# Adelaide-Autonomous-Racing-Kit/ac-mpc

Measured on AMD Instinct MI355X. Metric: candidate-trajectories/sec (horizon=50), higher is better.
Workload: dtype f32; 1 GPU; monza (synthetic circuit): 4096 candidates x horizon 50 per solve per GPU, 4096 solves (poses) batched per launch (256 distinct poses); mode S rollout + cost + argmin + winner record; horizon=50, mode=S, layout=U[P][n][2][N], parallelism=candidate-sharded x1, one all-reduce(MIN) of 4096 packed keys per step

## Files before the change

ac-mpc_amd/acmpc_amd/_build.py:

```python
from __future__ import annotations

import os
import shutil
import subprocess

PKG_DIR = os.path.dirname(os.path.abspath(__file__))
CSRC_DIR = os.path.normpath(os.path.join(PKG_DIR, "..", "csrc"))
LIB_DIR = os.path.join(PKG_DIR, "lib")
LIB_PATH = os.path.join(LIB_DIR, "libacmpc_hip.so")
SOURCES = ("acmpc_kernels.hip", "acmpc_kernels_temporal.hip", "acmpc_capi.hip", "acmpc_prologue.hip", "acmpc_pf.hip",
           "acmpc_speed_profile.cpp", "acmpc_host_path.cpp", "acmpc_dynamic.hip", "acmpc_dynamic_terms.hip", "acmpc_identify.hip")
HEADERS = ("acmpc_kernels.h", "acmpc_device.h", "acmpc_dynamic.h", "acmpc_identify.h", "acmpc_frames.h", "acmpc_admm.h", "acmpc_prologue.h", "acmpc_lq.h", "acmpc_lq_box.h",
           os.path.join("..", "..", "include", "acmpc.h"))

HIPCC_FLAGS = ("--offload-arch=gfx950", "-O3", "-std=c++17", "-fPIC", "-ffp-contract=off", "-Wall", "-Wextra")
EXTRA_FLAGS = {"acmpc_kernels_temporal.hip": ("-fno-slp-vectorize",), "acmpc_speed_profile.cpp": ("-mfma",)}


def find_hipcc() -> str:
    for cand in (os.environ.get("HIPCC"), shutil.which("hipcc"), "/opt/rocm/bin/hipcc"):
        if cand and os.path.exists(cand):
            return cand
    raise RuntimeError("hipcc not found: set HIPCC or install ROCm")


FLAGS_PATH = os.path.join(LIB_DIR, "build_flags.txt")


def flag_record() -> str:
    lines = ["common: " + " ".join(HIPCC_FLAGS)]
    lines += ["%s: %s" % (src, " ".join(EXTRA_FLAGS.get(src, ()))) for src in SOURCES]
    lines.append("experiment: " + " ".join(os.environ.get("ACMPC_HIPCC_EXTRA", "").split()))
    return "\n".join(lines) + "\n"


def is_stale() -> bool:
    if not os.path.exists(LIB_PATH) or not os.path.exists(FLAGS_PATH):
        return True
    built = os.path.getmtime(LIB_PATH)
    deps = [os.path.join(CSRC_DIR, f) for f in SOURCES + HEADERS]
    deps.append(os.path.abspath(__file__))
    if any(os.path.getmtime(d) > built for d in deps):
        return True
    with open(FLAGS_PATH) as handle:
        return handle.read() != flag_record()


def build_library(force: bool = False, verbose: bool = False) -> str:
    if not force and not is_stale():
        return LIB_PATH
    os.makedirs(LIB_DIR, exist_ok=True)
    obj_dir = os.path.join(LIB_DIR, "obj")
    os.makedirs(obj_dir, exist_ok=True)
    hipcc = find_hipcc()

    def run(cmd):
        if verbose:
            print(" ".join(cmd))
        proc = subprocess.run(cmd, capture_output=True, text=True)
        if proc.returncode != 0:
            raise RuntimeError("hipcc failed:\n" + proc.stdout + proc.stderr)

    from concurrent.futures import ThreadPoolExecutor
    objects = [os.path.join(obj_dir, os.path.splitext(src)[0] + ".o") for src in SOURCES]
    experiment = tuple(os.environ.get("ACMPC_HIPCC_EXTRA", "").split())
    with ThreadPoolExecutor(max_workers=4) as pool:
        list(pool.map(lambda so: run([hipcc, *HIPCC_FLAGS, *EXTRA_FLAGS.get(so[0], ()), *experiment, "-c",
                                      os.path.join(CSRC_DIR, so[0]), "-o", so[1]]), zip(SOURCES, objects)))
    run([hipcc, "--offload-arch=gfx950", "-shared", "-fPIC", *objects, "-o", LIB_PATH])
    with open(FLAGS_PATH, "w") as handle:
        handle.write(flag_record())
    return LIB_PATH


if __name__ == "__main__":
    print(build_library(force=True, verbose=True))
```

ac-mpc_amd/csrc/acmpc_capi.hip:

```cpp
#include <dlfcn.h>
#include <hip/hip_runtime.h>
#include <rccl/rccl.h>

#include <cmath>
#include <cstdio>
#include <cstdlib>
#include <cstring>
#include <algorithm>
#include <atomic>
#include <chrono>
#include <functional>
#include <limits>
#include <new>
#include <string>
#include <vector>

#include "../../include/acmpc.h"
#include "acmpc_dynamic.h"
#include "acmpc_frames.h"
#include "acmpc_identify.h"
#include "acmpc_kernels.h"
#include "acmpc_lq.h"
#include "acmpc_lq_box.h"
#include "acmpc_prologue.h"
// ... 13 lines not shown
  int coef_stride = 0;

  std::vector<float> h_coef;
  int P_set = 0, n_set = 0;
  bool tables_dirty = false;
  bool frames_dirty = false;

  bool device_ready = false;
  bool touched_device = false;
  float* d_coef = nullptr;
  int64_t* d_partial_keys = nullptr;
  int* d_partial_feas = nullptr;
  size_t partial_slots = 0;
  bool stream_pending = false;
  acmpc::FinalizeArgs stream_fin{};
  int stream_fin_layout = 0;
  int stream_set = 0;
  double* d_soft_partial = nullptr;
  size_t soft_partial_doubles = 0;

  float* d_segments = nullptr;
  int segments_n = 0;
  int knot_begin[acmpc::kKnots + 1] = {};
  float* d_centre = nullptr;
  float* d_uref = nullptr;

  bool staging_ready = false;
  hipStream_t stream = nullptr;
  float* d_U = nullptr;
  float* d_x0 = nullptr;
  float* d_costs = nullptr;
  float* d_records = nullptr;
  int64_t* d_keys = nullptr;
  int* d_tickets = nullptr;
  unsigned tick_sequence = 0;
  float* d_trace = nullptr;
  std::vector<float> h_nn_frames;
  float* d_nn_frames = nullptr;
  int64_t* h_keys = nullptr;
  float* h_io = nullptr;

  struct OptKey {
    int P = 0, N = 0, n = 0, rounds = 0, has_uref = 0;
    double sigma_v = 0, sigma_k = 0, shrink = 0;
    bool operator==(const OptKey& o) const {
      return P == o.P && N == o.N && n == o.n && rounds == o.rounds && has_uref == o.has_uref &&
             sigma_v == o.sigma_v && sigma_k == o.sigma_k && shrink == o.shrink;
    }
  };
  static constexpr int kOptGraphs = 4;
  hipGraphExec_t opt_graph[kOptGraphs] = {nullptr, nullptr, nullptr, nullptr};
  OptKey opt_key[kOptGraphs];
  uint64_t opt_used[kOptGraphs] = {0, 0, 0, 0};
  uint64_t opt_clock = 0;
  bool opt_ready = false;
  unsigned char* h_opt = nullptr;
  unsigned char* d_opt = nullptr;
  size_t opt_capacity = 0;
  float* h_opt_records = nullptr;
  uint32_t* d_seed = nullptr;

  struct TickKey {
    int N = 0, n = 0, rounds = 0, from_map = 0;
    double sigma_v = 0, sigma_k = 0, shrink = 0;
    bool operator==(const TickKey& o) const {
      return N == o.N && n == o.n && rounds == o.rounds && from_map == o.from_map && sigma_v == o.sigma_v &&
             sigma_k == o.sigma_k && shrink == o.shrink;
    }
  };
  bool tick_ready = false;
  hipGraphExec_t tick_graph[kOptGraphs] = {nullptr, nullptr, nullptr, nullptr};
  TickKey tick_key[kOptGraphs];
  uint64_t tick_used[kOptGraphs] = {0, 0, 0, 0};
  unsigned char* h_tick = nullptr;
  unsigned char* d_tick = nullptr;
  unsigned char* h_tick_out = nullptr;
  std::vector<double> h_map;
  double map_spacing = 0.0;
  bool map_dirty = false;
  double* d_map = nullptr;
  double* d_coords = nullptr;
  double* d_warm = nullptr;
  int warm_stride = 0;
  int tick_last_n = 0;

  std::vector<double> h_tables;
  float* h_lq = nullptr;
  std::vector<double> tick_prev_table;
  double tick_prev_x0[3] = {0.0, 0.0, 0.0};
  std::vector<double> tick_lq_table;
  std::vector<double> tick_lq_scratch;
  std::vector<double> tick_host_coords;
  int tick_prev_n = 0;
  bool want_start_clocks = false;
  unsigned long long* d_start_clock = nullptr;
  size_t start_clock_slots = 0;
  int start_clock_count = 0;
  std::vector<acmpc::lqbox::State> lq_box_state;
  acmpc::lqbox::Workspace lq_box_ws;
  acmpc::lqbox::Result lq_box_last;
  int lq_box_iterations = 40;

  acmpc::LaunchOptions opt;
  struct Switches {
    bool no_verified_search = false, no_solo = false, no_fused_finalize = false, no_traced_finalize = false,
         no_chained_rounds = false, no_chained_stream = false, no_graph = false, no_fused_sampling = false, tick_graph = false, tick_no_flag = false, tick_no_inline_path = false, no_zero_copy = false,
         tailed_rollout = false,
         dynamic_matrix_rounds = false;
  } sw;

  std::vector<hipEvent_t> prof_start, prof_stop;
  size_t prof_used = 0;

  bool has_dynamics = false;
  acmpc::VehicleEnsemble vehicles{};
  int substeps = 1;
  double blend_lo = 0.0, blend_hi = 0.0;
  double vehicle_L[acmpc::kMaxVehicles] = {};
  double vehicle0[acmpc::kDynamicsCount] = {};
  unsigned char* d_identify = nullptr;
  float* d_identify_e = nullptr;
  size_t identify_e_floats = 0;
  std::vector<unsigned char> h_identify;
  double rate_weight[2] = {0.0, 0.0}, rate_max[2] = {HUGE_VAL, HUGE_VAL};
  double slip_weight = 0.0, slip_max = HUGE_VAL;
  std::vector<float> h_uprev;
  int uprev_P = 0;
  bool uprev_dirty = false;
  float* d_uprev = nullptr;

  mutable std::string err;
};

namespace {

int fail(const acmpc_ctx* ctx, int code, const std::string& msg) {
  if (ctx != nullptr) {
    ctx->err = msg;
  } else {
    g_create_error = msg;
  }
  return code;
}

int fail_hip(const acmpc_ctx* ctx, hipError_t e, const char* what) {
  (void)hipGetLastError();
  const bool nodev = (e == hipErrorNoDevice || e == hipErrorInvalidDevice || e == hipErrorInsufficientDriver ||
                      e == hipErrorNotInitialized);
  return fail(ctx, nodev ? ACMPC_ENODEVICE : ACMPC_EHIP,
              std::string(what) + ": " + hipGetErrorName(e) + " (" + hipGetErrorString(e) + ")");
}

#define ACMPC_HIP(ctx, call)                                   \
  do {                                                         \
    const hipError_t e_ = (call);                              \
    if (e_ != hipSuccess) return fail_hip((ctx), e_, #call);   \
  } while (0)

constexpr int kMaxVerifiedSteps = 256;

void verified_frames(const float* coef, int P, int n, std::vector<float>* out) {
  constexpr int W = acmpc::kVerifiedWindow;
  const int windows = n - W + 1;
  const int floats = acmpc::verified_frame_floats(n);
  out->assign(static_cast<size_t>(P) * floats, 0.0f);
  std::vector<acmpc::frames::Geometry> geometry(static_cast<size_t>(windows));
  for (int p = 0; p < P; ++p) {
    const float* t = coef + static_cast<size_t>(p) * n * acmpc::kCoefT;
    const float ox = t[0], oy = t[1];
    auto at = [t, ox, oy](int m, double& x, double& y) {
      x = static_cast<double>(t[m * acmpc::kCoefT] - ox);
      y = static_cast<double>(t[m * acmpc::kCoefT + 1] - oy);
    };
    double wn = 0.0;
    bool finite = true;
    for (int m = 0; m < n; ++m) {
      double x, y;
      at(m, x, y);
      finite = finite && std::isfinite(x) && std::isfinite(y);
      wn = std::max(wn, std::sqrt(x * x + y * y));
    }
    float largest_gap2 = 0.0f;
    for (int m = 0; m + 1 < n; ++m) {
      const float gap2 = acmpc::frames::squared_gap(t[(m + 1) * acmpc::kCoefT] - ox, t[(m + 1) * acmpc::kCoefT + 1] - oy,
                                                    t[m * acmpc::kCoefT] - ox, t[m * acmpc::kCoefT + 1] - oy);
      largest_gap2 = (gap2 > largest_gap2) ? gap2 : largest_gap2;
    }
    const int first = acmpc::frames::near_first(largest_gap2);
    double slab_max = 0.0;
// ... 435 lines not shown
  a.x0 = d_x0;
  a.coef = c->d_coef;
  a.costs = d_costs;
  a.partial_keys = c->d_partial_keys;
  a.partial_feas = c->d_partial_feas;
  a.P = P;
  a.N = N;
  a.n = n;
  a.index_offset = 0;
  a.w = c->w;
  acmpc::FinalizeArgs f{};
  if (regen != nullptr) {
    f.regenerate = true;
    f.centre = regen->d_centre;
    f.centre_stride = regen->centre_stride;
    f.u_ref = regen->d_uref;
    f.u_extra = regen->d_extra;
    f.spec = regen->spec;
  }
  f.U = d_U;
  f.x0 = d_x0;
  f.coef = c->d_coef;
  f.partial_keys = c->d_partial_keys;
  f.partial_feas = c->d_partial_feas;
  f.keys_out = d_keys;
  f.records = d_records;
  f.blocks_per_problem = shape.blocks_per_problem;
  f.P = P;
  f.N = N;
  f.n = n;
  f.index_offset = 0;
  f.w = c->w;
  hipEvent_t e0 = nullptr, e1 = nullptr;
  if (c->prof_used < c->prof_start.size()) {
    e0 = c->prof_start[c->prof_used];
    e1 = c->prof_stop[c->prof_used];
    ++c->prof_used;
  }
  ACMPC_HIP(c, acmpc::launch_rollout_tailed(layout, shape, a, f, c->d_tickets, s, e0, e1));
  return ACMPC_OK;
}

int ensure_matrix(acmpc_ctx* c) {
  const acmpc_params& p = c->prm;
  ACMPC_HIP(c, alloc_once(&c->d_U, static_cast<size_t>(p.max_problems) * p.max_candidates * p.max_steps * 2 * sizeof(float)));
  return ACMPC_OK;
}

int ensure_staging(acmpc_ctx* c) {
  if (c->staging_ready) return ACMPC_OK;
  c->touched_device = true;
  const acmpc_params& p = c->prm;
  const size_t cand = static_cast<size_t>(p.max_problems) * p.max_candidates;
  ACMPC_HIP(c, alloc_once(&c->d_centre, static_cast<size_t>(p.max_problems) * p.max_steps * 2 * sizeof(float)));
  ACMPC_HIP(c, alloc_once(&c->d_uref, static_cast<size_t>(p.max_problems) * p.max_steps * 2 * sizeof(float)));
  if (c->stream == nullptr) ACMPC_HIP(c, hipStreamCreateWithFlags(&c->stream, hipStreamNonBlocking));
  if (p.mode != ACMPC_MODE_DYNAMIC) {
    const int rc_matrix = ensure_matrix(c);
    if (rc_matrix != ACMPC_OK) return rc_matrix;
  }
  const size_t state_floats = p.mode == ACMPC_MODE_DYNAMIC ? acmpc::kDynamicStateFloats : 3;
  ACMPC_HIP(c, alloc_once(&c->d_x0, static_cast<size_t>(p.max_problems) * state_floats * sizeof(float)));
  ACMPC_HIP(c, alloc_once(&c->d_costs, cand * sizeof(float)));
  ACMPC_HIP(c, alloc_once(&c->d_records,
                          static_cast<size_t>(p.max_problems) * acmpc_record_floats(p.max_steps) * sizeof(float)));
  ACMPC_HIP(c, alloc_once(&c->d_keys, static_cast<size_t>(p.max_problems) * sizeof(int64_t)));
  const int rc_tail = ensure_tail_buffers(c);
  if (rc_tail != ACMPC_OK) return rc_tail;
  ACMPC_HIP(c, host_alloc_once(&c->h_keys, static_cast<size_t>(p.max_problems) * sizeof(int64_t)));
  ACMPC_HIP(c, host_alloc_once(&c->h_io, (static_cast<size_t>(p.max_problems) * (state_floats + acmpc_record_floats(p.max_steps)) + 4) * sizeof(float)));
  if (p.lq_candidate != 0 && c->h_lq == nullptr) {
    const size_t lq_bytes = static_cast<size_t>(p.max_problems) * p.max_steps * 2 * sizeof(float);
    ACMPC_HIP(c, host_alloc_once(&c->h_lq, lq_bytes));
    std::memset(c->h_lq, 0, lq_bytes);
  }
  c->staging_ready = true;
  return ACMPC_OK;
}

const char* const kOptionNames[] = {
    "ACMPC_SHAPE", "ACMPC_T_PACK", "ACMPC_NO_TILE", "ACMPC_TILE_ROWS", "ACMPC_TILE_TABLE", "ACMPC_NO_TRIO_ROUNDS",
    "ACMPC_NO_QUAD_ROUNDS", "ACMPC_NO_PAIR_ROUNDS", "ACMPC_SOLO_REGISTERS", "ACMPC_SOLO_SPLIT", "ACMPC_NO_VERIFIED_SEARCH",
    "ACMPC_NO_SOLO", "ACMPC_NO_FUSED_FINALIZE", "ACMPC_NO_TRACED_FINALIZE", "ACMPC_NO_CHAINED_ROUNDS", "ACMPC_NO_GRAPH",
    "ACMPC_NO_FUSED_SAMPLING", "ACMPC_TICK_GRAPH", "ACMPC_TICK_NO_FLAG", "ACMPC_TICK_NO_INLINE_PATH", "ACMPC_NO_ZERO_COPY", "ACMPC_TAILED_ROLLOUT", "ACMPC_NO_GROUP_FINALIZE", "ACMPC_FINALIZE_WAVES",
    "ACMPC_NO_CHAINED_STREAM", "ACMPC_LQ_BOX_ITERATIONS", "ACMPC_START_CLOCKS", "ACMPC_DYNAMIC_MATRIX_ROUNDS",
    "ACMPC_CONFORMANT_SYNC"};

bool apply_option(acmpc_ctx* c, const char* name, const char* value) {
  const std::string key(name);
  const bool present = value != nullptr && value[0] != '\0';
  const bool on = present && !(value[0] == '0' && value[1] == '\0');
  auto tri = [&](int* field) { *field = present ? (value[0] == '1' ? 1 : 0) : -1; return true; };
  acmpc::LaunchOptions& o = c->opt;
  if (key == "ACMPC_SHAPE") {
    o.shape_block = o.shape_cpt = 0;
    if (present && std::sscanf(value, "%d,%d", &o.shape_block, &o.shape_cpt) != 2) o.shape_block = o.shape_cpt = 0;
    return true;
  }
  if (key == "ACMPC_T_PACK") { o.temporal_pack = present ? (value[0] == '1' ? 1 : 2) : 0; return true; }
  if (key == "ACMPC_NO_TILE") { o.no_tile = on; return true; }
  if (key == "ACMPC_TILE_ROWS") { o.tile_rows = present ? std::atoi(value) : -1; return true; }
  if (key == "ACMPC_TILE_TABLE") { o.tile_table = present ? (value[0] == 'l' ? 1 : 2) : 0; return true; }
  if (key == "ACMPC_NO_TRIO_ROUNDS") { o.no_trio_rounds = on; return true; }
  if (key == "ACMPC_NO_QUAD_ROUNDS") { o.no_quad_rounds = on; return true; }
  if (key == "ACMPC_NO_PAIR_ROUNDS") { o.no_pair_rounds = on; return true; }
  if (key == "ACMPC_SOLO_REGISTERS") return tri(&o.solo_registers);
  if (key == "ACMPC_SOLO_SPLIT") return tri(&o.solo_split);
  if (key == "ACMPC_NO_GROUP_FINALIZE") { o.no_group_finalize = on; return true; }
  if (key == "ACMPC_FINALIZE_WAVES") { o.finalize_waves = on; return true; }
  acmpc_ctx::Switches& w = c->sw;
  if (key == "ACMPC_NO_VERIFIED_SEARCH") { w.no_verified_search = on; return true; }
  if (key == "ACMPC_NO_SOLO") { w.no_solo = on; return true; }
  if (key == "ACMPC_NO_FUSED_FINALIZE") { w.no_fused_finalize = on; return true; }
  if (key == "ACMPC_NO_TRACED_FINALIZE") { w.no_traced_finalize = on; return true; }
  if (key == "ACMPC_NO_CHAINED_ROUNDS") { w.no_chained_rounds = on; return true; }
  if (key == "ACMPC_NO_CHAINED_STREAM") { w.no_chained_stream = on; return true; }
  if (key == "ACMPC_NO_GRAPH") { w.no_graph = on; return true; }
  if (key == "ACMPC_NO_FUSED_SAMPLING") { w.no_fused_sampling = on; return true; }
  if (key == "ACMPC_TICK_GRAPH") { w.tick_graph = on; return true; }
  if (key == "ACMPC_TICK_NO_FLAG") { w.tick_no_flag = on; return true; }
  if (key == "ACMPC_TICK_NO_INLINE_PATH") { w.tick_no_inline_path = on; return true; }
  if (key == "ACMPC_NO_ZERO_COPY") { w.no_zero_copy = on; return true; }
  if (key == "ACMPC_TAILED_ROLLOUT") { w.tailed_rollout = on; return true; }
  if (key == "ACMPC_START_CLOCKS") { c->want_start_clocks = on; return true; }
  if (key == "ACMPC_DYNAMIC_MATRIX_ROUNDS") { w.dynamic_matrix_rounds = on; return true; }
  if (key == "ACMPC_CONFORMANT_SYNC") {
    w.no_solo = w.no_fused_finalize = w.no_chained_stream = w.tick_no_flag = on;
    if (on) w.tailed_rollout = false;
    return true;
  }
  if (key == "ACMPC_LQ_BOX_ITERATIONS") { c->lq_box_iterations = present ? std::max(0, std::atoi(value)) : 40; return true; }
  return false;
}

}

extern "C" {

const char* acmpc_version(void) { return "acmpc-hip 0.1 gfx950"; }

int32_t acmpc_record_floats(int32_t n) { return ACMPC_REC_HEADER + 2 * n + 3 * (n + 1); }

int acmpc_lq_plan(const double* table, int32_t n, const double x0[3], const double step_cost[3], const double r_term[2],
                  const double final_cost[3], const float u_min[2], const float u_max[2], float* plan) {
  if (table == nullptr || x0 == nullptr || step_cost == nullptr || r_term == nullptr || final_cost == nullptr ||
      u_min == nullptr || u_max == nullptr || plan == nullptr || n < 1)
    return ACMPC_EINVAL;
  return acmpc::lq::plan(table, n, x0, step_cost, r_term, final_cost, u_min, u_max, plan) ? ACMPC_OK : ACMPC_ESTATE;
}

int acmpc_lq_box_plan(const double* table, int32_t n, const double x0[3], const double step_cost[3], const double r_term[2],
                      const double final_cost[3], const float u_min[2], const float u_max[2], double margin, double w_bound,
                      int32_t iterations, double* state, float* plan, double* info) {
  if (table == nullptr || x0 == nullptr || step_cost == nullptr || r_term == nullptr || final_cost == nullptr ||
      u_min == nullptr || u_max == nullptr || plan == nullptr || state == nullptr || info == nullptr || n < 1)
    return ACMPC_EINVAL;
  if (!acmpc::lq::plan(table, n, x0, step_cost, r_term, final_cost, u_min, u_max, plan)) return ACMPC_ESTATE;
  acmpc::lqbox::State st;
  const size_t m = static_cast<size_t>(n) * 2;
  if (state[0] == static_cast<double>(n)) {
    st.n = n;
    st.wx.assign(state + 1, state + 1 + m);
    st.wu.assign(state + 1 + m, state + 1 + 2 * m);
    st.lx.assign(state + 1 + 2 * m, state + 1 + 3 * m);
    st.lu.assign(state + 1 + 3 * m, state + 1 + 4 * m);
  }
  acmpc::lqbox::Workspace ws;
  const acmpc::lqbox::Result r = acmpc::lqbox::refine(table, n, x0, step_cost, r_term, final_cost, u_min, u_max, margin,
                                                      w_bound, iterations, st, ws, plan);
  state[0] = static_cast<double>(st.n);
  if (st.n == n) {
    std::copy(st.wx.begin(), st.wx.end(), state + 1);
    std::copy(st.wu.begin(), st.wu.end(), state + 1 + m);
    std::copy(st.lx.begin(), st.lx.end(), state + 1 + 2 * m);
    std::copy(st.lu.begin(), st.lu.end(), state + 1 + 3 * m);
  }
  info[0] = r.iterations, info[1] = r.chosen, info[2] = r.triggered ? 1.0 : 0.0, info[3] = r.cost.J, info[4] = r.cost.V;
  return ACMPC_OK;
}

int acmpc_lq_box_stats(const acmpc_ctx* c, double info[5]) {
  if (c == nullptr || info == nullptr) return ACMPC_EINVAL;
  const acmpc::lqbox::Result& r = c->lq_box_last;
  info[0] = r.iterations, info[1] = r.chosen, info[2] = r.triggered ? 1.0 : 0.0, info[3] = r.cost.J, info[4] = r.cost.V;
  return ACMPC_OK;
}

int64_t acmpc_pack_key(float cost, uint32_t index) { return acmpc::pack_key(cost, index); }

float acmpc_key_cost(int64_t key) {
  const int32_t hi = static_cast<int32_t>(key >> 32);
  const int32_t bits = (hi >= 0) ? hi : (hi ^ 0x7fffffff);
  float f;
  std::memcpy(&f, &bits, sizeof f);
  return f;
}

uint32_t acmpc_key_index(int64_t key) { return static_cast<uint32_t>(key & 0xffffffffLL); }

const char* acmpc_last_error(const acmpc_ctx* ctx) { return ctx != nullptr ? ctx->err.c_str() : g_create_error.c_str(); }

int acmpc_create(const acmpc_params* params, acmpc_ctx** out) {
  if (params == nullptr || out == nullptr) return fail(nullptr, ACMPC_EINVAL, "null argument");
  *out = nullptr;
// ... 834 lines not shown
  if (rc != ACMPC_OK) return rc;
  Regenerate regen{d_centre, centre_stride, d_u_ref, make_spec(c, sigma_v, sigma_kappa, seed, round)};
  const int blocks = c->prm.mode == ACMPC_MODE_DYNAMIC
                         ? acmpc::dynamic_blocks_per_problem(P, N, c->vehicles.K)
                         : acmpc::choose_shape(P, N, ACMPC_LAYOUT_STEP_MAJOR, c->prm.mode, n, c->opt).blocks_per_problem;
  return finalize(c, d_keys, nullptr, d_x0, nullptr, P, N, n, ACMPC_LAYOUT_STEP_MAJOR, 0, d_records, blocks, s, &regen);
}

int acmpc_rollout_sampled_device(acmpc_ctx* c, const float* d_x0, const float* d_centre, int32_t centre_stride,
                                 const float* d_u_ref, int32_t P, int32_t N, int32_t n, int64_t index_offset,
                                 double sigma_v, double sigma_kappa, uint64_t seed, uint32_t round, float* d_costs,
                                 int64_t* d_keys, void* stream) {
  if (c == nullptr) return ACMPC_EINVAL;
  if (d_x0 == nullptr || d_centre == nullptr) return fail(c, ACMPC_EINVAL, "null device pointer");
  if (c->prm.mode != ACMPC_MODE_DYNAMIC)
    return fail(c, ACMPC_ESTATE, "acmpc_rollout_sampled_device is mode D's: modes S and T draw inside acmpc_optimize");
  if (centre_stride < 2 * n) return fail(c, ACMPC_EINVAL, "centre_stride must be at least 2 n");
  if (index_offset < 0 || index_offset + N > 0xffffffffLL) return fail(c, ACMPC_EINVAL, "global index exceeds 32 bits");
  int rc = check_shape(c, P, N, n, ACMPC_LAYOUT_STEP_MAJOR);
  if (rc != ACMPC_OK) return rc;
  rc = ensure_device(c);
  if (rc != ACMPC_OK) return rc;
  hipStream_t s = static_cast<hipStream_t>(stream);
  rc = upload_tables(c, s);
  if (rc != ACMPC_OK) return rc;
  rc = rollout_sampled_dynamic(c, d_x0, d_centre, centre_stride, d_u_ref, P, N, n, index_offset, sigma_v, sigma_kappa, seed,
                               round, d_costs, s);
  if (rc != ACMPC_OK || d_keys == nullptr) return rc;
  return finalize(c, nullptr, d_keys, d_x0, nullptr, P, N, n, ACMPC_LAYOUT_STEP_MAJOR, index_offset, nullptr,
                  acmpc::dynamic_blocks_per_problem(P, N, c->vehicles.K), s);
}

extern "C++" {
namespace {

struct OptInputs {
  const float* x0;
  const float* centre;
  const float* uref;
  const float* coef;
  const float* frames = nullptr;
  const float* extra = nullptr;
  std::function<bool()> before_last;
};

const float* own_frames(const acmpc_ctx* c) { return c->h_nn_frames.empty() ? nullptr : c->d_nn_frames; }

bool use_fused_finalize(const acmpc_ctx* c, int n) {
  return !c->sw.no_fused_finalize && acmpc::fused_finalize_fits(c->prm.mode, n);
}

bool use_traced_finalize(const acmpc_ctx* c, int P, int N, int n) {
  return !c->sw.no_traced_finalize && acmpc::traced_finalize_fits(c->prm.mode, n) &&
         static_cast<long long>(P) * ((N + 63) / 64) <= kTraceBlocks;
}

bool lq_plan_into(acmpc_ctx* c, const double* table, int n, const double start[3], float* out,
                  bool start_is_pose = false, int problem = 0) {
  double x0[3] = {start[0], start[1], start[2]};
  if (start_is_pose || c->prm.mode == ACMPC_MODE_TEMPORAL) acmpc::lq::frenet_start(table, n, start, x0);
  const float lo[2] = {c->w.ulo0, c->w.ulo1}, hi[2] = {c->w.uhi0, c->w.uhi1};
  const bool finite_start = std::isfinite(x0[0]) && std::isfinite(x0[1]) && std::isfinite(x0[2]);
  if (finite_start && acmpc::lq::plan(table, n, x0, c->prm.step_cost, c->prm.r_term, c->prm.final_cost, lo, hi, out)) {
    if (c->prm.lq_candidate == 2) {
      if (c->lq_box_state.size() <= static_cast<size_t>(problem)) c->lq_box_state.resize(static_cast<size_t>(problem) + 1);
      c->lq_box_last = acmpc::lqbox::refine(table, n, x0, c->prm.step_cost, c->prm.r_term, c->prm.final_cost, lo, hi,
                                            c->prm.margin, c->prm.w_bound, c->lq_box_iterations,
                                            c->lq_box_state[static_cast<size_t>(problem)], c->lq_box_ws, out);
    }
    return true;
  }
  if (c->prm.lq_candidate == 2 && c->lq_box_state.size() > static_cast<size_t>(problem))
    c->lq_box_state[static_cast<size_t>(problem)].reset();
  const double *kappa = table + 3 * static_cast<size_t>(n), *vel = table + 6 * static_cast<size_t>(n);
  for (int i = 0; i < n; ++i) {
    out[2 * i] = std::fmin(std::fmax(static_cast<float>(vel[i]), lo[0]), hi[0]);
    out[2 * i + 1] = std::fmin(std::fmax(static_cast<float>(kappa[i]), lo[1]), hi[1]);
  }
  return false;
}

int enqueue_rounds(acmpc_ctx* c, const OptInputs& in, int P, int N, int n, int rounds, double sigma_v, double sigma_k,
                   double shrink, uint64_t seed, const uint32_t* d_seed, hipStream_t s, bool fused,
                   float* final_records = nullptr, unsigned* done = nullptr, unsigned done_value = 0) {
  const bool has_uref = in.uref != nullptr;
  const bool fused_finalize = use_fused_finalize(c, n);
  const int layout = ACMPC_LAYOUT_STEP_MAJOR;
  const int rec_floats = acmpc_record_floats(n);
  double scale = 1.0;
  for (int r = 0; r < rounds; ++r, scale *= shrink) {
    const float* d_c = (r == 0) ? in.centre : c->d_records + ACMPC_REC_HEADER;
    const int stride = (r == 0) ? 2 * n : rec_floats;
    const float* d_ref = has_uref ? in.uref : nullptr;
    const float* d_extra = nullptr;
    if (r + 1 == rounds && in.extra != nullptr && (!in.before_last || in.before_last())) d_extra = in.extra;
    if (!fused) {
      const bool softmin = c->prm.centre_update == 1;
      const bool mean_round = softmin && r > 0;
      if (mean_round)
        ACMPC_HIP(c, hipMemcpy2DAsync(c->d_uref, static_cast<size_t>(2 * n) * sizeof(float),
                                      c->d_records + ACMPC_REC_HEADER, static_cast<size_t>(rec_floats) * sizeof(float),
                                      static_cast<size_t>(2 * n) * sizeof(float), P, hipMemcpyDeviceToDevice, s));
      int rc = sample(c, mean_round ? c->d_centre : d_c, mean_round ? 2 * n : stride, mean_round ? c->d_uref : d_ref, P,
                      N, n, layout, 0, sigma_v * scale, sigma_k * scale, seed, static_cast<uint32_t>(r), c->d_U, s,
                      d_seed, d_extra);
      if (rc != ACMPC_OK) return rc;
      acmpc::LaunchShape shape;
      rc = rollout(c, in.x0, c->d_U, P, N, n, layout, 0, softmin ? c->d_costs : nullptr, s, &shape);
      if (rc != ACMPC_OK) return rc;
      rc = finalize(c, nullptr, softmin ? c->d_keys : nullptr, in.x0, c->d_U, P, N, n, layout, 0, c->d_records,
                    shape.blocks_per_problem, s);
      if (rc != ACMPC_OK) return rc;
      if (softmin && r + 1 < rounds) {
        acmpc::SoftminArgs sm{};
        sm.costs = c->d_costs;
        sm.keys = c->d_keys;
        sm.U = c->d_U;
        sm.partial = c->d_soft_partial;
        sm.mean = c->d_centre;
        sm.weight_sum = nullptr;
        sm.chunks = acmpc::softmin_chunks(N);
        sm.P = P;
        sm.N = N;
        sm.n = n;
        sm.lambda = static_cast<float>(c->prm.softmin_lambda);
        ACMPC_HIP(c, acmpc::launch_softmin(layout, sm, s));
      }
      continue;
    }
    int rc = upload_segments(c, n, s);
    if (rc != ACMPC_OK) return rc;
    const int blocks = (N + 63) / 64;
    const bool traced = fused_finalize && use_traced_finalize(c, P, N, n);
    const bool chain = traced && blocks <= acmpc::kChainBlocks && !c->sw.no_chained_rounds;
    const size_t set = (chain && (r & 1)) ? 1 : 0;
    const size_t trace_set_floats = static_cast<size_t>(kTraceBlocks) * acmpc::trace_floats(c->prm.max_steps);
    float* d_trace = c->d_trace + set * trace_set_floats;
    acmpc::RolloutArgs ra{};
    ra.x0 = in.x0;
    ra.coef = in.coef;
    ra.nn_frames = !c->sw.no_verified_search ? in.frames : nullptr;
    ra.partial_keys = c->d_partial_keys + set * c->partial_slots;
    ra.partial_feas = c->d_partial_feas + set * c->partial_slots;
    ra.P = P;
    ra.N = N;
    ra.n = n;
    ra.index_offset = 0;
    ra.w = c->w;
    acmpc::SampleArgs sa{};
    sa.centre = d_c;
    sa.centre_stride = stride;
    sa.u_ref = d_ref;
    sa.u_extra = d_extra;
    sa.P = P;
    sa.N = N;
    sa.n = n;
    sa.spec = make_spec(c, sigma_v * scale, sigma_k * scale, seed, static_cast<uint32_t>(r));
    sa.spec.seed_ptr = d_seed;
    if (chain && r > 0) {
      sa.prev_keys = c->d_partial_keys + (set ^ 1) * c->partial_slots;
      sa.prev_trace = c->d_trace + (set ^ 1) * trace_set_floats;
      sa.prev_blocks = blocks;
      sa.prev_pitch = acmpc::trace_floats(n);
    }
    hipEvent_t e0 = nullptr, e1 = nullptr;
    if (c->prof_used < c->prof_start.size()) {
      e0 = c->prof_start[c->prof_used];
      e1 = c->prof_stop[c->prof_used];
      ++c->prof_used;
    }
    if (fused_finalize) {
      const bool last = r + 1 == rounds;
      const bool tail = last || !chain;
      const acmpc::FusedFinalize ff{tail ? c->d_tickets : nullptr,
                                    (last && final_records != nullptr) ? final_records : c->d_records, !last,
                                    traced ? d_trace : nullptr, acmpc::trace_floats(n),
                                    last ? done : nullptr, done_value};
      ACMPC_HIP(c, acmpc::launch_rollout_sampled(c->prm.mode, ra, sa, ff, s, e0, e1, c->opt));
    } else {
      ACMPC_HIP(c, acmpc::launch_rollout_sampled(c->prm.mode, ra, sa, acmpc::FusedFinalize{nullptr, nullptr, false, nullptr, 0, nullptr, 0}, s, e0, e1, c->opt));
      Regenerate regen{d_c, stride, d_ref, sa.spec, d_extra};
      rc = finalize(c, nullptr, nullptr, in.x0, nullptr, P, N, n, layout, 0, c->d_records, (N + 63) / 64, s, &regen,
                    in.coef);
      if (rc != ACMPC_OK) return rc;
    }
  }
  return ACMPC_OK;
}

}
}

int acmpc_optimize(acmpc_ctx* c, const float* x0, const float* centre, const float* u_ref, int32_t P, int32_t N,
                   int32_t n, int32_t rounds, const double sigma[2], double shrink, uint64_t seed, float* records) {
  if (c == nullptr) return ACMPC_EINVAL;
  if (x0 == nullptr || centre == nullptr || sigma == nullptr || records == nullptr)
    return fail(c, ACMPC_EINVAL, "null argument");
  if (rounds < 1) return fail(c, ACMPC_EINVAL, "rounds must be positive");
  const int layout = ACMPC_LAYOUT_STEP_MAJOR;
  int rc = check_shape(c, P, N, n, layout);
  if (rc != ACMPC_OK) return rc;
  if (c->prm.mode == ACMPC_MODE_DYNAMIC && c->prm.centre_update == 1 && !(c->prm.softmin_lambda > 0.0))
    return fail(c, ACMPC_EINVAL, "softmin_lambda must be positive");
  rc = ensure_device(c);
  if (rc != ACMPC_OK) return rc;
  rc = ensure_staging(c);
  if (rc != ACMPC_OK) return rc;
  if (c->prm.mode == ACMPC_MODE_DYNAMIC) {
    return optimize_dynamic(c, x0, centre, u_ref, P, N, n, rounds, sigma, shrink, seed, records);
  }
  hipStream_t s = c->stream;
  const size_t x0_bytes = static_cast<size_t>(P) * 3 * sizeof(float);
  const size_t path_bytes = static_cast<size_t>(P) * n * 2 * sizeof(float);
  const size_t table_bytes = static_cast<size_t>(P) * n * c->coef_stride * sizeof(float);
  const size_t rec_bytes = static_cast<size_t>(P) * acmpc_record_floats(n) * sizeof(float);
  const bool has_uref = u_ref != nullptr;
  const bool has_extra = c->prm.lq_candidate != 0 && c->h_tables.size() == static_cast<size_t>(P) * 7 * n;
  if (has_extra) {
    for (int p = 0; p < P; ++p) {
      const double start[3] = {x0[3 * p], x0[3 * p + 1], x0[3 * p + 2]};
      (void)lq_plan_into(c, c->h_tables.data() + static_cast<size_t>(p) * 7 * n, n, start, c->h_lq + static_cast<size_t>(p) * n * 2,
                         false, p);
    }
  }

  if (c->prof_used < c->prof_start.size() || c->sw.no_graph) {
    rc = upload_tables(c, s);
    if (rc != ACMPC_OK) return rc;
    ACMPC_HIP(c, hipMemcpyAsync(c->d_x0, x0, x0_bytes, hipMemcpyHostToDevice, s));
    ACMPC_HIP(c, hipMemcpyAsync(c->d_centre, centre, path_bytes, hipMemcpyHostToDevice, s));
    if (has_uref) ACMPC_HIP(c, hipMemcpyAsync(c->d_uref, u_ref, path_bytes, hipMemcpyHostToDevice, s));
    OptInputs in{c->d_x0, c->d_centre, has_uref ? c->d_uref : nullptr, c->d_coef, own_frames(c)};
    in.extra = has_extra ? c->h_lq : nullptr;
    rc = enqueue_rounds(c, in, P, N, n, rounds, sigma[0], sigma[1], shrink, seed, nullptr, s,
                        !c->sw.no_fused_sampling && c->prm.centre_update == 0);
    if (rc != ACMPC_OK) return rc;
    ACMPC_HIP(c, hipMemcpyAsync(records, c->d_records, rec_bytes, hipMemcpyDeviceToHost, s));
    ACMPC_HIP(c, hipStreamSynchronize(s));
    return ACMPC_OK;
  }

  auto align16 = [](size_t v) { return (v + 15) & ~static_cast<size_t>(15); };
  const size_t off_x0 = 0, off_centre = align16(off_x0 + x0_bytes), off_uref = align16(off_centre + path_bytes),
               off_table = align16(off_uref + path_bytes), off_seed = align16(off_table + table_bytes);
  if (!c->opt_ready) {
    const acmpc_params& p = c->prm;
    const size_t cap = 64 + 16 * 5 + static_cast<size_t>(p.max_problems) *
                                         (3 + 4 * static_cast<size_t>(p.max_steps) +
                                          static_cast<size_t>(p.max_steps) * c->coef_stride) * sizeof(float);
    ACMPC_HIP(c, host_alloc_once(&c->h_opt, cap));
    ACMPC_HIP(c, alloc_once(&c->d_opt, cap));
    c->opt_capacity = cap;
    ACMPC_HIP(c, host_alloc_once(&c->h_opt_records,
                                 static_cast<size_t>(p.max_problems) * acmpc_record_floats(p.max_steps) * sizeof(float)));
    ACMPC_HIP(c, alloc_once(&c->d_seed, 2 * sizeof(uint32_t)));
    c->opt_ready = true;
  }
  acmpc_ctx::OptKey key;
  key.P = P;
  key.N = N;
  key.n = n;
  key.rounds = rounds;
// ... 70 lines not shown
  ACMPC_HIP(c, hipGraphLaunch(c->opt_graph[slot], s));
  ACMPC_HIP(c, hipStreamSynchronize(s));
  std::memcpy(records, c->h_opt_records, rec_bytes);
  return ACMPC_OK;
}


extern "C++" {
namespace {

size_t align16(size_t v) { return (v + 15) & ~static_cast<size_t>(15); }

struct TickLayout {
  size_t coords, centre_in, host_total;
  size_t seed, x0, centre, uref, coef, frames, total;
  explicit TickLayout(int n, int coef_stride = ACMPC_COEF_STRIDE_SPATIAL) {
    coords = align16(sizeof(acmpc::TickHeader));
    centre_in = align16(coords + static_cast<size_t>(n + 1) * 3 * sizeof(double));
    host_total = align16(centre_in + static_cast<size_t>(n) * 2 * sizeof(float));
    seed = 0;
    x0 = 16;
    centre = 32;
    uref = align16(centre + static_cast<size_t>(n) * 2 * sizeof(float));
    coef = align16(uref + static_cast<size_t>(n) * 2 * sizeof(float));
    frames = align16(coef + static_cast<size_t>(n) * coef_stride * sizeof(float));
    total = align16(frames + static_cast<size_t>(acmpc::verified_frame_floats(std::max(n, acmpc::kVerifiedWindow))) * sizeof(float));
  }
};

struct TickOutLayout {
  size_t record, table, status, coords, done, total;
  explicit TickOutLayout(int n) {
    record = 0;
    table = align16(static_cast<size_t>(acmpc_record_floats(n)) * sizeof(float));
    status = align16(table + static_cast<size_t>(7) * n * sizeof(double));
    coords = status + 16;
    done = align16(coords + static_cast<size_t>(n + 1) * 3 * sizeof(double));
    total = done + 16;
  }
};

int upload_map(acmpc_ctx* c, hipStream_t s) {
  if (!c->map_dirty) return ACMPC_OK;
  for (hipGraphExec_t& g : c->tick_graph) {
    if (g != nullptr) (void)hipGraphExecDestroy(g);
    g = nullptr;
  }
  ACMPC_HIP(c, hipStreamSynchronize(s));
  (void)hipFree(c->d_map);
  c->d_map = nullptr;
  ACMPC_HIP(c, hipMalloc(reinterpret_cast<void**>(&c->d_map), c->h_map.size() * sizeof(double)));
  ACMPC_HIP(c, hipMemcpyAsync(c->d_map, c->h_map.data(), c->h_map.size() * sizeof(double), hipMemcpyHostToDevice, s));
  ACMPC_HIP(c, hipStreamSynchronize(s));
  c->map_dirty = false;
  return ACMPC_OK;
}

int map_window_args(acmpc_ctx* c, int H, int points, const TickOutLayout& out, acmpc::MapWindowArgs* a) {
  if (c->h_map.empty()) return fail(c, ACMPC_ESTATE, "no map bound (acmpc_bind_map)");
  if (points < H || points % H != 0) return fail(c, ACMPC_EINVAL, "centreline_points must be a multiple of the horizon");
  a->header = reinterpret_cast<const acmpc::TickHeader*>(c->h_tick);
  a->centre = c->d_map;
  a->M = static_cast<int>(c->h_map.size() / 2);
  a->count = static_cast<int>(std::lround(150.0 / c->map_spacing)) + 1;
  if (a->count < 2 || a->count > a->M) return fail(c, ACMPC_EINVAL, "the map is shorter than the 150 m look-ahead window");
  a->points = points;
  a->H = H;
  a->coords = c->d_coords;
  a->coords_out = reinterpret_cast<double*>(c->h_tick_out + out.coords);
  a->first_out = reinterpret_cast<int*>(c->h_tick_out + out.status) + 2;
  return ACMPC_OK;
}

int ensure_tick(acmpc_ctx* c) {
  if (c->tick_ready) return ACMPC_OK;
  c->touched_device = true;
  const int n_cap = std::min(c->prm.max_steps, acmpc::kPrologueMaxSteps);
  ACMPC_HIP(c, host_alloc_once(&c->h_tick, TickLayout(n_cap).host_total));
  ACMPC_HIP(c, alloc_once(&c->d_tick, TickLayout(n_cap).total));
  ACMPC_HIP(c, host_alloc_once(&c->h_tick_out, TickOutLayout(n_cap).total));
  std::memset(c->h_tick_out, 0, TickOutLayout(n_cap).total);
  ACMPC_HIP(c, alloc_once(&c->d_coords, static_cast<size_t>(n_cap + 1) * 3 * sizeof(double)));
  c->warm_stride = 2 + 3 * n_cap;
  const size_t warm_bytes = static_cast<size_t>(2) * c->warm_stride * sizeof(double);
  ACMPC_HIP(c, alloc_once(&c->d_warm, warm_bytes));
  ACMPC_HIP(c, hipMemset(c->d_warm, 0, warm_bytes));
  ACMPC_HIP(c, hipStreamSynchronize(nullptr));
  c->tick_ready = true;
  return ACMPC_OK;
}

}
}

int acmpc_control_tick(acmpc_ctx* c, const acmpc_tick* t, const double* coords, const float* centre, double* table,
                       float* record, double* decision, double* projected_control, double* prediction,
                       double* cum_time, double* times, double* accelerations, double* steer_rates, double* info,
                       double* coords_out) {
  if (c == nullptr) return ACMPC_EINVAL;
  if (t == nullptr || table == nullptr || record == nullptr || decision == nullptr ||
      projected_control == nullptr || prediction == nullptr || cum_time == nullptr || times == nullptr ||
      accelerations == nullptr || steer_rates == nullptr || info == nullptr)
    return fail(c, ACMPC_EINVAL, "null argument");
  if (t->struct_size != sizeof(acmpc_tick)) return fail(c, ACMPC_EINVAL, "acmpc_tick size mismatch");
  if (c->stream_pending)
    return fail(c, ACMPC_ESTATE, "a batch of acmpc_solve_stream_device is pending: acmpc_solve_stream_flush first");
  if (c->prm.mode == ACMPC_MODE_DYNAMIC)
    return fail(c, ACMPC_ESTATE, "mode D has no control tick: use acmpc_set_paths + acmpc_optimize");
  if (c->prm.centre_update != 0) return fail(c, ACMPC_ESTATE, "acmpc_control_tick needs a handle with centre_update = 0");
  const bool temporal = c->prm.mode == ACMPC_MODE_TEMPORAL;
  if (temporal && !(c->prm.dt > 0.0)) return fail(c, ACMPC_ESTATE, "mode T needs a positive dt");
  const int H = t->horizon, n = H - 1, N = t->n_candidates;
  if (H < 3 || t->rounds < 1 || N < 1) return fail(c, ACMPC_EINVAL, "need horizon >= 3, rounds >= 1, n_candidates >= 1");
  if (n > c->prm.max_steps || N > c->prm.max_candidates) return fail(c, ACMPC_ECAPACITY, "horizon or candidates exceed capacity");
  if (n > acmpc::kPrologueMaxSteps) return fail(c, ACMPC_ESTATE, "the device prologue holds at most 128 steps");
  if (centre == nullptr && t->centre_is_reference == 0) return fail(c, ACMPC_EINVAL, "null centre");
  if (coords == nullptr && c->h_map.empty()) return fail(c, ACMPC_EINVAL, "null coords and no map bound");
  if (!acmpc::fused_finalize_fits(c->prm.mode, n)) return fail(c, ACMPC_ESTATE, "fused finalize does not fit");
  int rc = ensure_device(c);
  if (rc != ACMPC_OK) return rc;
  rc = ensure_staging(c);
  if (rc != ACMPC_OK) return rc;
  rc = ensure_tick(c);
  if (rc != ACMPC_OK) return rc;
  hipStream_t s = c->stream;
  const TickLayout in(n, c->coef_stride);
  const TickOutLayout out(n);
  const int rec_floats = acmpc_record_floats(n);
  const bool from_map = coords == nullptr;
  acmpc::MapWindowArgs ma{};
  if (from_map) {
    rc = map_window_args(c, H, t->centreline_points, out, &ma);
    if (rc != ACMPC_OK) return rc;
    rc = upload_map(c, s);
    if (rc != ACMPC_OK) return rc;
    ma.centre = c->d_map;
  }

  acmpc::PrologueArgs pa{};
  pa.header = reinterpret_cast<const acmpc::TickHeader*>(c->h_tick);
  pa.coords = reinterpret_cast<const double*>(c->h_tick + in.coords);
  if (from_map) {
    pa.map_centre = c->d_map;
    pa.map_M = ma.M;
    pa.map_count = ma.count;
    pa.map_points = ma.points;
    pa.map_first = reinterpret_cast<const int*>(c->d_coords);
    pa.coords_out = ma.coords_out;
    pa.index_out = ma.first_out;
    ma.coords = nullptr;
    ma.coords_out = nullptr;
    ma.first_out = reinterpret_cast<int*>(c->d_coords);
  }
  pa.temporal = temporal ? 1 : 0;
  pa.centre_in = reinterpret_cast<const float*>(c->h_tick + in.centre_in);
  pa.x0 = reinterpret_cast<float*>(c->d_tick + in.x0);
  pa.u_ref = reinterpret_cast<float*>(c->d_tick + in.uref);
  pa.coef = reinterpret_cast<float*>(c->d_tick + in.coef);
  pa.frames = (temporal && c->prm.nn_ahead < 0 && n >= acmpc::kVerifiedWindow && acmpc::trio_frames_fit(n) &&
               !c->opt.no_trio_rounds && !c->sw.no_verified_search)
                  ? reinterpret_cast<float*>(c->d_tick + in.frames)
                  : nullptr;
  pa.centre = reinterpret_cast<float*>(c->d_tick + in.centre);
  pa.seed = reinterpret_cast<uint32_t*>(c->d_tick + in.seed);
  pa.table_out = reinterpret_cast<double*>(c->h_tick_out + out.table);
  pa.status = reinterpret_cast<int*>(c->h_tick_out + out.status);
  pa.warm_state = c->d_warm;
  pa.warm_stride = c->warm_stride;
  pa.warm_capacity = (c->warm_stride - 2) / 3;
  pa.margin = c->prm.margin;
  pa.u_lo0 = c->prm.u_min[0];
  pa.u_lo1 = c->prm.u_min[1];
  pa.u_hi0 = c->prm.u_max[0];
  pa.u_hi1 = c->prm.u_max[1];
  const bool direct = use_fused_finalize(c, n);
  const bool use_graph = c->sw.tick_graph;
  const bool lq_on = c->prm.lq_candidate != 0;
  const double lq_offset = t->offset;
  const bool host_window = lq_on && from_map && t->map_index >= 0;
  const int window_M = ma.M, window_count = ma.count, window_points = ma.points;
  auto plan_previous = [c, n, H, given = coords, lq_offset, t, host_window, window_M, window_count, window_points]() -> bool {
    const double* coords = given;
    if (host_window) {
      c->tick_host_coords.resize(static_cast<size_t>(H) * 3);
      const int first = ((t->map_index % window_M) + window_M) % window_M;
      const acmpc::MapFrame frame = acmpc::map_frame(c->h_map.data(), window_M, first);
      for (int r = 0; r < H; ++r) {
        double row[3];
        acmpc::map_path_row(c->h_map.data(), window_M, first, window_count, window_points, H, r, t->lateral_offset, frame, row);
        for (int e = 0; e < 3; ++e) c->tick_host_coords[static_cast<size_t>(3) * r + e] = row[e];
      }
      coords = c->tick_host_coords.data();
    }
    const bool have_previous = c->tick_prev_n == n;
    if (!have_previous && coords == nullptr) return false;
    if (coords == nullptr) return lq_plan_into(c, c->tick_prev_table.data(), n, c->tick_prev_x0, c->h_lq);
    c->tick_lq_table.resize(static_cast<size_t>(7) * n);
    if (acmpc_waypoint_table(coords, H, kEps, c->tick_lq_table.data()) != ACMPC_OK) return false;
    {
      c->tick_lq_scratch.resize(static_cast<size_t>(3) * n);
      double* ceiling = c->tick_lq_scratch.data();
      double* dual = ceiling + n;
      double* profile = c->tick_lq_table.data() + static_cast<size_t>(6) * n;
      const double* spacing = c->tick_lq_table.data() + static_cast<size_t>(4) * n;
      int32_t iterations = 0;
      if (acmpc_velocity_ceiling(c->tick_lq_table.data() + static_cast<size_t>(3) * n, n, t->ay_max, t->ki_min, t->v_min,
                                 t->v_max, t->localised, t->has_end_velocity, t->end_velocity, ceiling) != ACMPC_OK)
        return false;
      const bool swept = t->qp_method == 0 &&
                         acmpc_speed_profile_exact(ceiling, spacing, n, t->a_min, t->a_max, t->v_min, profile, dual) == 0;
      if (!swept) {
        if (have_previous) {
          std::memcpy(profile, c->tick_prev_table.data() + static_cast<size_t>(6) * n, static_cast<size_t>(n) * sizeof(double));
        } else if (acmpc_speed_profile_qp(ceiling, spacing, n, t->a_min, t->a_max, t->v_min, t->qp_max_iter, t->qp_check_every,
                                          t->qp_eps_abs, t->qp_eps_rel, profile, dual, 0, &iterations) != 0) {
          return false;
        }
      }
    }
    const double pose[3] = {lq_offset, 0.0, M_PI / 2.0};
    return lq_plan_into(c, c->tick_lq_table.data(), n, pose, c->h_lq, true);
  };
  const bool flagged = direct && !use_graph && !c->sw.tick_no_flag;
  unsigned* done_flag = reinterpret_cast<unsigned*>(c->h_tick_out + out.done);
  const unsigned done_value = ++c->tick_sequence;
  auto enqueue = [&](hipStream_t q, int* rc_rounds) -> hipError_t {
    hipError_t e = (from_map && t->map_index < 0) ? acmpc::launch_map_window(ma, q) : hipSuccess;
    if (e == hipSuccess) e = acmpc::launch_prologue(pa, n, q);
    if (e != hipSuccess) return e;
    OptInputs oi{pa.x0, pa.centre, pa.u_ref, pa.coef, pa.frames};
    if (lq_on) {
      oi.extra = c->h_lq;
      if (!use_graph) oi.before_last = plan_previous;
    }
    *rc_rounds = enqueue_rounds(c, oi, 1, N, n, t->rounds, t->sigma[0], t->sigma[1], t->shrink,
                                use_graph ? 0 : t->seed, use_graph ? pa.seed : nullptr, q, true,
                                direct ? reinterpret_cast<float*>(c->h_tick_out + out.record) : nullptr,
                                flagged ? done_flag : nullptr, done_value);
    if (*rc_rounds == ACMPC_OK && !direct)
      e = hipMemcpyAsync(c->h_tick_out + out.record, c->d_records, static_cast<size_t>(rec_floats) * sizeof(float),
                         hipMemcpyDeviceToHost, q);
    return e;
  };
  int slot = -1;
  if (use_graph) {
    acmpc_ctx::TickKey key;
    key.N = N;
    key.n = n;
    key.rounds = t->rounds;
    key.sigma_v = t->sigma[0];
    key.sigma_k = t->sigma[1];
    key.shrink = t->shrink;
    key.from_map = from_map ? (t->map_index < 0 ? -t->centreline_points : t->centreline_points) : 0;
    for (int g = 0; g < acmpc_ctx::kOptGraphs; ++g)
      if (c->tick_graph[g] != nullptr && key == c->tick_key[g]) slot = g;
    if (slot < 0) {
      slot = 0;
      for (int g = 1; g < acmpc_ctx::kOptGraphs; ++g)
        if (c->tick_used[g] < c->tick_used[slot]) slot = g;
      if (c->tick_graph[slot] != nullptr) {
        (void)hipGraphExecDestroy(c->tick_graph[slot]);
        c->tick_graph[slot] = nullptr;
      }
      rc = upload_segments(c, n, s);
      if (rc != ACMPC_OK) return rc;
      hipGraph_t graph = nullptr;
      ACMPC_HIP(c, hipStreamBeginCapture(s, hipStreamCaptureModeThreadLocal));
      int rc_rounds = ACMPC_OK;
      const hipError_t e = enqueue(s, &rc_rounds);
      const hipError_t e_end = hipStreamEndCapture(s, &graph);
      if (rc_rounds != ACMPC_OK) {
        if (graph != nullptr) (void)hipGraphDestroy(graph);
        return rc_rounds;
      }
      if (e != hipSuccess) {
        if (graph != nullptr) (void)hipGraphDestroy(graph);
        return fail_hip(c, e, "capturing the tick graph");
      }
      ACMPC_HIP(c, e_end);
      const hipError_t e_inst = hipGraphInstantiate(&c->tick_graph[slot], graph, nullptr, nullptr, 0);
      (void)hipGraphDestroy(graph);
      if (e_inst != hipSuccess) c->tick_graph[slot] = nullptr;
      ACMPC_HIP(c, e_inst);
      c->tick_key[slot] = key;
    }
    c->tick_used[slot] = ++c->opt_clock;
  } else {
    rc = upload_segments(c, n, s);
    if (rc != ACMPC_OK) return rc;
  }

  acmpc::TickHeader* h = reinterpret_cast<acmpc::TickHeader*>(c->h_tick);
  h->offset = t->offset;
  h->v_min = t->v_min;
  h->v_max = t->v_max;
  h->a_min = t->a_min;
  h->a_max = t->a_max;
  h->ay_max = t->ay_max;
  h->ki_min = t->ki_min;
  h->end_velocity = t->end_velocity;
  h->qp_eps_abs = t->qp_eps_abs;
  h->qp_eps_rel = t->qp_eps_rel;
  h->eps = kEps;
  h->horizon = H;
  h->localised = t->localised;
  h->has_end_velocity = t->has_end_velocity;
  h->centre_is_reference = t->centre_is_reference;
  h->qp_max_iter = t->qp_max_iter;
  h->qp_check_every = t->qp_check_every;
  h->qp_method = t->qp_method;
  h->seed_lo = static_cast<uint32_t>(t->seed);
  h->seed_hi = static_cast<uint32_t>(t->seed >> 32);
  h->use_map = from_map ? 1 : 0;
  h->map_index = t->map_index;
  h->pose_x = t->pose_x;
  h->pose_y = t->pose_y;
  h->lateral_offset = t->lateral_offset;
  if (!from_map) std::memcpy(c->h_tick + in.coords, coords, static_cast<size_t>(H) * 3 * sizeof(double));
  if (centre != nullptr) std::memcpy(c->h_tick + in.centre_in, centre, static_cast<size_t>(n) * 2 * sizeof(float));
  if (use_graph) {
    if (lq_on && !plan_previous()) {
      if (centre != nullptr && t->centre_is_reference == 0)
        std::memcpy(c->h_lq, centre, static_cast<size_t>(n) * 2 * sizeof(float));
      else
        std::memset(c->h_lq, 0, static_cast<size_t>(n) * 2 * sizeof(float));
    }
    ACMPC_HIP(c, hipGraphLaunch(c->tick_graph[slot], s));
  } else {
    pa.header_by_value = 1;
    pa.header_value = *h;
    if (!from_map && H <= acmpc::kInlinePathPoints && !c->sw.tick_no_inline_path) {
      pa.path_by_value = 1;
      std::memcpy(pa.coords_value, coords, static_cast<size_t>(H) * 3 * sizeof(double));
      if (centre != nullptr) std::memcpy(pa.centre_value, centre, static_cast<size_t>(n) * 2 * sizeof(float));
    }
    int rc_rounds = ACMPC_OK;
    const hipError_t e = enqueue(s, &rc_rounds);
    if (rc_rounds != ACMPC_OK || e != hipSuccess) {
      (void)hipStreamSynchronize(s);
      if (rc_rounds != ACMPC_OK) return rc_rounds;
      ACMPC_HIP(c, e);
    }
  }
  if (flagged) {
    volatile unsigned* flag = done_flag;
    const auto give_up = std::chrono::steady_clock::now() + std::chrono::milliseconds(200);
    unsigned spins = 0;
    while (*flag != done_value) {
      __builtin_ia32_pause();
      if ((++spins & 0x3fffu) == 0 && std::chrono::steady_clock::now() > give_up) break;
    }
    std::atomic_thread_fence(std::memory_order_acquire);
    if (*flag != done_value) {
      ACMPC_HIP(c, hipStreamSynchronize(s));
      if (*flag != done_value) return fail(c, ACMPC_EHIP, "the tick finished without its completion flag");
    }
  } else {
    ACMPC_HIP(c, hipStreamSynchronize(s));
  }
  c->tick_last_n = n;

  const float* rec = reinterpret_cast<const float*>(c->h_tick_out + out.record);
  std::memcpy(record, rec, static_cast<size_t>(rec_floats) * sizeof(float));
  std::memcpy(table, c->h_tick_out + out.table, static_cast<size_t>(7) * n * sizeof(double));
  const int* status = reinterpret_cast<const int*>(c->h_tick_out + out.status);
  const float* ru = rec + ACMPC_REC_HEADER;
  const float* rx = ru + 2 * n;
  double biggest = 0.0;
  bool finite = std::isfinite(rec[ACMPC_REC_COST]) && std::isfinite(rec[ACMPC_REC_VIOLATION]);
  for (int i = 0; i < 3 * (n + 1); ++i) {
    decision[i] = static_cast<double>(rx[i]);
    biggest = std::max(biggest, std::fabs(decision[i]));
    finite = finite && std::isfinite(rx[i]);
  }
  for (int i = 0; i < 2 * n; ++i) {
    decision[3 * (n + 1) + i] = static_cast<double>(ru[i]);
    biggest = std::max(biggest, std::fabs(static_cast<double>(ru[i])));
    finite = finite && std::isfinite(ru[i]);
  }
  rc = temporal ? acmpc_unpack_decision_temporal(decision, n, c->prm.dt, c->prm.wheelbase, projected_control, prediction,
                                                 cum_time, times, accelerations, steer_rates)
                : acmpc_unpack_decision(decision, n, table, c->prm.wheelbase, projected_control, prediction, cum_time,
                                        times, accelerations, steer_rates);
  if (rc != ACMPC_OK) return fail(c, rc, "acmpc_unpack_decision");
  info[0] = rec[ACMPC_REC_COST];
  info[1] = rec[ACMPC_REC_VIOLATION];
  info[2] = rec[ACMPC_REC_NFEASIBLE];
  info[3] = biggest;
  info[4] = status[0];
  info[5] = status[1];
  info[6] = from_map ? static_cast<double>(status[2]) : -1.0;
  info[7] = finite ? 0.0 : 1.0;
  if (lq_on) {
    c->tick_prev_n = (finite && status[0] == 0) ? n : 0;
    if (c->tick_prev_n != 0) {
      c->tick_prev_table.assign(table, table + static_cast<size_t>(7) * n);
      for (int q = 0; q < 3; ++q) c->tick_prev_x0[q] = static_cast<double>(rx[q]);
    }
  }
  if (coords_out != nullptr)
    std::memcpy(coords_out, from_map ? reinterpret_cast<const void*>(c->h_tick_out + out.coords)
                                     : reinterpret_cast<const void*>(coords),
                static_cast<size_t>(H) * 3 * sizeof(double));
  return ACMPC_OK;
}

int acmpc_bind_map(acmpc_ctx* c, const double* centre, int32_t M, double spacing) {
  if (c == nullptr) return ACMPC_EINVAL;
  if (centre == nullptr || M < 3 || !(spacing > 0.0)) return fail(c, ACMPC_EINVAL, "need a centre line of >= 3 points and a positive spacing");
  c->h_map.assign(centre, centre + 2 * static_cast<size_t>(M));
  c->map_spacing = spacing;
  c->map_dirty = true;
  return ACMPC_OK;
}

int acmpc_map_reference_path(acmpc_ctx* c, int32_t map_index, double pose_x, double pose_y, double lateral_offset,
                             int32_t horizon, int32_t centreline_points, double* coords, int32_t* first_index) {
  if (c == nullptr) return ACMPC_EINVAL;
  if (coords == nullptr) return fail(c, ACMPC_EINVAL, "null output");
  const int n = horizon - 1;
  if (horizon < 3 || n > std::min(c->prm.max_steps, acmpc::kPrologueMaxSteps))
    return fail(c, ACMPC_ECAPACITY, "horizon out of range for this handle");
  int rc = ensure_device(c);
  if (rc != ACMPC_OK) return rc;
  rc = ensure_staging(c);
  if (rc != ACMPC_OK) return rc;
  rc = ensure_tick(c);
  if (rc != ACMPC_OK) return rc;
  hipStream_t s = c->stream;
  const TickOutLayout out(n);
  acmpc::MapWindowArgs ma{};
  rc = map_window_args(c, horizon, centreline_points, out, &ma);
  if (rc != ACMPC_OK) return rc;
  rc = upload_map(c, s);
  if (rc != ACMPC_OK) return rc;
  ma.centre = c->d_map;
  acmpc::TickHeader* h = reinterpret_cast<acmpc::TickHeader*>(c->h_tick);
  h->use_map = 1;
  h->map_index = map_index;
  h->pose_x = pose_x;
  h->pose_y = pose_y;
  h->lateral_offset = lateral_offset;
  ACMPC_HIP(c, acmpc::launch_map_window(ma, s));
  ACMPC_HIP(c, hipStreamSynchronize(s));
  std::memcpy(coords, c->h_tick_out + out.coords, static_cast<size_t>(horizon) * 3 * sizeof(double));
  if (first_index != nullptr) *first_index = reinterpret_cast<const int*>(c->h_tick_out + out.status)[2];
  return ACMPC_OK;
}
// ... 242 lines not shown
```

ac-mpc_amd/csrc/acmpc_kernels.h:

```cpp
#pragma once
#include <hip/hip_runtime.h>
#include <stdint.h>

#include "acmpc_device.h"

namespace acmpc {

struct RolloutArgs {
  const float* U;
  const float* x0;
  const float* coef;
  const float* nn_frames;
  float* costs;
  int64_t* partial_keys;
  int* partial_feas;
  int P, N, n;
  int64_t index_offset;
  Weights w;
  int even_progress = 0;
  unsigned long long* start_clock = nullptr;
};

struct FinalizeArgs {
  const float* U;
  const float* x0;
  const float* coef;
  const int64_t* partial_keys;
  const int* partial_feas;
  const int64_t* keys_in;
  int64_t* keys_out;
  float* records;
  bool regenerate;
  bool controls_only;
  const float* centre;
  const float* u_ref;
  const float* u_extra;
  int centre_stride;
  SampleSpec spec;
  int blocks_per_problem;
  int P, N, n;
  int64_t index_offset;
  Weights w;
};

struct SoftminArgs {
  const float* costs;
  const int64_t* keys;
  const float* U;
  double* partial;
  float* mean;
  double* weight_sum;
  int chunks;
  int P, N, n;
  float lambda;
};

constexpr int kSampleKnots = kKnots;

struct SampleArgs {
  const float* centre;
  const float* u_ref;
  const float* u_extra;
  float* U;
  int centre_stride;
  int P, N, n;
  int64_t index_offset;
  SampleSpec spec;
  const int64_t* prev_keys;
  const float* prev_trace;
  int prev_blocks;
  int prev_pitch;
};
constexpr int kTileRowsMaxSteps = 80;
constexpr int kChainBlocks = 256;

struct LaunchOptions {
  int shape_block = 0, shape_cpt = 0;
  int temporal_pack = 0;
  bool no_tile = false;
  int tile_rows = -1;
  int tile_table = 0;
  bool no_trio_rounds = false, no_quad_rounds = false, no_pair_rounds = false;
  int solo_registers = -1, solo_split = -1;
  bool no_group_finalize = false;
  bool finalize_waves = false;
};

struct LaunchShape {
  int block;
  int cpt;
  int blocks_per_problem;
  bool tile;
  int tile_waves;
  int pack;
  int tile_table = 0;
};

LaunchShape choose_shape(int P, int N, int layout, int mode, int n, const LaunchOptions& opt = LaunchOptions());
int max_blocks_per_problem(int N);
size_t tile_lds_bytes(int mode, int n);

hipError_t launch_rollout(int mode, int layout, const LaunchShape& shape, const RolloutArgs& args, hipStream_t s,
                          hipEvent_t start = nullptr, hipEvent_t stop = nullptr);
hipError_t launch_rollout_temporal_plain(const LaunchShape& shape, const RolloutArgs& args, hipStream_t s,
                                         hipEvent_t start, hipEvent_t stop);
hipError_t launch_rollout_tile_rows_plain(const LaunchShape& shape, const RolloutArgs& args, hipStream_t s,
                                          hipEvent_t start, hipEvent_t stop);
hipError_t launch_finalize(int mode, int layout, const FinalizeArgs& args, hipStream_t s,
                           const LaunchOptions& opt = LaunchOptions());
bool chained_rollout_fits(int mode, int layout, const LaunchShape& shape, int P, const FinalizeArgs& fin, int fin_layout);
hipError_t launch_rollout_chained(int layout, const LaunchShape& shape, const RolloutArgs& args, const FinalizeArgs& fin,
                                  int fin_layout, hipStream_t s, hipEvent_t e0, hipEvent_t e1);
bool tailed_rollout_fits(int mode, int layout, const LaunchShape& shape, int n);
hipError_t launch_rollout_tailed(int layout, const LaunchShape& shape, const RolloutArgs& args, const FinalizeArgs& fin,
                                 int* tickets, hipStream_t s, hipEvent_t start = nullptr, hipEvent_t stop = nullptr);
hipError_t launch_sample(int layout, const SampleArgs& args, hipStream_t s);
constexpr int kTicketGroups = 8;
constexpr int kTicketStride = 64;
constexpr int kTicketGroupsMax = 32;
constexpr int kSoloBlocks = 1024;
struct FusedFinalize {
  int* tickets;
  float* records;
  bool controls_only;
  float* trace;
  int trace_pitch;
  unsigned* done;
  unsigned done_value;
  int64_t* keys_out = nullptr;
  int ticket_groups = 0;
};

hipError_t launch_rollout_sampled(int mode, const RolloutArgs& rollout, const SampleArgs& sample,
                                  const FusedFinalize& fused, hipStream_t s, hipEvent_t start = nullptr,
                                  hipEvent_t stop = nullptr, const LaunchOptions& opt = LaunchOptions());
bool solo_fits(int P, int N, int n, int layout, const LaunchOptions& opt = LaunchOptions());
int solo_trace_floats(int n);
hipError_t launch_rollout_solo(int layout, const RolloutArgs& args, const FusedFinalize& fused, hipStream_t s,
                               hipEvent_t start = nullptr, hipEvent_t stop = nullptr,
                               const LaunchOptions& opt = LaunchOptions());
int trace_floats(int n);
bool trio_frames_fit(int n);
bool traced_finalize_fits(int mode, int n);
bool fused_finalize_fits(int mode, int n);
int softmin_chunks(int N);
hipError_t launch_softmin(int layout, const SoftminArgs& args, hipStream_t s);
hipError_t launch_softmin_sampled(const SoftminArgs& args, const SampleArgs& sample, hipStream_t s);

}
```

ac-mpc_amd/csrc/acmpc_kernels.hip:

```cpp
#include "acmpc_kernels.h"

#include <hip/hip_ext.h>

#include <algorithm>
#include <cstdint>
#include <cstdio>
#include <cstdlib>
#include <type_traits>

#pragma clang fp contract(off)

#if defined(__HIP_DEVICE_COMPILE__) && !defined(__gfx950__)
#error "acmpc kernels are written for gfx950 (MI355X): see the note above before building for another architecture"
#endif

namespace acmpc {

namespace {

typedef float f32x4 __attribute__((ext_vector_type(4)));

#ifdef ACMPC_STAMPS
__device__ unsigned long long g_stamps[4096 * 16];
#define ACMPC_STAMP(slot)                                                                                         \
  do {                                                                                                            \
    if ((threadIdx.x & 63) == 0)                                                                                  \
      g_stamps[((blockIdx.y * gridDim.x + blockIdx.x) * 2 + (threadIdx.x >> 6)) * 16 + (slot)] = wall_clock64(); \
  } while (0)
#else
#define ACMPC_STAMP(slot) \
  do {                    \
  } while (0)
#endif

template <int CPT>
struct VecOf;
template <>
struct VecOf<1> {
  using type = float;
};
template <>
struct VecOf<2> {
  using type = f32x2;
};
template <>
struct VecOf<4> {
  using type = f32x4;
};

template <int CPT>
__device__ __forceinline__ void unpack(const typename VecOf<CPT>::type& v, float (&out)[CPT]) {
  if constexpr (CPT == 1) {
    out[0] = v;
  } else {
#pragma unroll
    for (int j = 0; j < CPT; ++j) out[j] = v[j];
  }
}

template <int LAYOUT, int CPT>
__device__ __forceinline__ void load_controls(const float* __restrict__ U, int p, int N, int n, int i, int c0,
                                              float (&v)[CPT], float (&k)[CPT]) {
  if constexpr (LAYOUT == 1) {
    using V = typename VecOf<CPT>::type;
    const float* row = U + (static_cast<size_t>(p) * n + i) * 2 * static_cast<size_t>(N) + c0;
    unpack<CPT>(__builtin_nontemporal_load(reinterpret_cast<const V*>(row)), v);
    unpack<CPT>(__builtin_nontemporal_load(reinterpret_cast<const V*>(row + N)), k);
  } else {
#pragma unroll
    for (int j = 0; j < CPT; ++j) {
      const f32x2 vk = *reinterpret_cast<const f32x2*>(U + ((static_cast<size_t>(p) * N + c0 + j) * n + i) * 2);
      v[j] = vk[0];
      k[j] = vk[1];
    }
  }
}

template <typename T>
__device__ __forceinline__ void publish(T* where, T value) {
  __hip_atomic_store(where, value, __ATOMIC_RELAXED, __HIP_MEMORY_SCOPE_AGENT);
}
template <typename T>
__device__ __forceinline__ T observe(const T* where) {
// ... 1010 lines not shown
  }
  wave_lds_handoff();

  float J = 0.0f, V = 0.0f;
  for (int base = 0; base < n; base += kAhead) {
    f32x4 first[kAhead];
    float ht[kAhead];
#pragma unroll
    for (int j = 0; j < kAhead; ++j) {
      const int i = min(base + j, n - 1);
      first[j] = *reinterpret_cast<const f32x4*>(s_terms + i * kGroupRow);
      ht[j] = s_terms[i * kGroupRow + 4];
    }
#pragma unroll
    for (int j = 0; j < kAhead; ++j) {
      if (base + j < n) {
        J = J + first[j][0];
        V = V + first[j][1];
        V = V + first[j][2];
        V = V + first[j][3];
        V = V + ht[j];
      }
    }
  }
  wave_lds_handoff();
  if (owner) {
    if (sub == 0) {
      const StateS st{ey, ep, t, J, V};
      s_rec[0] = finish_spatial(st, w);
      s_rec[1] = V;
      s_rec[2] = static_cast<float>(nfeas);
      s_rec[3] = 1.0f;
    }
  } else {
    for (int e = sub; e < rec_floats; e += kLanes) s_rec[e] = (e == 2) ? static_cast<float>(nfeas) : 0.0f;
  }
  wave_lds_handoff();
  const int count = min(kProblems, a.P - p_first) * rec_floats;
  float* __restrict__ out = a.records + static_cast<size_t>(p_first) * rec_floats;
  const int whole = ((reinterpret_cast<uintptr_t>(out) & 15u) == 0) ? (count & ~3) : 0;
  for (int e = 4 * lane; e < whole; e += 4 * kWave) *reinterpret_cast<f32x4*>(out + e) = *reinterpret_cast<const f32x4*>(s_group + e);
  for (int e = whole + lane; e < count; e += kWave) out[e] = s_group[e];
}

template <int LAYOUT>
__global__ void __launch_bounds__(kWave) finalize_groups_kernel(const FinalizeArgs a) {
  extern __shared__ __attribute__((aligned(16))) float s_group[];
  finalize_group<LAYOUT, kGroupPass, kGroupAhead>(a, static_cast<int>(blockIdx.x), s_group);
}

constexpr int kFinalizeWaves = 4;

template <int LAYOUT>
__global__ void __launch_bounds__(kFinalizeWaves * kWave) finalize_waves_kernel(const FinalizeArgs a) {
  extern __shared__ __attribute__((aligned(16))) float s_group[];
  const int wave = static_cast<int>(threadIdx.x) / kWave;
  const int p = static_cast<int>(blockIdx.x) * kFinalizeWaves + wave;
  if (p >= a.P) return;
  finalize_group<LAYOUT, 1, kGroupAhead, kWave>(a, p, s_group + wave * group_finalize_floats_device(a.n));
}

#ifndef ACMPC_CHAINED_PASS
#define ACMPC_CHAINED_PASS 1
#endif
#ifndef ACMPC_CHAINED_AHEAD
#define ACMPC_CHAINED_AHEAD 4
#endif
template <int LAYOUT, int CPT, int BLOCK, int PACK>
__global__ void __launch_bounds__(BLOCK, 8) rollout_chained_kernel(const RolloutArgs a, const FinalizeArgs f) {
  extern __shared__ __attribute__((aligned(16))) unsigned char smem[];
  const int y = static_cast<int>(blockIdx.y);
  if (y >= a.P) {
    static_assert(BLOCK == kFinalizeWaves * kWave, "a finalize workgroup is four wavefronts, a problem each");
    const int wave = static_cast<int>(threadIdx.x) / kWave;
    const int p = ((y - a.P) * static_cast<int>(gridDim.x) + static_cast<int>(blockIdx.x)) * kFinalizeWaves + wave;
    if (p >= f.P) return;
    finalize_group<1, ACMPC_CHAINED_PASS, ACMPC_CHAINED_AHEAD, kWave>(
        f, p, reinterpret_cast<float*>(smem) + wave * group_finalize_floats_device(f.n));
    return;
  }
  rollout_block<0, LAYOUT, CPT, BLOCK, PACK, false>(a, smem, y);
}

__device__ __forceinline__ void finalize_from_trace(const RolloutArgs& a, const FusedFinalize& fused, const int p) {
  const int lane = threadIdx.x;
  const int n = a.n;
  const int blocks = static_cast<int>(gridDim.x);
  constexpr int kBatch = 4;
  int nfeas = 0;
  int64_t key = kKeyMax;
  for (int b0 = 0; b0 < blocks; b0 += kBatch * kWave) {
    int64_t kb[kBatch];
    int fb[kBatch];
#pragma unroll
    for (int q = 0; q < kBatch; ++q) {
      kb[q] = kKeyMax;
      fb[q] = 0;
      if (b0 + q * kWave < blocks) {
        const size_t slot = static_cast<size_t>(p) * blocks + min(b0 + q * kWave + lane, blocks - 1);
        kb[q] = observe(&a.partial_keys[slot]);
        fb[q] = observe(&a.partial_feas[slot]);
      }
    }
#pragma unroll
    for (int q = 0; q < kBatch; ++q) {
      const bool mine = b0 + q * kWave + lane < blocks;
      key = (mine && kb[q] < key) ? kb[q] : key;
      nfeas += mine ? fb[q] : 0;
    }
  }
  nfeas = wave_sum_int(nfeas);
  const int64_t best = wave_min_key(key);
  const int block = static_cast<int>(static_cast<int64_t>(static_cast<uint32_t>(best & 0xffffffffLL)) - a.index_offset) / kWave;
  const float* trace = fused.trace + (static_cast<size_t>(p) * blocks + block) * fused.trace_pitch;
  const int rec_floats = 4 + 2 * n + 3 * (n + 1);
  float* __restrict__ rec = fused.records + static_cast<size_t>(p) * rec_floats;
  const float* __restrict__ x0 = a.x0 + p * 3;
  const int count = fused.controls_only ? 4 + 2 * n : rec_floats;
  constexpr int kSlots = 8;
  for (int e0 = 0; e0 < count; e0 += kSlots * kWave) {
    float value[kSlots];
#pragma unroll
    for (int q = 0; q < kSlots; ++q) {
      if (e0 + q * kWave < count) {
        const int e = min(e0 + q * kWave + lane, count - 1);
        const float* src = trace + (e - 7);
        src = (e < 4 + 2 * n + 3) ? x0 + (e - (4 + 2 * n)) : src;
        src = (e < 4 + 2 * n) ? trace + (e - 4) : src;
        src = (e < 4) ? trace + 5 * n + (1 - min(e, 1)) : src;
        value[q] = observe(src);
      }
    }
#pragma unroll
    for (int q = 0; q < kSlots; ++q) {
      const int e = e0 + q * kWave + lane;
      if (e0 + q * kWave < count) {
        float out = value[q];
        if (fused.controls_only) out = (e == 0) ? key_cost(best) : (e == 1) ? 0.0f : out;
        out = (e == 2) ? static_cast<float>(nfeas) : (e == 3) ? 1.0f : out;
        if (e < count) rec[e] = out;
      }
    }
  }
}

__device__ __forceinline__ bool last_workgroup_of_problem(int* tickets, const int groups_cfg) {
  const int blocks = static_cast<int>(gridDim.x);
  const int group = static_cast<int>(blockIdx.x) & (groups_cfg - 1);
  const int group_size = (blocks - group + groups_cfg - 1) / groups_cfg;
  const int groups = min(blocks, groups_cfg);
  published();
  ACMPC_STAMP(5);
  int ticket = 0;
  if (threadIdx.x == 0) ticket = atomicAdd(&tickets[group * kTicketStride], 1);
  ticket = __builtin_amdgcn_readfirstlane(ticket);
  __atomic_signal_fence(__ATOMIC_SEQ_CST);
  if (ticket != group_size - 1) return false;
  ACMPC_STAMP(6);
  if (threadIdx.x == 0) {
    publish(&tickets[group * kTicketStride], 0);
    ticket = atomicAdd(&tickets[groups_cfg * kTicketStride], 1);
  }
  ticket = __builtin_amdgcn_readfirstlane(ticket);
  __atomic_signal_fence(__ATOMIC_SEQ_CST);
  if (ticket != groups - 1) return false;
  ACMPC_STAMP(7);
  if (threadIdx.x == 0) publish(&tickets[groups_cfg * kTicketStride], 0);
  return true;
}

#ifndef ACMPC_TAILED_WAVES
#define ACMPC_TAILED_WAVES 8
#endif
template <int MODE, int LAYOUT, int CPT, int BLOCK, int PACK>
__global__ void __launch_bounds__(BLOCK, ACMPC_TAILED_WAVES) rollout_tailed_kernel(const RolloutArgs a, const FinalizeArgs f, int* tickets) {
  extern __shared__ __attribute__((aligned(16))) unsigned char smem[];
  rollout_block<MODE, LAYOUT, CPT, BLOCK, PACK, true>(a, smem, static_cast<int>(blockIdx.y));
  if (threadIdx.x >= kWave) return;
  const int p = blockIdx.y;
  if (!last_workgroup_of_problem(tickets + static_cast<size_t>(p) * (kTicketGroups + 1) * kTicketStride, kTicketGroups)) return;
  finalize_problem<MODE, LAYOUT>(f, p, reinterpret_cast<float*>(smem + 64));
}

template <int MODE>
__device__ __forceinline__ void fused_tail(const RolloutArgs& a, const SampleArgs& smp, const FusedFinalize& fused,
                                           const bool traced, float* s_finalize) {
  const int p = blockIdx.y;
  if (fused.tickets == nullptr) return;
  if (!last_workgroup_of_problem(fused.tickets + static_cast<size_t>(p) * (kTicketGroups + 1) * kTicketStride, kTicketGroups)) return;
  auto signal_done = [&]() {
    if (fused.done == nullptr || p != 0) return;
    __threadfence_system();
    if (threadIdx.x == 0) __hip_atomic_store(fused.done, fused.done_value, __ATOMIC_RELAXED, __HIP_MEMORY_SCOPE_SYSTEM);
  };
  if (traced) {
    finalize_from_trace(a, fused, p);
    signal_done();
    return;
  }
  FinalizeArgs f{};
  f.x0 = a.x0;
  f.coef = a.coef;
  f.partial_keys = a.partial_keys;
  f.partial_feas = a.partial_feas;
  f.records = fused.records;
  f.regenerate = true;
  f.controls_only = fused.controls_only;
  f.centre = smp.centre;
  f.u_ref = smp.u_ref;
  f.u_extra = smp.u_extra;
  f.centre_stride = smp.centre_stride;
  f.spec = smp.spec;
  f.blocks_per_problem = static_cast<int>(gridDim.x);
  f.P = a.P;
  f.N = a.N;
  f.n = a.n;
  f.index_offset = a.index_offset;
  f.w = a.w;
  finalize_problem<MODE, 1>(f, p, s_finalize);
  signal_done();
}

template <int MODE>
__global__ void __launch_bounds__(kWave) rollout_sampled_kernel(const RolloutArgs a, const SampleArgs smp,
                                                                const FusedFinalize fused, const int rollout_lds_floats,
                                                                const int uniform_lds_floats) {
  extern __shared__ __attribute__((aligned(16))) float s_fused[];
  const int p = blockIdx.y;
  const bool traced = fused.trace != nullptr;
  rollout_sampled_body<MODE>(a, smp, s_fused, uniform_lds_floats, traced, rollout_lds_floats,
                             fused.trace + (static_cast<size_t>(p) * gridDim.x + blockIdx.x) * fused.trace_pitch);
  fused_tail<MODE>(a, smp, fused, traced, s_fused + rollout_lds_floats);
}

constexpr int kPairChunk = 7;
constexpr int kPairValues = 2;

__global__ void __launch_bounds__(2 * kWave) rollout_sampled_pair_kernel(const RolloutArgs a, const SampleArgs smp,
                                                                         const FusedFinalize fused,
                                                                         const int uniform_lds_floats,
                                                                         const int exchange_lds_floats) {
  extern __shared__ __attribute__((aligned(16))) float s_fused[];
  float* s_trace = s_fused;
  float* s_row = s_fused + uniform_lds_floats;
  const int p = blockIdx.y;
  const int lane = threadIdx.x & (kWave - 1);
  const bool consumer = threadIdx.x < kWave;
  const int n = a.n;
  float* s_centre = s_row + n * kCoefS;
  float* s_ref = s_centre + 2 * n;
  float* s_extra = s_ref + 2 * n;
  float* s_weight = s_extra + 2 * n;
  float* s_exchange = s_fused + exchange_lds_floats + lane;
  constexpr int kStepFloats = kPairValues * kWave, kBufferFloats = kPairChunk * kStepFloats;
  const int c = blockIdx.x * kWave + lane;
  const bool active = c < a.N;
  const Weights w = a.w;

  if (!consumer) {
    const SampleSpec sp = smp.spec;
    const float* __restrict__ centre = smp.centre + static_cast<size_t>(p) * smp.centre_stride;
    const float* __restrict__ ref = (smp.u_ref != nullptr) ? smp.u_ref + static_cast<size_t>(p) * n * 2 : nullptr;
    const float* __restrict__ extra = holds_candidate_2(a, smp) ? smp.u_extra + static_cast<size_t>(p) * n * 2 : nullptr;
    const float* __restrict__ knot_weight = sp.segments;
    const bool chained = smp.prev_keys != nullptr;
    constexpr int kPairs = (kStagedSteps + kWave - 1) / kWave;
    f32x2 g_centre[kPairs], g_ref[kPairs], g_extra[kPairs], g_weight[kPairs];
#pragma unroll
    for (int q = 0; q < kPairs; ++q) {
      const int j = min(lane + q * kWave, n - 1);
      if (!chained) g_centre[q] = reinterpret_cast<const f32x2*>(centre)[j];
      if (ref != nullptr) g_ref[q] = reinterpret_cast<const f32x2*>(ref)[j];
      if (extra != nullptr) g_extra[q] = reinterpret_cast<const f32x2*>(extra)[j];
      g_weight[q] = reinterpret_cast<const f32x2*>(knot_weight)[j];
    }
    int64_t prev_key[kChainBlocks / kWave];
    if (chained) {
#pragma unroll
      for (int q = 0; q < kChainBlocks / kWave; ++q)
// ... 71 lines not shown
        if (++in_chunk == kPairChunk || i == n - 1) {
          __syncthreads();
          in_chunk = 0;
          buffer ^= 1;
          out = s_exchange + buffer * kBufferFloats;
        }
      }
    }
    return;
  }

  {
    const float* __restrict__ coef = a.coef + static_cast<size_t>(p) * n * kCoefS;
    for (int q = lane; q < n * (kCoefS / 4); q += kWave)
      reinterpret_cast<f32x4*>(s_row)[q] = reinterpret_cast<const f32x4*>(coef)[q];
  }
  const float* __restrict__ x0 = a.x0 + p * 3;
  StateS st{x0[0], x0[1], x0[2], 0.0f, 0.0f};
  __syncthreads();
  struct StepInputs {
    float v, k;
    f32x4 lo, hi;
    float last;
  };
  auto inputs_of = [&](const float* in, int i) {
    StepInputs s;
    s.v = in[0];
    s.k = in[kWave];
    const float* t = s_row + i * kCoefS;
    s.lo = *reinterpret_cast<const f32x4*>(t);
    s.hi = *reinterpret_cast<const f32x4*>(t + 4);
    s.last = t[8];
    return s;
  };
  auto advance = [&](int i, const StepInputs& in) {
    const float row[9] = {in.lo[0], in.lo[1], in.lo[2], in.lo[3], in.hi[0], in.hi[1], in.hi[2], in.hi[3], in.last};
    step_spatial<float>(st, row, in.v, in.k, w);
    s_trace[(2 * n + 3 * i) * kWave + lane] = st.ey;
    s_trace[(2 * n + 3 * i + 1) * kWave + lane] = st.ep;
    s_trace[(2 * n + 3 * i + 2) * kWave + lane] = st.t;
  };
  for (int first = 0, buffer = 0; first < n; first += kPairChunk, buffer ^= 1) {
    __syncthreads();
    const float* in = s_exchange + buffer * kBufferFloats;
    if (first + kPairChunk <= n) {
      StepInputs steps[kPairChunk];
#pragma unroll
      for (int j = 0; j < kPairChunk; ++j) steps[j] = inputs_of(in + j * kStepFloats, first + j);
#pragma unroll
      for (int j = 0; j < kPairChunk; ++j) advance(first + j, steps[j]);
    } else {
      for (int j = 0; first + j < n; ++j) advance(first + j, inputs_of(in + j * kStepFloats, first + j));
    }
  }
  const float cost = finish_spatial<float>(st, w);
  s_trace[(5 * n) * kWave + lane] = st.V;
  s_trace[(5 * n + 1) * kWave + lane] = cost;
  if (active && a.costs != nullptr) a.costs[static_cast<size_t>(p) * a.N + c] = cost;
  const int64_t own_key = active ? pack_key(cost, static_cast<uint32_t>(a.index_offset + c)) : kKeyMax;
  int nfeas = (active && st.V == 0.0f) ? 1 : 0;
  int best_lane;
  const int64_t key = wave_min_key_by_lane(own_key, best_lane);
  nfeas = wave_sum_int(nfeas);
  {
    __syncthreads();
    float* trace_out = fused.trace + (static_cast<size_t>(p) * gridDim.x + blockIdx.x) * fused.trace_pitch;
    for (int e = lane; e < 5 * n + 2; e += kWave) publish(&trace_out[e], s_trace[e * kWave + best_lane]);
  }
  if (lane == 0) {
    const size_t slot = static_cast<size_t>(p) * gridDim.x + blockIdx.x;
    publish(&a.partial_keys[slot], key);
    publish(&a.partial_feas[slot], nfeas);
  }
  fused_tail<0>(a, smp, fused, true, nullptr);
}

#ifndef ACMPC_QUAD_CHUNK
#define ACMPC_QUAD_CHUNK 7
#endif
constexpr int kQuadChunk = ACMPC_QUAD_CHUNK;

constexpr int kQuadWaves = 4;

__global__ void __launch_bounds__(kQuadWaves * kWave) rollout_sampled_quad_kernel(const RolloutArgs a, const SampleArgs smp,
                                                                         const FusedFinalize fused, const int uniform_lds_floats,
                                                                         const int normals_lds_floats) {
  extern __shared__ __attribute__((aligned(16))) float s_fused[];
  float* s_trace = s_fused;
  float* s_row = s_fused + uniform_lds_floats;
  const int p = blockIdx.y;
  const int lane = threadIdx.x & (kWave - 1);
  const int wave = __builtin_amdgcn_readfirstlane(static_cast<int>(threadIdx.x) / kWave);
  const int n = a.n;
  float* s_centre = s_row + n * kCoefS;
  float* s_ref = s_centre + 2 * n;
  float* s_extra = s_ref + 2 * n;
  float* s_weight = s_extra + 2 * n;
  float* s_z = s_fused + normals_lds_floats;
  float* s_j = s_z + 2 * kKnots * kWave;
  const int c = blockIdx.x * kWave + lane;
  const bool active = c < a.N;
  const Weights w = a.w;
  const SampleSpec sp = smp.spec;
  const uint32_t gidx = static_cast<uint32_t>(a.index_offset + c);
  const int chunks = (n + kQuadChunk - 1) / kQuadChunk;
  float* col = s_trace + lane;
  const float* __restrict__ x0 = a.x0 + p * 3;

  auto draw_quarter = [&](auto quarter) {
    constexpr int Q = decltype(quarter)::value;
    float z[kKnots][2] = {};
    draw_normals<Q, Q + 1>(sp, gidx, static_cast<uint32_t>(p), z);
#pragma unroll
    for (int knot = 2 * Q; knot < 2 * Q + 2; ++knot) {
      s_z[(2 * knot) * kWave + lane] = z[knot][0];
      s_z[(2 * knot + 1) * kWave + lane] = z[knot][1];
    }
  };
  static_assert(kKnots == 8, "four Philox calls per candidate, one per wave");

  auto produce_controls = [&](const float (&z)[kKnots][2], const int parity) {
    const bool use_extra = (gidx == 2u) && (smp.u_extra != nullptr);
    const bool use_ref = ((gidx == 1u) && (smp.u_ref != nullptr)) || use_extra;
    const f32x2* s_alt = reinterpret_cast<const f32x2*>(use_extra ? s_extra : s_ref);
    const float amp = use_ref ? 0.0f : candidate_amplitude(gidx);
    struct Operands {
      f32x2 centre, ref;
      float weight;
    };
    auto request = [&](int i) {
      Operands o;
      o.centre = reinterpret_cast<const f32x2*>(s_centre)[i];
      o.ref = s_alt[i];
      o.weight = s_weight[i];
      return o;
    };
    Operands now = request(parity);
    int in_chunk = 0;
#pragma unroll
    for (int knot = 0; knot < kKnots - 1; ++knot) {
      for (int i = sp.knot_begin[knot]; i < sp.knot_begin[knot + 1]; ++i) {
        if ((i & 1) == parity) {
          const Operands next = request(i + 2);
          float v, k;
          blend_control(sp, amp, now.weight, use_ref ? now.ref[0] : now.centre[0], use_ref ? now.ref[1] : now.centre[1],
                        z[knot][0], z[knot][1], z[knot + 1][0], z[knot + 1][1], v, k);
          col[(2 * i) * kWave] = v;
          col[(2 * i + 1) * kWave] = k;
          now = next;
        }
        if (++in_chunk == kQuadChunk || i == n - 1) {
          __syncthreads();
          in_chunk = 0;
        }
      }
    }
  };

  if (wave == 3) {
    draw_quarter(std::integral_constant<int, 3>{});
    __syncthreads();
    float z[kKnots][2];
#pragma unroll
    for (int knot = 0; knot < kKnots; ++knot) {
      z[knot][0] = s_z[(2 * knot) * kWave + lane];
      z[knot][1] = s_z[(2 * knot + 1) * kWave + lane];
    }
    produce_controls(z, 1);
    return;
  }
  if (wave == 2) {
    const float* __restrict__ centre = smp.centre + static_cast<size_t>(p) * smp.centre_stride;
    const float* __restrict__ ref = (smp.u_ref != nullptr) ? smp.u_ref + static_cast<size_t>(p) * n * 2 : nullptr;
    const float* __restrict__ extra = holds_candidate_2(a, smp) ? smp.u_extra + static_cast<size_t>(p) * n * 2 : nullptr;
    const float* __restrict__ knot_weight = sp.segments;
    const bool chained = smp.prev_keys != nullptr;
    constexpr int kPairs = (kStagedSteps + kWave - 1) / kWave;
    f32x2 g_centre[kPairs], g_ref[kPairs], g_extra[kPairs], g_weight[kPairs];
#pragma unroll
    for (int q = 0; q < kPairs; ++q) {
      const int j = min(lane + q * kWave, n - 1);
      if (!chained) g_centre[q] = reinterpret_cast<const f32x2*>(centre)[j];
      if (ref != nullptr) g_ref[q] = reinterpret_cast<const f32x2*>(ref)[j];
      if (extra != nullptr) g_extra[q] = reinterpret_cast<const f32x2*>(extra)[j];
      g_weight[q] = reinterpret_cast<const f32x2*>(knot_weight)[j];
    }
    int64_t prev_key[kChainBlocks / kWave];
    if (chained) {
#pragma unroll
      for (int q = 0; q < kChainBlocks / kWave; ++q)
        prev_key[q] = smp.prev_keys[static_cast<size_t>(p) * smp.prev_blocks + min(lane + q * kWave, smp.prev_blocks - 1)];
    }
    draw_quarter(std::integral_constant<int, 2>{});
    if (chained) {
      int64_t best = kKeyMax;
#pragma unroll
      for (int q = 0; q < kChainBlocks / kWave; ++q) {
        const int64_t kb = (lane + q * kWave < smp.prev_blocks) ? prev_key[q] : kKeyMax;
        best = (kb < best) ? kb : best;
      }
      const int64_t winner = wave_min_key(best);
      const int block = static_cast<int>(static_cast<int64_t>(static_cast<uint32_t>(winner & 0xffffffffLL)) - a.index_offset) / kWave;
      centre = smp.prev_trace + (static_cast<size_t>(p) * smp.prev_blocks + block) * smp.prev_pitch;
#pragma unroll
      for (int q = 0; q < kPairs; ++q) g_centre[q] = reinterpret_cast<const f32x2*>(centre)[min(lane + q * kWave, n - 1)];
    }
#pragma unroll
    for (int q = 0; q < kPairs; ++q) {
      const int j = lane + q * kWave;
      if (j < n) {
        reinterpret_cast<f32x2*>(s_centre)[j] = g_centre[q];
        reinterpret_cast<f32x2*>(s_ref)[j] = (ref != nullptr) ? g_ref[q] : g_centre[q];
        if (extra != nullptr) reinterpret_cast<f32x2*>(s_extra)[j] = g_extra[q];
        s_weight[j] = g_weight[q][1];
      }
    }
    for (int j = lane + kPairs * kWave; j < n; j += kWave) {
      const f32x2 cj = reinterpret_cast<const f32x2*>(centre)[j];
      reinterpret_cast<f32x2*>(s_centre)[j] = cj;
      reinterpret_cast<f32x2*>(s_ref)[j] = (ref != nullptr) ? reinterpret_cast<const f32x2*>(ref)[j] : cj;
      if (extra != nullptr) reinterpret_cast<f32x2*>(s_extra)[j] = reinterpret_cast<const f32x2*>(extra)[j];
      s_weight[j] = knot_weight[2 * j + 1];
    }
    __syncthreads();
    float z[kKnots][2];
#pragma unroll
    for (int knot = 0; knot < kKnots; ++knot) {
      z[knot][0] = s_z[(2 * knot) * kWave + lane];
      z[knot][1] = s_z[(2 * knot + 1) * kWave + lane];
    }
    produce_controls(z, 0);
    return;
  }

  {
    const float* __restrict__ coef = a.coef + static_cast<size_t>(p) * n * kCoefS;
    for (int q = threadIdx.x; q < n * (kCoefS / 4); q += 2 * kWave)
      reinterpret_cast<f32x4*>(s_row)[q] = reinterpret_cast<const f32x4*>(coef)[q];
  }
  if (wave == 0) draw_quarter(std::integral_constant<int, 0>{});
  if (wave == 1) draw_quarter(std::integral_constant<int, 1>{});
  __syncthreads();

  if (wave == 1) {
    StateS st{x0[0], x0[1], x0[2], 0.0f, 0.0f};
    auto roll = [&](int i, float v, float k, const f32x4& lo, const f32x4& hi) {
      const float cr[7] = {lo[0], lo[1], lo[2], lo[3], hi[0], hi[1], hi[2]};
      step_spatial_cost(st, cr, v, k, w);
      col[(2 * n + 3 * i) * kWave] = st.ey;
      col[(2 * n + 3 * i + 1) * kWave] = st.ep;
      col[(2 * n + 3 * i + 2) * kWave] = st.t;
    };
    __syncthreads();
    for (int t = 1; t <= chunks; ++t) {
      const int first = (t - 1) * kQuadChunk;
      if (first + kQuadChunk <= n) {
        float v[kQuadChunk], k[kQuadChunk];
        f32x4 lo[kQuadChunk], hi[kQuadChunk];
#pragma unroll
        for (int q = 0; q < kQuadChunk; ++q) {
          v[q] = col[(2 * (first + q)) * kWave];
          k[q] = col[(2 * (first + q) + 1) * kWave];
          lo[q] = *reinterpret_cast<const f32x4*>(s_row + (first + q) * kCoefS);
          hi[q] = *reinterpret_cast<const f32x4*>(s_row + (first + q) * kCoefS + 4);
        }
#pragma unroll
        for (int q = 0; q < kQuadChunk; ++q) roll(first + q, v[q], k[q], lo[q], hi[q]);
      } else {
        for (int i = first; i < n; ++i)
          roll(i, col[(2 * i) * kWave], col[(2 * i + 1) * kWave], *reinterpret_cast<const f32x4*>(s_row + i * kCoefS),
               *reinterpret_cast<const f32x4*>(s_row + i * kCoefS + 4));
      }
      if (t == chunks) s_j[lane] = st.J;
      __syncthreads();
    }
    return;
  }

  StateS st{x0[0], x0[1], x0[2], 0.0f, 0.0f};
  __syncthreads();
  __syncthreads();
  {
    auto account = [&](float v, float k, float ey_lo, float ey_hi, float ey_after, float t_after) {
      st.V = st.V + hinge2<float>(w.ulo0 - v, v - w.uhi0);
      st.V = st.V + hinge2<float>(w.ulo1 - k, k - w.uhi1);
      st.V = st.V + hinge2<float>(ey_lo - ey_after, ey_after - ey_hi);
      const float tv = vmax(w.tmin - t_after, 0.0f);
      st.V = st.V + tv * tv;
    };
    for (int t = 2; t <= chunks + 1; ++t) {
      const int first = (t - 2) * kQuadChunk;
      if (first + kQuadChunk <= n) {
        float v[kQuadChunk], k[kQuadChunk], ey[kQuadChunk], tt[kQuadChunk], lo[kQuadChunk], hi[kQuadChunk];
#pragma unroll
        for (int q = 0; q < kQuadChunk; ++q) {
          const int i = first + q;
          v[q] = col[(2 * i) * kWave];
          k[q] = col[(2 * i + 1) * kWave];
          ey[q] = col[(2 * n + 3 * i) * kWave];
          tt[q] = col[(2 * n + 3 * i + 2) * kWave];
          lo[q] = s_row[i * kCoefS + 7];
          hi[q] = s_row[i * kCoefS + 8];
        }
#pragma unroll
        for (int q = 0; q < kQuadChunk; ++q) account(v[q], k[q], lo[q], hi[q], ey[q], tt[q]);
      } else {
        for (int i = first; i < n; ++i)
          account(col[(2 * i) * kWave], col[(2 * i + 1) * kWave], s_row[i * kCoefS + 7], s_row[i * kCoefS + 8],
                  col[(2 * n + 3 * i) * kWave], col[(2 * n + 3 * i + 2) * kWave]);
      }
      __syncthreads();
    }
    st.ey = col[(2 * n + 3 * (n - 1)) * kWave];
    st.ep = col[(2 * n + 3 * (n - 1) + 1) * kWave];
    st.t = col[(2 * n + 3 * (n - 1) + 2) * kWave];
  }
  st.J = s_j[lane];
  const float cost = finish_spatial<float>(st, w);
  s_trace[(5 * n) * kWave + lane] = st.V;
  s_trace[(5 * n + 1) * kWave + lane] = cost;
  if (active && a.costs != nullptr) a.costs[static_cast<size_t>(p) * a.N + c] = cost;
  const int64_t own_key = active ? pack_key(cost, static_cast<uint32_t>(a.index_offset + c)) : kKeyMax;
  int best_lane;
  const int64_t key = wave_min_key_by_lane(own_key, best_lane);
  const int nfeas = wave_sum_int((active && st.V == 0.0f) ? 1 : 0);
  {
    __syncthreads();
    float* trace_out = fused.trace + (static_cast<size_t>(p) * gridDim.x + blockIdx.x) * fused.trace_pitch;
    for (int e = lane; e < 5 * n + 2; e += kWave) publish(&trace_out[e], s_trace[e * kWave + best_lane]);
  }
  if (lane == 0) {
    const size_t slot = static_cast<size_t>(p) * gridDim.x + blockIdx.x;
    publish(&a.partial_keys[slot], key);
    publish(&a.partial_feas[slot], nfeas);
  }
  fused_tail<0>(a, smp, fused, true, nullptr);
}

#ifndef ACMPC_TRIO_CHUNK
#define ACMPC_TRIO_CHUNK 3
#endif
constexpr int kTrioChunk = ACMPC_TRIO_CHUNK;

__global__ void __launch_bounds__(3 * kWave) rollout_sampled_trio_kernel(const RolloutArgs a, const SampleArgs smp,
                                                                         const FusedFinalize fused, const int trace_lds_floats,
                                                                         const int uniform_lds_floats,
                                                                         const int index_lds_floats) {
  extern __shared__ __attribute__((aligned(16))) float s_fused[];
  const int p = blockIdx.y;
  const int lane = threadIdx.x & (kWave - 1);
  const int wave = __builtin_amdgcn_readfirstlane(static_cast<int>(threadIdx.x) / kWave);
  const int n = a.n;
  const Weights w = a.w;
  float* s_wp = s_fused;
  float* s_abc = s_wp + n * kCoefT;
  float* s_trace = s_fused + trace_lds_floats;
  float* s_centre = s_fused + uniform_lds_floats;
  float* s_ref = s_centre + 2 * n;
  float* s_extra = s_ref + 2 * n;
  float* s_weight = s_extra + 2 * n;
  unsigned short* s_index = reinterpret_cast<unsigned short*>(s_fused + index_lds_floats);
  const int c = blockIdx.x * kWave + lane;
  const bool active = c < a.N;
  const float* __restrict__ coef = a.coef + static_cast<size_t>(p) * n * kCoefT;
  const float* __restrict__ x0 = a.x0 + p * 3;
  const int chunks = (n + kTrioChunk - 1) / kTrioChunk;
  float* col = s_trace + lane;

  if (wave == 2) {
    const SampleSpec sp = smp.spec;
    const float* __restrict__ centre = smp.centre + static_cast<size_t>(p) * smp.centre_stride;
    const float* __restrict__ ref = (smp.u_ref != nullptr) ? smp.u_ref + static_cast<size_t>(p) * n * 2 : nullptr;
    const float* __restrict__ extra = holds_candidate_2(a, smp) ? smp.u_extra + static_cast<size_t>(p) * n * 2 : nullptr;
    const float* __restrict__ knot_weight = sp.segments;
    const bool chained = smp.prev_keys != nullptr;
    constexpr int kPairs = (kStagedSteps + kWave - 1) / kWave;
    f32x2 g_centre[kPairs], g_ref[kPairs], g_extra[kPairs], g_weight[kPairs];
#pragma unroll
    for (int q = 0; q < kPairs; ++q) {
      const int j = min(lane + q * kWave, n - 1);
      if (!chained) g_centre[q] = reinterpret_cast<const f32x2*>(centre)[j];
      if (ref != nullptr) g_ref[q] = reinterpret_cast<const f32x2*>(ref)[j];
      if (extra != nullptr) g_extra[q] = reinterpret_cast<const f32x2*>(extra)[j];
      g_weight[q] = reinterpret_cast<const f32x2*>(knot_weight)[j];
    }
    int64_t prev_key[kChainBlocks / kWave];
    if (chained) {
#pragma unroll
      for (int q = 0; q < kChainBlocks / kWave; ++q)
        prev_key[q] = smp.prev_keys[static_cast<size_t>(p) * smp.prev_blocks + min(lane + q * kWave, smp.prev_blocks - 1)];
    }
    float z[kKnots][2] = {};
    const uint32_t gidx = static_cast<uint32_t>(a.index_offset + c);
    draw_normals<0, kKnots / 4>(sp, gidx, static_cast<uint32_t>(p), z);
    if (chained) {
      int64_t best = kKeyMax;
#pragma unroll
      for (int q = 0; q < kChainBlocks / kWave; ++q) {
        const int64_t kb = (lane + q * kWave < smp.prev_blocks) ? prev_key[q] : kKeyMax;
        best = (kb < best) ? kb : best;
      }
      const int64_t winner = wave_min_key(best);
      const int block = static_cast<int>(static_cast<int64_t>(static_cast<uint32_t>(winner & 0xffffffffLL)) - a.index_offset) / kWave;
      centre = smp.prev_trace + (static_cast<size_t>(p) * smp.prev_blocks + block) * smp.prev_pitch;
#pragma unroll
      for (int q = 0; q < kPairs; ++q) g_centre[q] = reinterpret_cast<const f32x2*>(centre)[min(lane + q * kWave, n - 1)];
    }
    draw_normals<kKnots / 4, kKnots / 2>(sp, gidx, static_cast<uint32_t>(p), z);
#pragma unroll
    for (int q = 0; q < kPairs; ++q) {
      const int j = lane + q * kWave;
      if (j < n) {
        reinterpret_cast<f32x2*>(s_centre)[j] = g_centre[q];
        reinterpret_cast<f32x2*>(s_ref)[j] = (ref != nullptr) ? g_ref[q] : g_centre[q];
        if (extra != nullptr) reinterpret_cast<f32x2*>(s_extra)[j] = g_extra[q];
        s_weight[j] = g_weight[q][1];
      }
    }
    for (int j = lane + kPairs * kWave; j < n; j += kWave) {
// ... 935 lines not shown
        hipLaunchKernelGGL((finalize_waves_kernel<0>), waves_grid, dim3(kFinalizeWaves * kWave), waves_lds, s, args);
      } else {
        hipLaunchKernelGGL((finalize_waves_kernel<1>), waves_grid, dim3(kFinalizeWaves * kWave), waves_lds, s, args);
      }
      return hipGetLastError();
    }
    const dim3 groups_grid((args.P + kGroupProblems - 1) / kGroupProblems);
    const size_t groups_lds = group_finalize_floats(args.n) * sizeof(float);
    if (layout == 0) {
      hipLaunchKernelGGL((finalize_groups_kernel<0>), groups_grid, dim3(kWave), groups_lds, s, args);
    } else {
      hipLaunchKernelGGL((finalize_groups_kernel<1>), groups_grid, dim3(kWave), groups_lds, s, args);
    }
    return hipGetLastError();
  }
  const dim3 grid(args.P), block(kWave);
  const size_t rec_floats = static_cast<size_t>(4 + 2 * args.n + 3 * (args.n + 1));
  const size_t lds = (((rec_floats + 3) & ~static_cast<size_t>(3)) + (mode == 1 ? args.n * (kCoefT + kKeyStride) : 0)) * sizeof(float);
  if (mode == 0 && layout == 0) {
    hipLaunchKernelGGL((finalize_kernel<0, 0>), grid, block, lds, s, args);
  } else if (mode == 0 && layout == 1) {
    hipLaunchKernelGGL((finalize_kernel<0, 1>), grid, block, lds, s, args);
  } else if (mode == 1 && layout == 0) {
    hipLaunchKernelGGL((finalize_kernel<1, 0>), grid, block, lds, s, args);
  } else if (mode == 1 && layout == 1) {
    hipLaunchKernelGGL((finalize_kernel<1, 1>), grid, block, lds, s, args);
  } else {
    return hipErrorInvalidValue;
  }
  return hipGetLastError();
}

hipError_t launch_sample(int layout, const SampleArgs& args, hipStream_t s) {
  clear_stale_error();
  const dim3 grid((args.N + 255) / 256, args.P);
  const size_t sample_lds = (((static_cast<size_t>(args.n) + 3) & ~static_cast<size_t>(3)) + 2 * args.n) * sizeof(float);
  if (layout == 0) {
    hipLaunchKernelGGL((sample_kernel<0>), grid, dim3(256), sample_lds, s, args);
  } else if (layout == 1) {
    hipLaunchKernelGGL((sample_kernel<1>), grid, dim3(256), sample_lds, s, args);
  } else {
    return hipErrorInvalidValue;
  }
  return hipGetLastError();
}

namespace {
size_t sampled_rollout_floats(int mode, int n) {
  return (mode == 1) ? ((static_cast<size_t>(n) * (kCoefT + kKeyStride) + 3) & ~static_cast<size_t>(3)) : 0;
}
size_t sampled_uniform_floats(int mode, int n) {
  return static_cast<size_t>(n) * ((mode == 0 ? kCoefS : 0) + 7) + 4;
}
size_t sampled_finalize_floats(int mode, int n) {
  const size_t rec_floats = static_cast<size_t>(4 + 2 * n + 3 * (n + 1));
  return ((rec_floats + 3) & ~static_cast<size_t>(3)) + (mode == 1 ? static_cast<size_t>(n) * (kCoefT + kKeyStride) : 0);
}
}

bool fused_finalize_fits(int mode, int n) {
  return (sampled_rollout_floats(mode, n) + sampled_finalize_floats(mode, n) + sampled_uniform_floats(mode, n)) *
             sizeof(float) <= 64 * 1024;
}

int trace_floats(int n) { return 5 * n + 2; }

bool trio_frames_fit(int n) {
  if (n < kVerifiedWindow) return false;
  const size_t tables = ((static_cast<size_t>(n) * (kCoefT + kKeyStride) + 3) & ~static_cast<size_t>(3)) +
                        static_cast<size_t>(verified_frame_floats(n));
  const size_t trace = static_cast<size_t>(trace_floats(n)) * kWave;
  const size_t uniform = (static_cast<size_t>(n) * 7 + 4 + 3) & ~static_cast<size_t>(3);
  const size_t index = (static_cast<size_t>(n) * kWave / 2 + 3) & ~static_cast<size_t>(3);
  return (tables + trace + uniform + index) * sizeof(float) <= 160u * 1024u;
}

bool traced_finalize_fits(int mode, int n) {
  return (sampled_rollout_floats(mode, n) + static_cast<size_t>(trace_floats(n)) * kWave +
          sampled_uniform_floats(mode, n)) * sizeof(float) <= 160 * 1024;
}

static hipError_t raise_lds_limit(const void* kernel, int which, size_t lds) {
  if (lds <= 64 * 1024) return hipSuccess;
  static bool raised[13][64] = {};
  int device = 0;
  hipError_t e = hipGetDevice(&device);
  if (e != hipSuccess) return e;
  if (device < 0 || device >= 64) return hipErrorInvalidDevice;
  if (!raised[which][device]) {
    e = hipFuncSetAttribute(kernel, hipFuncAttributeMaxDynamicSharedMemorySize, 160 * 1024);
    if (e != hipSuccess) return e;
    raised[which][device] = true;
  }
  return hipSuccess;
}

hipError_t launch_rollout_sampled(int mode, const RolloutArgs& rollout, const SampleArgs& sample,
                                  const FusedFinalize& fused, hipStream_t s, hipEvent_t e0, hipEvent_t e1,
                                  const LaunchOptions& opt) {
  clear_stale_error();
  const int n = rollout.n;
  const dim3 grid((rollout.N + kWave - 1) / kWave, rollout.P);
  const size_t rollout_floats = sampled_rollout_floats(mode, n);
  const bool traced = fused.trace != nullptr;
  const size_t finalize_floats = traced                     ? static_cast<size_t>(trace_floats(n)) * kWave
                                 : fused.tickets != nullptr ? sampled_finalize_floats(mode, n)
                                                            : 0;
  const size_t uniform_floats = sampled_uniform_floats(mode, n);
  const size_t lds = (rollout_floats + finalize_floats + uniform_floats) * sizeof(float);
  if (lds > 160u * 1024u) return hipErrorInvalidValue;
  const int uniform_offset = static_cast<int>(rollout_floats + finalize_floats);
  if (traced && fused.trace_pitch < trace_floats(n)) return hipErrorInvalidValue;
  const int offset = static_cast<int>(rollout_floats);
  if (mode != 0 && mode != 1) return hipErrorInvalidValue;
  {
    const hipError_t e = raise_lds_limit(mode == 0 ? reinterpret_cast<const void*>(&rollout_sampled_kernel<0>)
                                                   : reinterpret_cast<const void*>(&rollout_sampled_kernel<1>),
                                         mode, lds);
    if (e != hipSuccess) return e;
  }
  if (mode == 1 && traced && !opt.no_trio_rounds) {
    const size_t plain_tables = (static_cast<size_t>(n) * (kCoefT + kKeyStride) + 3) & ~static_cast<size_t>(3);
    const size_t trace = static_cast<size_t>(trace_floats(n)) * kWave;
    const size_t uniform = (static_cast<size_t>(n) * 7 + 4 + 3) & ~static_cast<size_t>(3);
    const size_t index = (static_cast<size_t>(n) * kWave / 2 + 3) & ~static_cast<size_t>(3);
    RolloutArgs rollout_trio = rollout;
    size_t tables = plain_tables + (rollout.nn_frames != nullptr ? static_cast<size_t>(verified_frame_floats(n)) : 0);
    if ((tables + trace + uniform + index) * sizeof(float) > 160u * 1024u) {
      rollout_trio.nn_frames = nullptr;
      tables = plain_tables;
    }
    const size_t trio_lds = (tables + trace + uniform + index) * sizeof(float);
    if (trio_lds <= 160u * 1024u) {
      hipError_t e = raise_lds_limit(reinterpret_cast<const void*>(&rollout_sampled_trio_kernel), 11, trio_lds);
      if (e != hipSuccess) return e;
      if (e0 != nullptr && e1 != nullptr) {
        hipExtLaunchKernelGGL(rollout_sampled_trio_kernel, grid, dim3(3 * kWave), static_cast<std::uint32_t>(trio_lds), s, e0,
                              e1, 0, rollout_trio, sample, fused, static_cast<int>(tables), static_cast<int>(tables + trace),
                              static_cast<int>(tables + trace + uniform));
      } else {
        hipLaunchKernelGGL(rollout_sampled_trio_kernel, grid, dim3(3 * kWave), trio_lds, s, rollout_trio, sample, fused,
                           static_cast<int>(tables), static_cast<int>(tables + trace),
                           static_cast<int>(tables + trace + uniform));
      }
      return hipGetLastError();
    }
  }
  if (mode == 0 && traced && !opt.no_quad_rounds && !opt.no_pair_rounds) {
    const size_t trace = static_cast<size_t>(trace_floats(n)) * kWave;
    const size_t uniform = (uniform_floats + 3) & ~static_cast<size_t>(3);
    const size_t quad_lds = (trace + uniform + static_cast<size_t>(2 * kKnots + 1) * kWave) * sizeof(float);
    if (quad_lds <= 160u * 1024u) {
      hipError_t e = raise_lds_limit(reinterpret_cast<const void*>(&rollout_sampled_quad_kernel), 12, quad_lds);
      if (e != hipSuccess) return e;
      if (e0 != nullptr && e1 != nullptr) {
        hipExtLaunchKernelGGL(rollout_sampled_quad_kernel, grid, dim3(kQuadWaves * kWave), static_cast<std::uint32_t>(quad_lds), s, e0,
                              e1, 0, rollout, sample, fused, static_cast<int>(trace), static_cast<int>(trace + uniform));
      } else {
        hipLaunchKernelGGL(rollout_sampled_quad_kernel, grid, dim3(kQuadWaves * kWave), quad_lds, s, rollout, sample, fused,
                           static_cast<int>(trace), static_cast<int>(trace + uniform));
      }
      return hipGetLastError();
    }
  }
  if (mode == 0 && traced && !opt.no_pair_rounds) {
    const size_t trace = static_cast<size_t>(trace_floats(n)) * kWave;
    const size_t exchange = static_cast<size_t>(2) * kPairChunk * kPairValues * kWave;
    const size_t pair_lds = (trace + uniform_floats + exchange) * sizeof(float);
    if (pair_lds <= 160u * 1024u) {
      hipError_t e = raise_lds_limit(reinterpret_cast<const void*>(&rollout_sampled_pair_kernel), 2, pair_lds);
      if (e != hipSuccess) return e;
      if (e0 != nullptr && e1 != nullptr) {
        hipExtLaunchKernelGGL(rollout_sampled_pair_kernel, grid, dim3(2 * kWave), static_cast<std::uint32_t>(pair_lds), s,
                              e0, e1, 0, rollout, sample, fused, static_cast<int>(trace),
                              static_cast<int>(trace + uniform_floats));
      } else {
        hipLaunchKernelGGL(rollout_sampled_pair_kernel, grid, dim3(2 * kWave), pair_lds, s, rollout, sample, fused,
                           static_cast<int>(trace), static_cast<int>(trace + uniform_floats));
      }
      return hipGetLastError();
    }
  }
  const bool timed = e0 != nullptr && e1 != nullptr;
  const std::uint32_t lds32 = static_cast<std::uint32_t>(lds);
// ... 115 lines not shown
```

ac-mpc_amd/csrc/acmpc_prologue.h:

```cpp
#pragma once
#include <hip/hip_runtime.h>
#include <stdint.h>

#include "acmpc_admm.h"

namespace acmpc {

struct TickHeader {
  double offset;
  double v_min, v_max, a_min, a_max, ay_max, ki_min, end_velocity;
  double qp_eps_abs, qp_eps_rel;
  double eps;
  int32_t horizon;
  int32_t localised;
  int32_t has_end_velocity;
  int32_t centre_is_reference;
  int32_t qp_max_iter, qp_check_every;
  uint32_t seed_lo, seed_hi;
  int32_t qp_method;
  int32_t reserved;
  int32_t use_map;
  int32_t map_index;
  double pose_x, pose_y;
  double lateral_offset;
};

struct MapWindowArgs {
  const TickHeader* header;
  const double* centre;
  int M;
  int count;
  int points;
  int H;
  double* coords;
  double* coords_out;
  int* first_out;
};

struct PrologueArgs {
  int header_by_value;
  TickHeader header_value;
  int path_by_value;
  double coords_value[3 * 64];
  float centre_value[2 * 64];
  const TickHeader* header;
  const double* coords;
  const float* centre_in;
  int temporal;
  float* x0;
  float* u_ref;
  float* coef;
  float* frames;
  float* centre;
  uint32_t* seed;
  double* table_out;
  int* status;
  double* warm_state;
  int warm_stride;
  int warm_capacity;
  double margin;
  double u_lo0, u_lo1, u_hi0, u_hi1;
  const double* map_centre;
  int map_M, map_count, map_points;
  const int* map_first;
  double* coords_out;
  int* index_out;
};

struct MapFrame {
  double x0, y0, c, sn;
};
__host__ __device__ inline MapFrame map_frame(const double* centre, int M, int first) {
  const double* w0 = centre + 2 * first;
  const double* w1 = centre + 2 * ((first + 1) % M);
  const double heading = atan2(w1[1] - w0[1], w1[0] - w0[0]);
  const double rot = 3.14159265358979323846 / 2.0 - heading;
  return MapFrame{w0[0], w0[1], cos(rot), sin(rot)};
}
__host__ __device__ inline void map_path_row(const double* centre, int M, int first, int count, int points, int H, int r,
                                             double lateral_offset, const MapFrame& f, double (&row)[3]) {
  const int stride = points / H;
  const double step = static_cast<double>(count - 1) / static_cast<double>(points - 1);
  const int q = r * stride;
  const double t = (q == points - 1) ? static_cast<double>(count - 1) : static_cast<double>(q) * step;
  int j = static_cast<int>(t);
  if (j > count - 2) j = count - 2;
  double local[2][2];
  for (int e = 0; e < 2; ++e) {
    const double* wp = centre + 2 * ((first + j + e) % M);
    const double dx = wp[0] - f.x0, dy = wp[1] - f.y0;
    local[e][0] = (dx * f.c + dy * (-f.sn)) - lateral_offset;
    local[e][1] = dx * f.sn + dy * f.c;
  }
  const double frac = t - static_cast<double>(j);
  const bool last = t >= static_cast<double>(count - 1);
  const double x = last ? local[1][0] : (local[1][0] - local[0][0]) * frac + local[0][0];
  const double y = last ? local[1][1] : (local[1][1] - local[0][1]) * frac + local[0][1];
  row[0] = static_cast<double>(static_cast<float>(x));
  row[1] = static_cast<double>(static_cast<float>(y));
  row[2] = (r == H - 1) ? 6.0 : 10.0 + static_cast<double>(r) * ((6.0 - 10.0) / static_cast<double>(H - 1));
}

constexpr int kInlinePathPoints = 64;
// ... 11 lines not shown
```

ac-mpc_amd/csrc/acmpc_prologue.hip:

```cpp
#include <hip/hip_runtime.h>

#include <type_traits>

#include "acmpc_admm.h"
#include "acmpc_frames.h"
#include "acmpc_prologue.h"

#pragma clang fp contract(off)

namespace acmpc {

#ifdef ACMPC_STAMPS
__device__ unsigned long long g_prologue_stamps[16];
#define ACMPC_PSTAMP(slot)                                                    \
  do {                                                                        \
    if (threadIdx.x == 0) g_prologue_stamps[(slot)] = wall_clock64();         \
  } while (0)
#else
#define ACMPC_PSTAMP(slot) \
  do {                     \
  } while (0)
#endif

namespace {

constexpr double kPi = 3.14159265358979323846;

__device__ __forceinline__ double wrap_angle(double a) {
  const double two_pi = 2.0 * kPi;
  double m = fmod(a + kPi, two_pi);
  if (m != 0.0 && (m < 0.0)) m += two_pi;
  return m - kPi;
}

struct WaveTeam {
  static constexpr int size = 64;
  __device__ __forceinline__ int rank() const { return static_cast<int>(threadIdx.x); }
  __device__ __forceinline__ void sync() const { __syncthreads(); }
  __device__ __forceinline__ double max(double v, double*) const {
#pragma unroll
    for (int m = 32; m >= 1; m >>= 1) {
      const double o = __shfl_xor(v, m, 64);
      v = o > v ? o : v;
    }
    return v;
  }
};

}

__device__ void tabulate_frames(const double* xr, const double* yr, double* gap_doubles, int n, int lane, float* out) {
  const WaveTeam team;
  constexpr int W = kVerifiedWindow;
  const int windows = n - W + 1;
  const double inf = __builtin_huge_val();
  auto at = [&](int mm, double& x, double& y) {
    x = xr[mm];
    y = yr[mm];
  };
  double wn = 0.0;
  bool finite = true;
  for (int i = lane; i < n; i += 64) {
    const double x = xr[i], y = yr[i];
    finite = finite && (fabs(x) < inf) && (fabs(y) < inf);
    const double norm = sqrt(x * x + y * y);
    wn = (norm > wn) ? norm : wn;
  }
  wn = team.max(wn, nullptr);
  finite = __ballot(!finite) == 0ull;
  float largest_gap2 = 0.0f;
  for (int i = lane; i + 1 < n; i += 64) {
    const float gap2 = frames::squared_gap(static_cast<float>(xr[i + 1]), static_cast<float>(yr[i + 1]),
                                           static_cast<float>(xr[i]), static_cast<float>(yr[i]));
    largest_gap2 = (gap2 > largest_gap2) ? gap2 : largest_gap2;
  }
#pragma unroll
  for (int m = 32; m >= 1; m >>= 1) {
    const float other = __shfl_xor(largest_gap2, m, 64);
    largest_gap2 = (other > largest_gap2) ? other : largest_gap2;
  }
  const int near0 = __builtin_amdgcn_readfirstlane(frames::near_first(largest_gap2));
  constexpr int kSlots = (kPrologueMaxSteps + 63) / 64;
  const int slots = (n + 63) / 64;
  float own_x[kSlots], own_y[kSlots];
#pragma unroll
  for (int r = 0; r < kSlots; ++r) {
    const int q = min(lane + 64 * r, n - 1);
    own_x[r] = static_cast<float>(xr[q]);
    own_y[r] = static_cast<float>(yr[q]);
  }
  auto lane_value = [](float v, int src) {
    return __builtin_bit_cast(float, __builtin_amdgcn_readlane(__builtin_bit_cast(int, v), src));
  };
  auto waypoint = [&](int mm, float& x, float& y) {
    const int src = mm & 63;
    x = lane_value((mm < 64) ? own_x[0] : own_x[kSlots - 1], src);
    y = lane_value((mm < 64) ? own_y[0] : own_y[kSlots - 1], src);
  };
  static_assert(kSlots <= 2, "waypoint(): two slots per lane");
  float* gap = reinterpret_cast<float*>(gap_doubles);
  const int nowhere = n * W;
  const float finf = __builtin_inff();
  float r2[kSlots];
#pragma unroll
  for (int q = 0; q < kSlots; ++q) r2[q] = finf;
  auto sweep = [&](auto slots_tag, auto pass_tag) {
    constexpr int kLive = decltype(slots_tag)::value;
    constexpr bool kAhead = decltype(pass_tag)::value == 0;
    float running[kLive];
#pragma unroll
    for (int r = 0; r < kLive; ++r) running[r] = finf;
    const int count = n - 1 - near0;
    for (int it = 0, mm = kAhead ? n - 1 : 0; it < count; ++it, mm += kAhead ? -1 : 1) {
      float xm, ym;
      waypoint(mm, xm, ym);
#pragma unroll
      for (int r = 0; r < kLive; ++r) {
        const int q = lane + 64 * r;
        const int j = kAhead ? q + near0 + W - mm : q - near0 - 1 - mm;
        const int applies = static_cast<int>(q < n) & static_cast<int>(kAhead ? mm > q + near0
                                                                              : mm < q - near0);
        const float d2 = frames::squared_gap(xm, ym, own_x[r], own_y[r]);
        running[r] = ((applies & static_cast<int>(d2 < running[r])) != 0) ? d2 : running[r];
        const int kept = applies & static_cast<int>(j >= 0) & static_cast<int>(j < W);
        gap[(kept != 0) ? q * W + j : nowhere] = running[r];
      }
    }
  };
  auto sweep_either = [&](auto pass_tag) {
    if (slots == 1) {
      sweep(std::integral_constant<int, 1>{}, pass_tag);
    } else {
      sweep(std::integral_constant<int, kSlots>{}, pass_tag);
    }
  };
  for (int pass = 0; pass < 2; ++pass) {
    for (int e = lane; e < n * W; e += 64) gap[e] = finf;
    team.sync();
    if (pass == 0) {
      sweep_either(std::integral_constant<int, 0>{});
    } else {
      sweep_either(std::integral_constant<int, 1>{});
    }
    team.sync();
#pragma unroll
    for (int q = 0; q < kSlots; ++q) {
      const int lo = lane + 64 * q;
      if (lo < windows) {
        float g[W];
#pragma unroll
        for (int j = 0; j < W; ++j) g[j] = gap[(lo + j) * W + j];
#pragma unroll
        for (int j = 0; j < W; ++j) r2[q] = (g[j] < r2[q]) ? g[j] : r2[q];
      }
    }
    team.sync();
  }
  frames::Geometry geometry[kSlots];
  double slab_max = 0.0;
#pragma unroll
  for (int q = 0; q < kSlots; ++q) {
    const int lo = lane + 64 * q;
    geometry[q].usable = false;
    const bool mine = lo < windows;
    double R = (mine && finite) ? frames::far_from_squared(r2[q]) : inf;
    const int near = (mine && finite) ? frames::choose_near(at, n, lo, near0, R) : near0;
    const bool first_choice_stands = __ballot(mine && near != near0) == 0ull;
    if (first_choice_stands && near0 == 16) {
      if (mine) geometry[q] = frames::window_geometry<16>(at, n, lo, finite, near, R);
    } else if (first_choice_stands && near0 == 32) {
      if (mine) geometry[q] = frames::window_geometry<32>(at, n, lo, finite, near, R);
    } else if (mine) {
      geometry[q] = frames::window_geometry<0>(at, n, lo, finite, near, R);
    }
    const double slab = geometry[q].aA - geometry[q].aB;
    if (mine && geometry[q].usable) slab_max = (slab > slab_max) ? slab : slab_max;
  }
  slab_max = team.max(slab_max, nullptr);
  const frames::Scale scale = frames::path_scale(wn, slab_max);
#pragma unroll
  for (int q = 0; q < kSlots; ++q) {
    const int lo = lane + 64 * q;
    if (lo < windows) frames::frame_row(geometry[q], scale, out + static_cast<size_t>(kFrameStride) * lo);
  }
}

__global__ void __launch_bounds__(64) prologue_kernel(const PrologueArgs a) {
  extern __shared__ __attribute__((aligned(16))) double s_mem[];
  const TickHeader h = (a.header_by_value != 0) ? a.header_value : *a.header;
  ACMPC_PSTAMP(0);
  const int lane = static_cast<int>(threadIdx.x);
  const int H = __builtin_amdgcn_readfirstlane(h.horizon);
  const int n = H - 1;
  const int m = n - 1;
  if (blockIdx.x == 1) {
    if (a.frames == nullptr || n < kVerifiedWindow) return;
    double* xr = s_mem;
    double* yr = s_mem + n;
    if (h.use_map != 0) {
      int first = (h.map_index < 0) ? a.map_first[0] : h.map_index;
      first = ((first % a.map_M) + a.map_M) % a.map_M;
      const MapFrame frame = map_frame(a.map_centre, a.map_M, first);
      for (int r = lane; r < n; r += 64) {
        double row[3];
        map_path_row(a.map_centre, a.map_M, first, a.map_count, a.map_points, H, r, h.lateral_offset, frame, row);
        xr[r] = static_cast<double>(static_cast<float>(row[0]));
        yr[r] = static_cast<double>(static_cast<float>(row[1]));
      }
    } else {
      for (int r = lane; r < n; r += 64) {
        xr[r] = static_cast<double>(static_cast<float>((a.path_by_value != 0) ? a.coords_value[3 * r] : a.coords[3 * r]));
        yr[r] = static_cast<double>(static_cast<float>((a.path_by_value != 0) ? a.coords_value[3 * r + 1] : a.coords[3 * r + 1]));
      }
    }
    __syncthreads();
    {
      const float ox = static_cast<float>(xr[0]), oy = static_cast<float>(yr[0]);
      __syncthreads();
      for (int r = lane; r < n; r += 64) {
        xr[r] = static_cast<double>(static_cast<float>(xr[r]) - ox);
        yr[r] = static_cast<double>(static_cast<float>(yr[r]) - oy);
      }
      __syncthreads();
    }
    tabulate_frames(xr, yr, s_mem + 2 * n, n, lane, a.frames);
    return;
  }
  double* table = s_mem;
  double *tx = table, *ty = table + n, *tpsi = table + 2 * n, *tkappa = table + 3 * n, *tds = table + 4 * n,
         *twidth = table + 5 * n, *tv = table + 6 * n;
  double* v_hi = table + 7 * n;
  double* seg = v_hi + n;
  double* qv = seg + (n + 1);
  double* qy = qv + n;
  admm::Workspace ws;
  ws.bind(qy + 2 * n, n);
  double* s_coords = qy + 2 * n + admm::workspace_doubles(n);
  const double* __restrict__ coords = a.coords;
  const WaveTeam team;
  constexpr int kPerLane = (kPrologueMaxSteps + 63) / 64;
  float centre_in_v[kPerLane], centre_in_k[kPerLane];
  double warm_v[kPerLane], warm_y[2 * kPerLane];
  double* state = a.warm_state + static_cast<size_t>(h.localised != 0 ? 1 : 0) * a.warm_stride;
  const double warm_flag = state[0], warm_n = state[1];
#pragma unroll
  for (int q = 0; q < kPerLane; ++q) {
    const int i = min(lane + 64 * q, n - 1);
    if (a.path_by_value != 0) {
      centre_in_v[q] = (h.centre_is_reference != 0) ? 0.0f : a.centre_value[2 * min(i, kInlinePathPoints - 1)];
      centre_in_k[q] = (h.centre_is_reference != 0) ? 0.0f : a.centre_value[2 * min(i, kInlinePathPoints - 1) + 1];
    } else {
      centre_in_v[q] = (h.centre_is_reference != 0) ? 0.0f : a.centre_in[2 * i];
      centre_in_k[q] = (h.centre_is_reference != 0) ? 0.0f : a.centre_in[2 * i + 1];
    }
    warm_v[q] = (a.warm_capacity >= n) ? state[2 + i] : 0.0;
  }
#pragma unroll
  for (int q = 0; q < 2 * kPerLane; ++q)
    warm_y[q] = (a.warm_capacity >= n) ? state[2 + n + min(lane + 64 * q, 2 * n - 2)] : 0.0;
  if (h.use_map != 0) {
    int first = (h.map_index < 0) ? a.map_first[0] : h.map_index;
    first = ((first % a.map_M) + a.map_M) % a.map_M;
    const MapFrame frame = map_frame(a.map_centre, a.map_M, first);
    for (int r = lane; r < H; r += 64) {
      double row[3];
      map_path_row(a.map_centre, a.map_M, first, a.map_count, a.map_points, H, r, h.lateral_offset, frame, row);
      for (int e = 0; e < 3; ++e) {
        s_coords[3 * r + e] = row[e];
        a.coords_out[3 * r + e] = row[e];
      }
    }
    if (lane == 0) a.index_out[0] = first;
    team.sync();
    coords = s_coords;
  } else if (a.path_by_value != 0) {
    for (int r = lane; r < 3 * H; r += 64) s_coords[r] = a.coords_value[r];
    team.sync();
    coords = s_coords;
  }

  ACMPC_PSTAMP(1);
  for (int i = lane; i <= n; i += 64) {
    const double* here = coords + 3 * ((i == n) ? 0 : i);
    const double* from = coords + 3 * ((i == n) ? H - 1 : i);
    const double* to = coords + 3 * ((i == n) ? 0 : i + 1);
    const double ax = to[0] - from[0], ay = to[1] - from[1];
    seg[i] = atan2(ay, ax);
    if (i < n) {
      tx[i] = here[0];
      ty[i] = here[1];
      tds[i] = sqrt(ax * ax + ay * ay);
      twidth[i] = to[2];
    }
  }
  team.sync();
  for (int i = lane; i < n; i += 64) {
    const double psi = seg[i];
    const double behind = seg[(i == 0) ? n : i - 1];
    tpsi[i] = psi;
    tkappa[i] = wrap_angle(psi - behind) / (tds[i] + h.eps) + h.eps;
  }
  team.sync();
  if (lane == 0) tkappa[0] = tkappa[1];
  team.sync();

  ACMPC_PSTAMP(2);
  for (int i = lane; i < n; i += 64) {
    double c;
    if (h.localised != 0) {
      c = h.v_max;
    } else {
      const double curvature = fabs(tkappa[i]);
      c = sqrt(h.ay_max / (curvature + 1e-12));
      if (curvature < h.ki_min) c = h.v_max;
      c = fmin(c, h.v_max);
      c = fmax(h.v_min, c);
      c = c + 2.0;
      if (h.has_end_velocity != 0 && i == n - 1) c = h.end_velocity;
    }
    v_hi[i] = c;
  }
  const bool warm = warm_flag == 1.0 && warm_n == static_cast<double>(n) && a.warm_capacity >= n;
  if (warm) {
#pragma unroll
    for (int q = 0; q < kPerLane; ++q)
      if (lane + 64 * q < n) qv[lane + 64 * q] = warm_v[q];
#pragma unroll
    for (int q = 0; q < 2 * kPerLane; ++q)
      if (lane + 64 * q < 2 * n - 1) qy[lane + 64 * q] = warm_y[q];
  }
  team.sync();
  ACMPC_PSTAMP(3);
  const admm::Settings settings{h.a_min, h.a_max, h.v_min, h.qp_max_iter, h.qp_check_every > 0 ? h.qp_check_every : 10,
                                h.qp_eps_abs, h.qp_eps_rel};
  int iterations = 0;
  const bool swept = h.qp_method == 0 && admm::exact_profile(team, ws, v_hi, tds, n, settings, qv, qy, ws.ex[0]);
  const int status = swept ? 0 : admm::solve(team, ws, v_hi, tds, n, settings, qv, qy, warm ? 1 : 0, &iterations);
  ACMPC_PSTAMP(4);
  if (status == 0 && a.warm_capacity >= n) {
    for (int i = lane; i < n; i += 64) state[2 + i] = qv[i];
    for (int i = lane; i < 2 * n - 1; i += 64) state[2 + n + i] = qy[i];
    if (lane == 0) {
      state[0] = 1.0;
      state[1] = static_cast<double>(n);
    }
  }
  for (int i = lane; i < n; i += 64) tv[i] = (status == 0) ? qv[i] : 0.0;
  team.sync();

  ACMPC_PSTAMP(5);
  if (lane == 0) {
    const double wx = tx[0], wy = ty[0], wpsi = tpsi[0];
    const double lateral = cos(wpsi) * (0.0 - wy) - sin(wpsi) * (h.offset - wx);
    if (a.temporal != 0) {
      a.x0[0] = static_cast<float>(h.offset);
      a.x0[1] = 0.0f;
      a.x0[2] = static_cast<float>(kPi / 2.0);
    } else {
      a.x0[0] = static_cast<float>(lateral);
      a.x0[1] = static_cast<float>(wrap_angle(kPi / 2.0 - wpsi));
      a.x0[2] = 0.0f;
    }
    a.status[0] = status;
    a.status[1] = iterations;
    a.seed[0] = h.seed_lo;
    a.seed[1] = h.seed_hi;
  }
#pragma unroll
  for (int q = 0; q < kPerLane; ++q) {
    const int i = lane + 64 * q;
    if (i >= n) break;
    const double v = tv[i], ds = tds[i], kappa = tkappa[i], width = twidth[i];
    const double vds = v * ds + 1e-12;
    if (a.temporal != 0) {
      float* out = a.coef + static_cast<size_t>(i) * 8;
      const double psi = tpsi[i];
      out[0] = static_cast<float>(tx[i]);
      out[1] = static_cast<float>(ty[i]);
      out[2] = static_cast<float>(cos(psi));
      out[3] = static_cast<float>(sin(psi));
      out[4] = static_cast<float>(psi);
      out[5] = static_cast<float>(kappa);
      out[6] = static_cast<float>(v);
      out[7] = static_cast<float>(width / 2.0 - a.margin);
    } else {
      float* out = a.coef + static_cast<size_t>(i) * 12;
      out[0] = static_cast<float>(ds);
      out[1] = static_cast<float>(-(kappa * kappa) * ds);
      out[2] = static_cast<float>(-kappa / vds);
      out[3] = static_cast<float>(-1.0 / (v * v * ds + 1e-12));
      out[4] = static_cast<float>(1.0 / vds);
      out[5] = static_cast<float>(v);
      out[6] = static_cast<float>(kappa);
      out[7] = static_cast<float>(-width / 2.0 + a.margin);
      out[8] = static_cast<float>(width / 2.0 - a.margin);
      out[9] = 0.0f;
      out[10] = 0.0f;
      out[11] = 0.0f;
    }
    const double uv = fmin(fmax(v, a.u_lo0), a.u_hi0);
    const double uk = fmin(fmax(kappa, a.u_lo1), a.u_hi1);
    a.u_ref[2 * i] = static_cast<float>(uv);
    a.u_ref[2 * i + 1] = static_cast<float>(uk);
    a.centre[2 * i] = (h.centre_is_reference != 0) ? static_cast<float>(uv) : centre_in_v[q];
    a.centre[2 * i + 1] = (h.centre_is_reference != 0) ? static_cast<float>(uk) : centre_in_k[q];
  }
  ACMPC_PSTAMP(6);
  for (int e = lane; e < 7 * n; e += 64) a.table_out[e] = table[e];
  ACMPC_PSTAMP(7);
  (void)m;
}

__global__ void __launch_bounds__(256) map_window_kernel(const MapWindowArgs a) {
  __shared__ double s_d[4];
  __shared__ int s_i[4];
  __shared__ int s_first;
  const int tid = static_cast<int>(threadIdx.x);
  const TickHeader h = *a.header;
  int first = h.map_index;
  if (first < 0) {
    double best = __builtin_inf();
    int best_i = 0x7fffffff;
    for (int m = tid; m < a.M; m += 256) {
      const double dx = h.pose_x - a.centre[2 * m], dy = h.pose_y - a.centre[2 * m + 1];
      const double d = dx * dx + dy * dy;
      if (d < best) {
        best = d;
        best_i = m;
      }
    }
#pragma unroll
    for (int mask = 32; mask >= 1; mask >>= 1) {
      const double od = __shfl_xor(best, mask, 64);
      const int oi = __shfl_xor(best_i, mask, 64);
      if (od < best || (od == best && oi < best_i)) {
        best = od;
        best_i = oi;
      }
    }
    if ((tid & 63) == 0) {
      s_d[tid >> 6] = best;
      s_i[tid >> 6] = best_i;
    }
    __syncthreads();
    if (tid == 0) {
      for (int q = 1; q < 4; ++q)
        if (s_d[q] < best || (s_d[q] == best && s_i[q] < best_i)) {
          best = s_d[q];
          best_i = s_i[q];
        }
      s_first = best_i;
    }
    __syncthreads();
    first = s_first;
  }
  first = ((first % a.M) + a.M) % a.M;
  const MapFrame frame = map_frame(a.centre, a.M, first);
  for (int r = tid; r < a.H; r += 256) {
    double row[3];
    map_path_row(a.centre, a.M, first, a.count, a.points, a.H, r, h.lateral_offset, frame, row);
    for (int e = 0; e < 3; ++e) {
      if (a.coords != nullptr) a.coords[3 * r + e] = row[e];
      if (a.coords_out != nullptr) a.coords_out[3 * r + e] = row[e];
    }
  }
  if (tid == 0 && a.first_out != nullptr) a.first_out[0] = first;
}

#ifdef ACMPC_STAMPS
extern "C" int acmpc_debug_prologue_stamps(unsigned long long* out) {
  return static_cast<int>(hipMemcpyFromSymbol(out, HIP_SYMBOL(g_prologue_stamps), sizeof(unsigned long long) * 16));
}
#endif

hipError_t launch_map_window(const MapWindowArgs& args, hipStream_t s) {
  (void)hipGetLastError();
  hipLaunchKernelGGL(map_window_kernel, dim3(1), dim3(256), 0, s, args);
  return hipGetLastError();
}

size_t prologue_lds_bytes(int n) {
  return static_cast<size_t>(7 * n + n + (n + 1) + n + 2 * n + admm::workspace_doubles(n) + 3 * (n + 1)) * sizeof(double);
}

hipError_t launch_prologue(const PrologueArgs& args, int n, hipStream_t s) {
  (void)hipGetLastError();
  hipLaunchKernelGGL(prologue_kernel, dim3(args.frames != nullptr ? 2 : 1), dim3(64), prologue_lds_bytes(n), s, args);
  return hipGetLastError();
}

__global__ void __launch_bounds__(64) admm_kernel(const double* v_hi_in, const double* ds_in, int n, admm::Settings s,
                                                  double* v, double* y, int warm, int* out) {
  extern __shared__ __attribute__((aligned(16))) double s_mem[];
  double* v_hi = s_mem;
  double* ds = v_hi + n;
  double* qv = ds + n;
  double* qy = qv + n;
  admm::Workspace ws;
  ws.bind(qy + 2 * n, n);
  const int lane = static_cast<int>(threadIdx.x);
  for (int i = lane; i < n; i += 64) {
    v_hi[i] = v_hi_in[i];
    ds[i] = ds_in[i];
    qv[i] = v[i];
  }
  for (int i = lane; i < 2 * n - 1; i += 64) qy[i] = y[i];
  __syncthreads();
  int iterations = 0;
  const int status = admm::solve(WaveTeam{}, ws, v_hi, ds, n, s, qv, qy, warm, &iterations);
  for (int i = lane; i < n; i += 64) v[i] = qv[i];
  for (int i = lane; i < 2 * n - 1; i += 64) y[i] = qy[i];
  if (lane == 0) {
    out[0] = status;
    out[1] = iterations;
  }
}

hipError_t launch_admm(const double* d_v_hi, const double* d_ds, int n, const admm::Settings& s, double* d_v, double* d_y,
                       int warm, int* d_out, hipStream_t stream) {
  (void)hipGetLastError();
  const size_t lds = static_cast<size_t>(5 * n + admm::workspace_doubles(n)) * sizeof(double);
  hipLaunchKernelGGL(admm_kernel, dim3(1), dim3(64), lds, stream, d_v_hi, d_ds, n, s, d_v, d_y, warm, d_out);
  return hipGetLastError();
}

}
```

Before: 16.19 billion candidate-trajectories/s.

## Fuse the tick prologue into the first quad rollout round via an extra wave

Adds a path where the prologue (path tables, speed-profile QP, coefficient rows) runs inside an extra wave of the first quad rollout kernel. Every workgroup recomputes it into LDS, and one writer block publishes it to global memory. The separate prologue kernel launch and its dependency are removed from the tick path. Warm-start state is now double-buffered so that concurrent readers and the single writer do not race. The trade-off is redundant prologue work in every workgroup and more LDS and registers in the rollout kernel. The path only applies to the tick API under specific conditions, so the batched throughput benchmark may not use it.

```diff
diff --git a/ac-mpc_amd/acmpc_amd/_build.py b/ac-mpc_amd/acmpc_amd/_build.py
--- a/ac-mpc_amd/acmpc_amd/_build.py
+++ b/ac-mpc_amd/acmpc_amd/_build.py
@@ -10,7 +10,7 @@
 LIB_PATH = os.path.join(LIB_DIR, "libacmpc_hip.so")
 SOURCES = ("acmpc_kernels.hip", "acmpc_kernels_temporal.hip", "acmpc_capi.hip", "acmpc_prologue.hip", "acmpc_pf.hip",
            "acmpc_speed_profile.cpp", "acmpc_host_path.cpp", "acmpc_dynamic.hip", "acmpc_dynamic_terms.hip", "acmpc_identify.hip")
-HEADERS = ("acmpc_kernels.h", "acmpc_device.h", "acmpc_dynamic.h", "acmpc_identify.h", "acmpc_frames.h", "acmpc_admm.h", "acmpc_prologue.h", "acmpc_lq.h", "acmpc_lq_box.h",
+HEADERS = ("acmpc_kernels.h", "acmpc_device.h", "acmpc_dynamic.h", "acmpc_identify.h", "acmpc_frames.h", "acmpc_admm.h", "acmpc_prologue.h", "acmpc_prologue_body.h", "acmpc_lq.h", "acmpc_lq_box.h",
            os.path.join("..", "..", "include", "acmpc.h"))
 
 HIPCC_FLAGS = ("--offload-arch=gfx950", "-O3", "-std=c++17", "-fPIC", "-ffp-contract=off", "-Wall", "-Wextra")
diff --git a/ac-mpc_amd/csrc/acmpc_capi.hip b/ac-mpc_amd/csrc/acmpc_capi.hip
--- a/ac-mpc_amd/csrc/acmpc_capi.hip
+++ b/ac-mpc_amd/csrc/acmpc_capi.hip
@@ -119,6 +119,7 @@
   double* d_coords = nullptr;
   double* d_warm = nullptr;
   int warm_stride = 0;
+  int warm_copy[2] = {0, 0};
   int tick_last_n = 0;
 
   std::vector<double> h_tables;
@@ -142,6 +143,7 @@
   struct Switches {
     bool no_verified_search = false, no_solo = false, no_fused_finalize = false, no_traced_finalize = false,
          no_chained_rounds = false, no_chained_stream = false, no_graph = false, no_fused_sampling = false, tick_graph = false, tick_no_flag = false, tick_no_inline_path = false, no_zero_copy = false,
+         no_fused_prologue = false,
          tailed_rollout = false,
          dynamic_matrix_rounds = false;
   } sw;
@@ -743,7 +745,7 @@
     "ACMPC_SHAPE", "ACMPC_T_PACK", "ACMPC_NO_TILE", "ACMPC_TILE_ROWS", "ACMPC_TILE_TABLE", "ACMPC_NO_TRIO_ROUNDS",
     "ACMPC_NO_QUAD_ROUNDS", "ACMPC_NO_PAIR_ROUNDS", "ACMPC_SOLO_REGISTERS", "ACMPC_SOLO_SPLIT", "ACMPC_NO_VERIFIED_SEARCH",
     "ACMPC_NO_SOLO", "ACMPC_NO_FUSED_FINALIZE", "ACMPC_NO_TRACED_FINALIZE", "ACMPC_NO_CHAINED_ROUNDS", "ACMPC_NO_GRAPH",
-    "ACMPC_NO_FUSED_SAMPLING", "ACMPC_TICK_GRAPH", "ACMPC_TICK_NO_FLAG", "ACMPC_TICK_NO_INLINE_PATH", "ACMPC_NO_ZERO_COPY", "ACMPC_TAILED_ROLLOUT", "ACMPC_NO_GROUP_FINALIZE", "ACMPC_FINALIZE_WAVES",
+    "ACMPC_NO_FUSED_SAMPLING", "ACMPC_TICK_GRAPH", "ACMPC_TICK_NO_FLAG", "ACMPC_TICK_NO_INLINE_PATH", "ACMPC_NO_FUSED_PROLOGUE", "ACMPC_NO_ZERO_COPY", "ACMPC_TAILED_ROLLOUT", "ACMPC_NO_GROUP_FINALIZE", "ACMPC_FINALIZE_WAVES",
     "ACMPC_NO_CHAINED_STREAM", "ACMPC_LQ_BOX_ITERATIONS", "ACMPC_START_CLOCKS", "ACMPC_DYNAMIC_MATRIX_ROUNDS",
     "ACMPC_CONFORMANT_SYNC"};
 
@@ -781,6 +783,7 @@
   if (key == "ACMPC_TICK_GRAPH") { w.tick_graph = on; return true; }
   if (key == "ACMPC_TICK_NO_FLAG") { w.tick_no_flag = on; return true; }
   if (key == "ACMPC_TICK_NO_INLINE_PATH") { w.tick_no_inline_path = on; return true; }
+  if (key == "ACMPC_NO_FUSED_PROLOGUE") { w.no_fused_prologue = on; return true; }
   if (key == "ACMPC_NO_ZERO_COPY") { w.no_zero_copy = on; return true; }
   if (key == "ACMPC_TAILED_ROLLOUT") { w.tailed_rollout = on; return true; }
   if (key == "ACMPC_START_CLOCKS") { c->want_start_clocks = on; return true; }
@@ -1781,7 +1784,8 @@
 
 int enqueue_rounds(acmpc_ctx* c, const OptInputs& in, int P, int N, int n, int rounds, double sigma_v, double sigma_k,
                    double shrink, uint64_t seed, const uint32_t* d_seed, hipStream_t s, bool fused,
-                   float* final_records = nullptr, unsigned* done = nullptr, unsigned done_value = 0) {
+                   float* final_records = nullptr, unsigned* done = nullptr, unsigned done_value = 0,
+                   const acmpc::PrologueArgs* tick = nullptr) {
   const bool has_uref = in.uref != nullptr;
   const bool fused_finalize = use_fused_finalize(c, n);
   const int layout = ACMPC_LAYOUT_STEP_MAJOR;
@@ -1794,6 +1798,7 @@
     const float* d_extra = nullptr;
     if (r + 1 == rounds && in.extra != nullptr && (!in.before_last || in.before_last())) d_extra = in.extra;
     if (!fused) {
+      if (tick != nullptr) return fail(c, ACMPC_ESTATE, "the prologue inside the first round needs the fused rounds");
       const bool softmin = c->prm.centre_update == 1;
       const bool mean_round = softmin && r > 0;
       if (mean_round)
@@ -1875,8 +1880,9 @@
                                     (last && final_records != nullptr) ? final_records : c->d_records, !last,
                                     traced ? d_trace : nullptr, acmpc::trace_floats(n),
                                     last ? done : nullptr, done_value};
-      ACMPC_HIP(c, acmpc::launch_rollout_sampled(c->prm.mode, ra, sa, ff, s, e0, e1, c->opt));
+      ACMPC_HIP(c, acmpc::launch_rollout_sampled(c->prm.mode, ra, sa, ff, s, e0, e1, c->opt, r == 0 ? tick : nullptr));
     } else {
+      if (tick != nullptr) return fail(c, ACMPC_ESTATE, "the prologue inside the first round needs the fused finalize");
       ACMPC_HIP(c, acmpc::launch_rollout_sampled(c->prm.mode, ra, sa, acmpc::FusedFinalize{nullptr, nullptr, false, nullptr, 0, nullptr, 0}, s, e0, e1, c->opt));
       Regenerate regen{d_c, stride, d_ref, sa.spec, d_extra};
       rc = finalize(c, nullptr, nullptr, in.x0, nullptr, P, N, n, layout, 0, c->d_records, (N + 63) / 64, s, &regen,
@@ -2113,7 +2119,8 @@
   std::memset(c->h_tick_out, 0, TickOutLayout(n_cap).total);
   ACMPC_HIP(c, alloc_once(&c->d_coords, static_cast<size_t>(n_cap + 1) * 3 * sizeof(double)));
   c->warm_stride = 2 + 3 * n_cap;
-  const size_t warm_bytes = static_cast<size_t>(2) * c->warm_stride * sizeof(double);
+  const size_t warm_bytes = static_cast<size_t>(4) * c->warm_stride * sizeof(double);
+  c->warm_copy[0] = c->warm_copy[1] = 0;
   ACMPC_HIP(c, alloc_once(&c->d_warm, warm_bytes));
   ACMPC_HIP(c, hipMemset(c->d_warm, 0, warm_bytes));
   ACMPC_HIP(c, hipStreamSynchronize(nullptr));
@@ -2252,12 +2259,17 @@
     const double pose[3] = {lq_offset, 0.0, M_PI / 2.0};
     return lq_plan_into(c, c->tick_lq_table.data(), n, pose, c->h_lq, true);
   };
+  const bool inline_inputs = from_map ? (t->centre_is_reference != 0 || n <= acmpc::kInlinePathPoints)
+                                      : (H <= acmpc::kInlinePathPoints && !c->sw.tick_no_inline_path);
+  const bool fuse_prologue = !temporal && !use_graph && !c->sw.no_fused_prologue && direct &&
+                             use_traced_finalize(c, 1, N, n) && acmpc::quad_prologue_fits(n, c->opt) && inline_inputs &&
+                             !(t->rounds == 1 && lq_on);
   const bool flagged = direct && !use_graph && !c->sw.tick_no_flag;
   unsigned* done_flag = reinterpret_cast<unsigned*>(c->h_tick_out + out.done);
   const unsigned done_value = ++c->tick_sequence;
   auto enqueue = [&](hipStream_t q, int* rc_rounds) -> hipError_t {
     hipError_t e = (from_map && t->map_index < 0) ? acmpc::launch_map_window(ma, q) : hipSuccess;
-    if (e == hipSuccess) e = acmpc::launch_prologue(pa, n, q);
+    if (e == hipSuccess && !fuse_prologue) e = acmpc::launch_prologue(pa, n, q);
     if (e != hipSuccess) return e;
     OptInputs oi{pa.x0, pa.centre, pa.u_ref, pa.coef, pa.frames};
     if (lq_on) {
@@ -2267,7 +2279,7 @@
     *rc_rounds = enqueue_rounds(c, oi, 1, N, n, t->rounds, t->sigma[0], t->sigma[1], t->shrink,
                                 use_graph ? 0 : t->seed, use_graph ? pa.seed : nullptr, q, true,
                                 direct ? reinterpret_cast<float*>(c->h_tick_out + out.record) : nullptr,
-                                flagged ? done_flag : nullptr, done_value);
+                                flagged ? done_flag : nullptr, done_value, fuse_prologue ? &pa : nullptr);
     if (*rc_rounds == ACMPC_OK && !direct)
       e = hipMemcpyAsync(c->h_tick_out + out.record, c->d_records, static_cast<size_t>(rec_floats) * sizeof(float),
                          hipMemcpyDeviceToHost, q);
@@ -2340,6 +2352,7 @@
   h->qp_max_iter = t->qp_max_iter;
   h->qp_check_every = t->qp_check_every;
   h->qp_method = t->qp_method;
+  h->warm_copy = c->warm_copy[t->localised != 0 ? 1 : 0];
   h->seed_lo = static_cast<uint32_t>(t->seed);
   h->seed_hi = static_cast<uint32_t>(t->seed >> 32);
   h->use_map = from_map ? 1 : 0;
@@ -2364,6 +2377,10 @@
       pa.path_by_value = 1;
       std::memcpy(pa.coords_value, coords, static_cast<size_t>(H) * 3 * sizeof(double));
       if (centre != nullptr) std::memcpy(pa.centre_value, centre, static_cast<size_t>(n) * 2 * sizeof(float));
+    } else if (fuse_prologue) {
+      pa.path_by_value = 1;
+      if (centre != nullptr && t->centre_is_reference == 0)
+        std::memcpy(pa.centre_value, centre, static_cast<size_t>(n) * 2 * sizeof(float));
     }
     int rc_rounds = ACMPC_OK;
     const hipError_t e = enqueue(s, &rc_rounds);
@@ -2395,6 +2412,7 @@
   std::memcpy(record, rec, static_cast<size_t>(rec_floats) * sizeof(float));
   std::memcpy(table, c->h_tick_out + out.table, static_cast<size_t>(7) * n * sizeof(double));
   const int* status = reinterpret_cast<const int*>(c->h_tick_out + out.status);
+  if (status[0] == 0 && pa.warm_capacity >= n) c->warm_copy[t->localised != 0 ? 1 : 0] ^= 1;
   const float* ru = rec + ACMPC_REC_HEADER;
   const float* rx = ru + 2 * n;
   double biggest = 0.0;
diff --git a/ac-mpc_amd/csrc/acmpc_kernels.h b/ac-mpc_amd/csrc/acmpc_kernels.h
--- a/ac-mpc_amd/csrc/acmpc_kernels.h
+++ b/ac-mpc_amd/csrc/acmpc_kernels.h
@@ -3,6 +3,7 @@
 #include <stdint.h>
 
 #include "acmpc_device.h"
+#include "acmpc_prologue.h"
 
 namespace acmpc {
 
@@ -133,7 +134,9 @@
 
 hipError_t launch_rollout_sampled(int mode, const RolloutArgs& rollout, const SampleArgs& sample,
                                   const FusedFinalize& fused, hipStream_t s, hipEvent_t start = nullptr,
-                                  hipEvent_t stop = nullptr, const LaunchOptions& opt = LaunchOptions());
+                                  hipEvent_t stop = nullptr, const LaunchOptions& opt = LaunchOptions(),
+                                  const PrologueArgs* tick = nullptr);
+bool quad_prologue_fits(int n, const LaunchOptions& opt = LaunchOptions());
 bool solo_fits(int P, int N, int n, int layout, const LaunchOptions& opt = LaunchOptions());
 int solo_trace_floats(int n);
 hipError_t launch_rollout_solo(int layout, const RolloutArgs& args, const FusedFinalize& fused, hipStream_t s,
diff --git a/ac-mpc_amd/csrc/acmpc_kernels.hip b/ac-mpc_amd/csrc/acmpc_kernels.hip
--- a/ac-mpc_amd/csrc/acmpc_kernels.hip
+++ b/ac-mpc_amd/csrc/acmpc_kernels.hip
@@ -1,4 +1,5 @@
 #include "acmpc_kernels.h"
+#include "acmpc_prologue_body.h"
 
 #include <hip/hip_ext.h>
 
@@ -1175,7 +1176,8 @@
   rollout_block<0, LAYOUT, CPT, BLOCK, PACK, false>(a, smem, y);
 }
 
-__device__ __forceinline__ void finalize_from_trace(const RolloutArgs& a, const FusedFinalize& fused, const int p) {
+__device__ __forceinline__ void finalize_from_trace(const RolloutArgs& a, const FusedFinalize& fused, const int p,
+                                                    const float* local_x0 = nullptr) {
   const int lane = threadIdx.x;
   const int n = a.n;
   const int blocks = static_cast<int>(gridDim.x);
@@ -1221,7 +1223,10 @@
         src = (e < 4 + 2 * n + 3) ? x0 + (e - (4 + 2 * n)) : src;
         src = (e < 4 + 2 * n) ? trace + (e - 4) : src;
         src = (e < 4) ? trace + 5 * n + (1 - min(e, 1)) : src;
+        const bool start_state = e >= 4 + 2 * n && e < 4 + 2 * n + 3;
+        if (local_x0 != nullptr && start_state) src = trace;
         value[q] = observe(src);
+        if (local_x0 != nullptr && start_state) value[q] = local_x0[e - (4 + 2 * n)];
       }
     }
 #pragma unroll
@@ -1277,7 +1282,7 @@
 
 template <int MODE>
 __device__ __forceinline__ void fused_tail(const RolloutArgs& a, const SampleArgs& smp, const FusedFinalize& fused,
-                                           const bool traced, float* s_finalize) {
+                                           const bool traced, float* s_finalize, const float* local_x0 = nullptr) {
   const int p = blockIdx.y;
   if (fused.tickets == nullptr) return;
   if (!last_workgroup_of_problem(fused.tickets + static_cast<size_t>(p) * (kTicketGroups + 1) * kTicketStride, kTicketGroups)) return;
@@ -1287,7 +1292,7 @@
     if (threadIdx.x == 0) __hip_atomic_store(fused.done, fused.done_value, __ATOMIC_RELAXED, __HIP_MEMORY_SCOPE_SYSTEM);
   };
   if (traced) {
-    finalize_from_trace(a, fused, p);
+    finalize_from_trace(a, fused, p, local_x0);
     signal_done();
     return;
   }
@@ -1525,10 +1530,10 @@
 
 constexpr int kQuadWaves = 4;
 
-__global__ void __launch_bounds__(kQuadWaves * kWave) rollout_sampled_quad_kernel(const RolloutArgs a, const SampleArgs smp,
-                                                                         const FusedFinalize fused, const int uniform_lds_floats,
-                                                                         const int normals_lds_floats) {
-  extern __shared__ __attribute__((aligned(16))) float s_fused[];
+template <bool PROLOGUE>
+__device__ __forceinline__ void quad_round(const RolloutArgs& a, const SampleArgs& smp, const FusedFinalize& fused,
+                                           const int uniform_lds_floats, const int normals_lds_floats, float* s_fused,
+                                           const PrologueArgs* tick) {
   float* s_trace = s_fused;
   float* s_row = s_fused + uniform_lds_floats;
   const int p = blockIdx.y;
@@ -1541,6 +1546,22 @@
   float* s_weight = s_extra + 2 * n;
   float* s_z = s_fused + normals_lds_floats;
   float* s_j = s_z + 2 * kKnots * kWave;
+  float* s_x0 = s_j + kWave;
+  if constexpr (PROLOGUE) {
+    if (wave == kQuadWaves) {
+      prologue::LocalRows rows;
+      rows.x0 = s_x0;
+      rows.coef = s_row;
+      rows.u_ref = s_ref;
+      rows.centre = s_centre;
+      const bool writer = blockIdx.x == 0 && blockIdx.y == 0;
+      prologue::tables(*tick, tick->header_value, prologue::WaveTeamOf<false>{}, reinterpret_cast<double*>(s_trace), rows,
+                       writer);
+      if (writer && fused.done != nullptr) __threadfence_system();
+      __syncthreads();
+      return;
+    }
+  }
   const int c = blockIdx.x * kWave + lane;
   const bool active = c < a.N;
   const Weights w = a.w;
@@ -1548,7 +1569,7 @@
   const uint32_t gidx = static_cast<uint32_t>(a.index_offset + c);
   const int chunks = (n + kQuadChunk - 1) / kQuadChunk;
   float* col = s_trace + lane;
-  const float* __restrict__ x0 = a.x0 + p * 3;
+  const float* __restrict__ x0 = PROLOGUE ? s_x0 : a.x0 + p * 3;
 
   auto draw_quarter = [&](auto quarter) {
     constexpr int Q = decltype(quarter)::value;
@@ -1623,8 +1644,8 @@
 #pragma unroll
     for (int q = 0; q < kPairs; ++q) {
       const int j = min(lane + q * kWave, n - 1);
-      if (!chained) g_centre[q] = reinterpret_cast<const f32x2*>(centre)[j];
-      if (ref != nullptr) g_ref[q] = reinterpret_cast<const f32x2*>(ref)[j];
+      if (!PROLOGUE && !chained) g_centre[q] = reinterpret_cast<const f32x2*>(centre)[j];
+      if (!PROLOGUE && ref != nullptr) g_ref[q] = reinterpret_cast<const f32x2*>(ref)[j];
       if (extra != nullptr) g_extra[q] = reinterpret_cast<const f32x2*>(extra)[j];
       g_weight[q] = reinterpret_cast<const f32x2*>(knot_weight)[j];
     }
@@ -1635,7 +1656,7 @@
         prev_key[q] = smp.prev_keys[static_cast<size_t>(p) * smp.prev_blocks + min(lane + q * kWave, smp.prev_blocks - 1)];
     }
     draw_quarter(std::integral_constant<int, 2>{});
-    if (chained) {
+    if (!PROLOGUE && chained) {
       int64_t best = kKeyMax;
 #pragma unroll
       for (int q = 0; q < kChainBlocks / kWave; ++q) {
@@ -1652,16 +1673,20 @@
     for (int q = 0; q < kPairs; ++q) {
       const int j = lane + q * kWave;
       if (j < n) {
-        reinterpret_cast<f32x2*>(s_centre)[j] = g_centre[q];
-        reinterpret_cast<f32x2*>(s_ref)[j] = (ref != nullptr) ? g_ref[q] : g_centre[q];
+        if constexpr (!PROLOGUE) {
+          reinterpret_cast<f32x2*>(s_centre)[j] = g_centre[q];
+          reinterpret_cast<f32x2*>(s_ref)[j] = (ref != nullptr) ? g_ref[q] : g_centre[q];
+        }
         if (extra != nullptr) reinterpret_cast<f32x2*>(s_extra)[j] = g_extra[q];
         s_weight[j] = g_weight[q][1];
       }
     }
     for (int j = lane + kPairs * kWave; j < n; j += kWave) {
-      const f32x2 cj = reinterpret_cast<const f32x2*>(centre)[j];
-      reinterpret_cast<f32x2*>(s_centre)[j] = cj;
-      reinterpret_cast<f32x2*>(s_ref)[j] = (ref != nullptr) ? reinterpret_cast<const f32x2*>(ref)[j] : cj;
+      if constexpr (!PROLOGUE) {
+        const f32x2 cj = reinterpret_cast<const f32x2*>(centre)[j];
+        reinterpret_cast<f32x2*>(s_centre)[j] = cj;
+        reinterpret_cast<f32x2*>(s_ref)[j] = (ref != nullptr) ? reinterpret_cast<const f32x2*>(ref)[j] : cj;
+      }
       if (extra != nullptr) reinterpret_cast<f32x2*>(s_extra)[j] = reinterpret_cast<const f32x2*>(extra)[j];
       s_weight[j] = knot_weight[2 * j + 1];
     }
@@ -1676,7 +1701,7 @@
     return;
   }
 
-  {
+  if constexpr (!PROLOGUE) {
     const float* __restrict__ coef = a.coef + static_cast<size_t>(p) * n * kCoefS;
     for (int q = threadIdx.x; q < n * (kCoefS / 4); q += 2 * kWave)
       reinterpret_cast<f32x4*>(s_row)[q] = reinterpret_cast<const f32x4*>(coef)[q];
@@ -1777,7 +1802,24 @@
     publish(&a.partial_keys[slot], key);
     publish(&a.partial_feas[slot], nfeas);
   }
-  fused_tail<0>(a, smp, fused, true, nullptr);
+  fused_tail<0>(a, smp, fused, true, nullptr, PROLOGUE ? s_x0 : nullptr);
+}
+
+__global__ void __launch_bounds__(kQuadWaves * kWave) rollout_sampled_quad_kernel(const RolloutArgs a, const SampleArgs smp,
+                                                                         const FusedFinalize fused, const int uniform_lds_floats,
+                                                                         const int normals_lds_floats) {
+  extern __shared__ __attribute__((aligned(16))) float s_fused[];
+  quad_round<false>(a, smp, fused, uniform_lds_floats, normals_lds_floats, s_fused, nullptr);
+}
+
+static_assert(sizeof(RolloutArgs) + sizeof(SampleArgs) + sizeof(FusedFinalize) + sizeof(PrologueArgs) + 4 * sizeof(int) + 64 <= 4096,
+              "the kernel arguments of the first round with the prologue inside: at most 4 kB (shorten the inline path)");
+
+__global__ void __launch_bounds__((kQuadWaves + 1) * kWave) rollout_sampled_quad_prologue_kernel(
+    const RolloutArgs a, const SampleArgs smp, const FusedFinalize fused, const int uniform_lds_floats,
+    const int normals_lds_floats, const PrologueArgs tick) {
+  extern __shared__ __attribute__((aligned(16))) float s_fused[];
+  quad_round<true>(a, smp, fused, uniform_lds_floats, normals_lds_floats, s_fused, &tick);
 }
 
 #ifndef ACMPC_TRIO_CHUNK
@@ -2879,7 +2921,7 @@
 
 static hipError_t raise_lds_limit(const void* kernel, int which, size_t lds) {
   if (lds <= 64 * 1024) return hipSuccess;
-  static bool raised[13][64] = {};
+  static bool raised[14][64] = {};
   int device = 0;
   hipError_t e = hipGetDevice(&device);
   if (e != hipSuccess) return e;
@@ -2892,11 +2934,44 @@
   return hipSuccess;
 }
 
+static size_t quad_lds_bytes(int n, bool with_prologue) {
+  const size_t trace = static_cast<size_t>(trace_floats(n)) * kWave;
+  const size_t uniform = (sampled_uniform_floats(0, n) + 3) & ~static_cast<size_t>(3);
+  return (trace + uniform + static_cast<size_t>(2 * kKnots + 1) * kWave + (with_prologue ? 4 : 0)) * sizeof(float);
+}
+
+bool quad_prologue_fits(int n, const LaunchOptions& opt) {
+  return !opt.no_quad_rounds && !opt.no_pair_rounds && n <= kPrologueMaxSteps && traced_finalize_fits(0, n) &&
+         quad_lds_bytes(n, true) <= 160u * 1024u &&
+         static_cast<size_t>(prologue::workspace_doubles(n)) * sizeof(double) <= static_cast<size_t>(trace_floats(n)) * kWave * sizeof(float);
+}
+
 hipError_t launch_rollout_sampled(int mode, const RolloutArgs& rollout, const SampleArgs& sample,
                                   const FusedFinalize& fused, hipStream_t s, hipEvent_t e0, hipEvent_t e1,
-                                  const LaunchOptions& opt) {
+                                  const LaunchOptions& opt, const PrologueArgs* tick) {
   clear_stale_error();
   const int n = rollout.n;
+  if (tick != nullptr) {
+    if (mode != 0 || fused.trace == nullptr || !quad_prologue_fits(n, opt) || rollout.P != 1 || sample.prev_keys != nullptr ||
+        sample.u_extra != nullptr || sample.u_ref == nullptr || sample.spec.seed_ptr != nullptr || tick->header_by_value == 0 ||
+        tick->temporal != 0 || tick->header_value.horizon != n + 1 || fused.trace_pitch < trace_floats(n))
+      return hipErrorInvalidValue;
+    const size_t trace = static_cast<size_t>(trace_floats(n)) * kWave;
+    const size_t uniform = (sampled_uniform_floats(0, n) + 3) & ~static_cast<size_t>(3);
+    const size_t lds = quad_lds_bytes(n, true);
+    const dim3 grid((rollout.N + kWave - 1) / kWave, 1);
+    hipError_t e = raise_lds_limit(reinterpret_cast<const void*>(&rollout_sampled_quad_prologue_kernel), 13, lds);
+    if (e != hipSuccess) return e;
+    if (e0 != nullptr && e1 != nullptr) {
+      hipExtLaunchKernelGGL(rollout_sampled_quad_prologue_kernel, grid, dim3((kQuadWaves + 1) * kWave),
+                            static_cast<std::uint32_t>(lds), s, e0, e1, 0, rollout, sample, fused, static_cast<int>(trace),
+                            static_cast<int>(trace + uniform), *tick);
+    } else {
+      hipLaunchKernelGGL(rollout_sampled_quad_prologue_kernel, grid, dim3((kQuadWaves + 1) * kWave), lds, s, rollout, sample,
+                         fused, static_cast<int>(trace), static_cast<int>(trace + uniform), *tick);
+    }
+    return hipGetLastError();
+  }
   const dim3 grid((rollout.N + kWave - 1) / kWave, rollout.P);
   const size_t rollout_floats = sampled_rollout_floats(mode, n);
   const bool traced = fused.trace != nullptr;
diff --git a/ac-mpc_amd/csrc/acmpc_prologue.h b/ac-mpc_amd/csrc/acmpc_prologue.h
--- a/ac-mpc_amd/csrc/acmpc_prologue.h
+++ b/ac-mpc_amd/csrc/acmpc_prologue.h
@@ -18,7 +18,7 @@
   int32_t qp_max_iter, qp_check_every;
   uint32_t seed_lo, seed_hi;
   int32_t qp_method;
-  int32_t reserved;
+  int32_t warm_copy;
   int32_t use_map;
   int32_t map_index;
   double pose_x, pose_y;
diff --git a/ac-mpc_amd/csrc/acmpc_prologue.hip b/ac-mpc_amd/csrc/acmpc_prologue.hip
--- a/ac-mpc_amd/csrc/acmpc_prologue.hip
+++ b/ac-mpc_amd/csrc/acmpc_prologue.hip
@@ -22,30 +22,15 @@
   } while (0)
 #endif
 
+}
+
+#include "acmpc_prologue_body.h"
+
+namespace acmpc {
+
 namespace {
 
-constexpr double kPi = 3.14159265358979323846;
-
-__device__ __forceinline__ double wrap_angle(double a) {
-  const double two_pi = 2.0 * kPi;
-  double m = fmod(a + kPi, two_pi);
-  if (m != 0.0 && (m < 0.0)) m += two_pi;
-  return m - kPi;
-}
-
-struct WaveTeam {
-  static constexpr int size = 64;
-  __device__ __forceinline__ int rank() const { return static_cast<int>(threadIdx.x); }
-  __device__ __forceinline__ void sync() const { __syncthreads(); }
-  __device__ __forceinline__ double max(double v, double*) const {
-#pragma unroll
-    for (int m = 32; m >= 1; m >>= 1) {
-      const double o = __shfl_xor(v, m, 64);
-      v = o > v ? o : v;
-    }
-    return v;
-  }
-};
+using WaveTeam = prologue::WaveTeamOf<true>;
 
 }
 
@@ -192,7 +177,6 @@
   const int lane = static_cast<int>(threadIdx.x);
   const int H = __builtin_amdgcn_readfirstlane(h.horizon);
   const int n = H - 1;
-  const int m = n - 1;
   if (blockIdx.x == 1) {
     if (a.frames == nullptr || n < kVerifiedWindow) return;
     double* xr = s_mem;
@@ -226,189 +210,7 @@
     tabulate_frames(xr, yr, s_mem + 2 * n, n, lane, a.frames);
     return;
   }
-  double* table = s_mem;
-  double *tx = table, *ty = table + n, *tpsi = table + 2 * n, *tkappa = table + 3 * n, *tds = table + 4 * n,
-         *twidth = table + 5 * n, *tv = table + 6 * n;
-  double* v_hi = table + 7 * n;
-  double* seg = v_hi + n;
-  double* qv = seg + (n + 1);
-  double* qy = qv + n;
-  admm::Workspace ws;
-  ws.bind(qy + 2 * n, n);
-  double* s_coords = qy + 2 * n + admm::workspace_doubles(n);
-  const double* __restrict__ coords = a.coords;
-  const WaveTeam team;
-  constexpr int kPerLane = (kPrologueMaxSteps + 63) / 64;
-  float centre_in_v[kPerLane], centre_in_k[kPerLane];
-  double warm_v[kPerLane], warm_y[2 * kPerLane];
-  double* state = a.warm_state + static_cast<size_t>(h.localised != 0 ? 1 : 0) * a.warm_stride;
-  const double warm_flag = state[0], warm_n = state[1];
-#pragma unroll
-  for (int q = 0; q < kPerLane; ++q) {
-    const int i = min(lane + 64 * q, n - 1);
-    if (a.path_by_value != 0) {
-      centre_in_v[q] = (h.centre_is_reference != 0) ? 0.0f : a.centre_value[2 * min(i, kInlinePathPoints - 1)];
-      centre_in_k[q] = (h.centre_is_reference != 0) ? 0.0f : a.centre_value[2 * min(i, kInlinePathPoints - 1) + 1];
-    } else {
-      centre_in_v[q] = (h.centre_is_reference != 0) ? 0.0f : a.centre_in[2 * i];
-      centre_in_k[q] = (h.centre_is_reference != 0) ? 0.0f : a.centre_in[2 * i + 1];
-    }
-    warm_v[q] = (a.warm_capacity >= n) ? state[2 + i] : 0.0;
-  }
-#pragma unroll
-  for (int q = 0; q < 2 * kPerLane; ++q)
-    warm_y[q] = (a.warm_capacity >= n) ? state[2 + n + min(lane + 64 * q, 2 * n - 2)] : 0.0;
-  if (h.use_map != 0) {
-    int first = (h.map_index < 0) ? a.map_first[0] : h.map_index;
-    first = ((first % a.map_M) + a.map_M) % a.map_M;
-    const MapFrame frame = map_frame(a.map_centre, a.map_M, first);
-    for (int r = lane; r < H; r += 64) {
-      double row[3];
-      map_path_row(a.map_centre, a.map_M, first, a.map_count, a.map_points, H, r, h.lateral_offset, frame, row);
-      for (int e = 0; e < 3; ++e) {
-        s_coords[3 * r + e] = row[e];
-        a.coords_out[3 * r + e] = row[e];
-      }
-    }
-    if (lane == 0) a.index_out[0] = first;
-    team.sync();
-    coords = s_coords;
-  } else if (a.path_by_value != 0) {
-    for (int r = lane; r < 3 * H; r += 64) s_coords[r] = a.coords_value[r];
-    team.sync();
-    coords = s_coords;
-  }
-
-  ACMPC_PSTAMP(1);
-  for (int i = lane; i <= n; i += 64) {
-    const double* here = coords + 3 * ((i == n) ? 0 : i);
-    const double* from = coords + 3 * ((i == n) ? H - 1 : i);
-    const double* to = coords + 3 * ((i == n) ? 0 : i + 1);
-    const double ax = to[0] - from[0], ay = to[1] - from[1];
-    seg[i] = atan2(ay, ax);
-    if (i < n) {
-      tx[i] = here[0];
-      ty[i] = here[1];
-      tds[i] = sqrt(ax * ax + ay * ay);
-      twidth[i] = to[2];
-    }
-  }
-  team.sync();
-  for (int i = lane; i < n; i += 64) {
-    const double psi = seg[i];
-    const double behind = seg[(i == 0) ? n : i - 1];
-    tpsi[i] = psi;
-    tkappa[i] = wrap_angle(psi - behind) / (tds[i] + h.eps) + h.eps;
-  }
-  team.sync();
-  if (lane == 0) tkappa[0] = tkappa[1];
-  team.sync();
-
-  ACMPC_PSTAMP(2);
-  for (int i = lane; i < n; i += 64) {
-    double c;
-    if (h.localised != 0) {
-      c = h.v_max;
-    } else {
-      const double curvature = fabs(tkappa[i]);
-      c = sqrt(h.ay_max / (curvature + 1e-12));
-      if (curvature < h.ki_min) c = h.v_max;
-      c = fmin(c, h.v_max);
-      c = fmax(h.v_min, c);
-      c = c + 2.0;
-      if (h.has_end_velocity != 0 && i == n - 1) c = h.end_velocity;
-    }
-    v_hi[i] = c;
-  }
-  const bool warm = warm_flag == 1.0 && warm_n == static_cast<double>(n) && a.warm_capacity >= n;
-  if (warm) {
-#pragma unroll
-    for (int q = 0; q < kPerLane; ++q)
-      if (lane + 64 * q < n) qv[lane + 64 * q] = warm_v[q];
-#pragma unroll
-    for (int q = 0; q < 2 * kPerLane; ++q)
-      if (lane + 64 * q < 2 * n - 1) qy[lane + 64 * q] = warm_y[q];
-  }
-  team.sync();
-  ACMPC_PSTAMP(3);
-  const admm::Settings settings{h.a_min, h.a_max, h.v_min, h.qp_max_iter, h.qp_check_every > 0 ? h.qp_check_every : 10,
-                                h.qp_eps_abs, h.qp_eps_rel};
-  int iterations = 0;
-  const bool swept = h.qp_method == 0 && admm::exact_profile(team, ws, v_hi, tds, n, settings, qv, qy, ws.ex[0]);
-  const int status = swept ? 0 : admm::solve(team, ws, v_hi, tds, n, settings, qv, qy, warm ? 1 : 0, &iterations);
-  ACMPC_PSTAMP(4);
-  if (status == 0 && a.warm_capacity >= n) {
-    for (int i = lane; i < n; i += 64) state[2 + i] = qv[i];
-    for (int i = lane; i < 2 * n - 1; i += 64) state[2 + n + i] = qy[i];
-    if (lane == 0) {
-      state[0] = 1.0;
-      state[1] = static_cast<double>(n);
-    }
-  }
-  for (int i = lane; i < n; i += 64) tv[i] = (status == 0) ? qv[i] : 0.0;
-  team.sync();
-
-  ACMPC_PSTAMP(5);
-  if (lane == 0) {
-    const double wx = tx[0], wy = ty[0], wpsi = tpsi[0];
-    const double lateral = cos(wpsi) * (0.0 - wy) - sin(wpsi) * (h.offset - wx);
-    if (a.temporal != 0) {
-      a.x0[0] = static_cast<float>(h.offset);
-      a.x0[1] = 0.0f;
-      a.x0[2] = static_cast<float>(kPi / 2.0);
-    } else {
-      a.x0[0] = static_cast<float>(lateral);
-      a.x0[1] = static_cast<float>(wrap_angle(kPi / 2.0 - wpsi));
-      a.x0[2] = 0.0f;
-    }
-    a.status[0] = status;
-    a.status[1] = iterations;
-    a.seed[0] = h.seed_lo;
-    a.seed[1] = h.seed_hi;
-  }
-#pragma unroll
-  for (int q = 0; q < kPerLane; ++q) {
-    const int i = lane + 64 * q;
-    if (i >= n) break;
-    const double v = tv[i], ds = tds[i], kappa = tkappa[i], width = twidth[i];
-    const double vds = v * ds + 1e-12;
-    if (a.temporal != 0) {
-      float* out = a.coef + static_cast<size_t>(i) * 8;
-      const double psi = tpsi[i];
-      out[0] = static_cast<float>(tx[i]);
-      out[1] = static_cast<float>(ty[i]);
-      out[2] = static_cast<float>(cos(psi));
-      out[3] = static_cast<float>(sin(psi));
-      out[4] = static_cast<float>(psi);
-      out[5] = static_cast<float>(kappa);
-      out[6] = static_cast<float>(v);
-      out[7] = static_cast<float>(width / 2.0 - a.margin);
-    } else {
-      float* out = a.coef + static_cast<size_t>(i) * 12;
-      out[0] = static_cast<float>(ds);
-      out[1] = static_cast<float>(-(kappa * kappa) * ds);
-      out[2] = static_cast<float>(-kappa / vds);
-      out[3] = static_cast<float>(-1.0 / (v * v * ds + 1e-12));
-      out[4] = static_cast<float>(1.0 / vds);
-      out[5] = static_cast<float>(v);
-      out[6] = static_cast<float>(kappa);
-      out[7] = static_cast<float>(-width / 2.0 + a.margin);
-      out[8] = static_cast<float>(width / 2.0 - a.margin);
-      out[9] = 0.0f;
-      out[10] = 0.0f;
-      out[11] = 0.0f;
-    }
-    const double uv = fmin(fmax(v, a.u_lo0), a.u_hi0);
-    const double uk = fmin(fmax(kappa, a.u_lo1), a.u_hi1);
-    a.u_ref[2 * i] = static_cast<float>(uv);
-    a.u_ref[2 * i + 1] = static_cast<float>(uk);
-    a.centre[2 * i] = (h.centre_is_reference != 0) ? static_cast<float>(uv) : centre_in_v[q];
-    a.centre[2 * i + 1] = (h.centre_is_reference != 0) ? static_cast<float>(uk) : centre_in_k[q];
-  }
-  ACMPC_PSTAMP(6);
-  for (int e = lane; e < 7 * n; e += 64) a.table_out[e] = table[e];
-  ACMPC_PSTAMP(7);
-  (void)m;
+  prologue::tables(a, h, WaveTeam{}, s_mem, prologue::LocalRows{}, true);
 }
 
 __global__ void __launch_bounds__(256) map_window_kernel(const MapWindowArgs a) {
@@ -480,7 +282,7 @@
 }
 
 size_t prologue_lds_bytes(int n) {
-  return static_cast<size_t>(7 * n + n + (n + 1) + n + 2 * n + admm::workspace_doubles(n) + 3 * (n + 1)) * sizeof(double);
+  return static_cast<size_t>(prologue::workspace_doubles(n)) * sizeof(double);
 }
 
 hipError_t launch_prologue(const PrologueArgs& args, int n, hipStream_t s) {
diff --git a/ac-mpc_amd/csrc/acmpc_prologue_body.h b/ac-mpc_amd/csrc/acmpc_prologue_body.h
--- /dev/null
+++ b/ac-mpc_amd/csrc/acmpc_prologue_body.h
@@ -0,0 +1,285 @@
+#pragma once
+#include <hip/hip_runtime.h>
+
+#include "acmpc_admm.h"
+#include "acmpc_prologue.h"
+
+#pragma clang fp contract(off)
+
+#ifndef ACMPC_PSTAMP
+#define ACMPC_PSTAMP(slot) \
+  do {                     \
+  } while (0)
+#endif
+
+namespace acmpc {
+namespace prologue {
+
+constexpr double kPi = 3.14159265358979323846;
+
+__device__ __forceinline__ double wrap_angle(double a) {
+  const double two_pi = 2.0 * kPi;
+  double m = fmod(a + kPi, two_pi);
+  if (m != 0.0 && (m < 0.0)) m += two_pi;
+  return m - kPi;
+}
+
+template <bool ALONE>
+struct WaveTeamOf {
+  static constexpr int size = 64;
+  __device__ __forceinline__ int rank() const { return static_cast<int>(threadIdx.x) & 63; }
+  __device__ __forceinline__ void sync() const {
+    if constexpr (ALONE) {
+      __syncthreads();
+    } else {
+      __builtin_amdgcn_fence(__ATOMIC_RELEASE, "wavefront");
+      __builtin_amdgcn_wave_barrier();
+      __builtin_amdgcn_fence(__ATOMIC_ACQUIRE, "wavefront");
+    }
+  }
+  __device__ __forceinline__ double max(double v, double*) const {
+#pragma unroll
+    for (int m = 32; m >= 1; m >>= 1) {
+      const double o = __shfl_xor(v, m, 64);
+      v = o > v ? o : v;
+    }
+    return v;
+  }
+};
+
+struct LocalRows {
+  float* x0 = nullptr;
+  float* coef = nullptr;
+  float* u_ref = nullptr;
+  float* centre = nullptr;
+};
+
+constexpr int workspace_doubles(int n) {
+  return 7 * n + n + (n + 1) + n + 2 * n + admm::workspace_doubles(n) + 3 * (n + 1);
+}
+
+template <class Team>
+__device__ __forceinline__ void tables(const PrologueArgs& a, const TickHeader& h, const Team team, double* s_mem,
+                                       const LocalRows rows, const bool writer) {
+  const int lane = team.rank();
+  const int H = __builtin_amdgcn_readfirstlane(h.horizon);
+  const int n = H - 1;
+  __builtin_assume(n >= 2 && n <= kPrologueMaxSteps);
+  double* table = s_mem;
+  double *tx = table, *ty = table + n, *tpsi = table + 2 * n, *tkappa = table + 3 * n, *tds = table + 4 * n,
+         *twidth = table + 5 * n, *tv = table + 6 * n;
+  double* v_hi = table + 7 * n;
+  double* seg = v_hi + n;
+  double* qv = seg + (n + 1);
+  double* qy = qv + n;
+  admm::Workspace ws;
+  ws.bind(qy + 2 * n, n);
+  double* s_coords = qy + 2 * n + admm::workspace_doubles(n);
+  const double* __restrict__ coords = a.coords;
+  constexpr int kPerLane = (kPrologueMaxSteps + 63) / 64;
+  float centre_in_v[kPerLane], centre_in_k[kPerLane];
+  double warm_v[kPerLane], warm_y[2 * kPerLane];
+  const size_t slot = static_cast<size_t>(h.localised != 0 ? 2 : 0);
+  const double* state = a.warm_state + (slot + static_cast<size_t>(h.warm_copy & 1)) * a.warm_stride;
+  double* state_out = a.warm_state + (slot + static_cast<size_t>((h.warm_copy & 1) ^ 1)) * a.warm_stride;
+  const double warm_flag = state[0], warm_n = state[1];
+#pragma unroll
+  for (int q = 0; q < kPerLane; ++q) {
+    const int i = min(lane + 64 * q, n - 1);
+    if (a.path_by_value != 0) {
+      centre_in_v[q] = (h.centre_is_reference != 0) ? 0.0f : a.centre_value[2 * min(i, kInlinePathPoints - 1)];
+      centre_in_k[q] = (h.centre_is_reference != 0) ? 0.0f : a.centre_value[2 * min(i, kInlinePathPoints - 1) + 1];
+    } else {
+      centre_in_v[q] = (h.centre_is_reference != 0) ? 0.0f : a.centre_in[2 * i];
+      centre_in_k[q] = (h.centre_is_reference != 0) ? 0.0f : a.centre_in[2 * i + 1];
+    }
+    warm_v[q] = (a.warm_capacity >= n) ? state[2 + i] : 0.0;
+  }
+#pragma unroll
+  for (int q = 0; q < 2 * kPerLane; ++q)
+    warm_y[q] = (a.warm_capacity >= n) ? state[2 + n + min(lane + 64 * q, 2 * n - 2)] : 0.0;
+  if (h.use_map != 0) {
+    int first = (h.map_index < 0) ? a.map_first[0] : h.map_index;
+    first = ((first % a.map_M) + a.map_M) % a.map_M;
+    const MapFrame frame = map_frame(a.map_centre, a.map_M, first);
+    for (int r = lane; r < H; r += 64) {
+      double row[3];
+      map_path_row(a.map_centre, a.map_M, first, a.map_count, a.map_points, H, r, h.lateral_offset, frame, row);
+      for (int e = 0; e < 3; ++e) {
+        s_coords[3 * r + e] = row[e];
+        if (writer) a.coords_out[3 * r + e] = row[e];
+      }
+    }
+    if (writer && lane == 0) a.index_out[0] = first;
+    team.sync();
+    coords = s_coords;
+  } else if (a.path_by_value != 0) {
+    for (int r = lane; r < 3 * H; r += 64) s_coords[r] = a.coords_value[r];
+    team.sync();
+    coords = s_coords;
+  }
+
+  ACMPC_PSTAMP(1);
+  for (int i = lane; i <= n; i += 64) {
+    const double* here = coords + 3 * ((i == n) ? 0 : i);
+    const double* from = coords + 3 * ((i == n) ? H - 1 : i);
+    const double* to = coords + 3 * ((i == n) ? 0 : i + 1);
+    const double ax = to[0] - from[0], ay = to[1] - from[1];
+    seg[i] = atan2(ay, ax);
+    if (i < n) {
+      tx[i] = here[0];
+      ty[i] = here[1];
+      tds[i] = sqrt(ax * ax + ay * ay);
+      twidth[i] = to[2];
+    }
+  }
+  team.sync();
+  for (int i = lane; i < n; i += 64) {
+    const double psi = seg[i];
+    const double behind = seg[(i == 0) ? n : i - 1];
+    tpsi[i] = psi;
+    tkappa[i] = wrap_angle(psi - behind) / (tds[i] + h.eps) + h.eps;
+  }
+  team.sync();
+  if (lane == 0) tkappa[0] = tkappa[1];
+  team.sync();
+
+  ACMPC_PSTAMP(2);
+  for (int i = lane; i < n; i += 64) {
+    double c;
+    if (h.localised != 0) {
+      c = h.v_max;
+    } else {
+      const double curvature = fabs(tkappa[i]);
+      c = sqrt(h.ay_max / (curvature + 1e-12));
+      if (curvature < h.ki_min) c = h.v_max;
+      c = fmin(c, h.v_max);
+      c = fmax(h.v_min, c);
+      c = c + 2.0;
+      if (h.has_end_velocity != 0 && i == n - 1) c = h.end_velocity;
+    }
+    v_hi[i] = c;
+  }
+  const bool warm = warm_flag == 1.0 && warm_n == static_cast<double>(n) && a.warm_capacity >= n;
+  if (warm) {
+#pragma unroll
+    for (int q = 0; q < kPerLane; ++q)
+      if (lane + 64 * q < n) qv[lane + 64 * q] = warm_v[q];
+#pragma unroll
+    for (int q = 0; q < 2 * kPerLane; ++q)
+      if (lane + 64 * q < 2 * n - 1) qy[lane + 64 * q] = warm_y[q];
+  }
+  team.sync();
+  ACMPC_PSTAMP(3);
+  const admm::Settings settings{h.a_min, h.a_max, h.v_min, h.qp_max_iter, h.qp_check_every > 0 ? h.qp_check_every : 10,
+                                h.qp_eps_abs, h.qp_eps_rel};
+  int iterations = 0;
+  const bool swept = h.qp_method == 0 && admm::exact_profile(team, ws, v_hi, tds, n, settings, qv, qy, ws.ex[0]);
+  const int status = swept ? 0 : admm::solve(team, ws, v_hi, tds, n, settings, qv, qy, warm ? 1 : 0, &iterations);
+  ACMPC_PSTAMP(4);
+  if (writer && status == 0 && a.warm_capacity >= n) {
+    for (int i = lane; i < n; i += 64) state_out[2 + i] = qv[i];
+    for (int i = lane; i < 2 * n - 1; i += 64) state_out[2 + n + i] = qy[i];
+    if (lane == 0) {
+      state_out[0] = 1.0;
+      state_out[1] = static_cast<double>(n);
+    }
+  }
+  for (int i = lane; i < n; i += 64) tv[i] = (status == 0) ? qv[i] : 0.0;
+  team.sync();
+
+  ACMPC_PSTAMP(5);
+  if (lane == 0) {
+    const double wx = tx[0], wy = ty[0], wpsi = tpsi[0];
+    const double lateral = cos(wpsi) * (0.0 - wy) - sin(wpsi) * (h.offset - wx);
+    float start[3];
+    if (a.temporal != 0) {
+      start[0] = static_cast<float>(h.offset);
+      start[1] = 0.0f;
+      start[2] = static_cast<float>(kPi / 2.0);
+    } else {
+      start[0] = static_cast<float>(lateral);
+      start[1] = static_cast<float>(wrap_angle(kPi / 2.0 - wpsi));
+      start[2] = 0.0f;
+    }
+    for (int e = 0; e < 3; ++e) {
+      if (rows.x0 != nullptr) rows.x0[e] = start[e];
+      if (writer) a.x0[e] = start[e];
+    }
+    if (writer) {
+      a.status[0] = status;
+      a.status[1] = iterations;
+      a.seed[0] = h.seed_lo;
+      a.seed[1] = h.seed_hi;
+    }
+  }
+#pragma unroll
+  for (int q = 0; q < kPerLane; ++q) {
+    const int i = lane + 64 * q;
+    if (i >= n) break;
+    const double v = tv[i], ds = tds[i], kappa = tkappa[i], width = twidth[i];
+    const double vds = v * ds + 1e-12;
+    if (a.temporal != 0) {
+      if (writer) {
+        float* out = a.coef + static_cast<size_t>(i) * 8;
+        const double psi = tpsi[i];
+        out[0] = static_cast<float>(tx[i]);
+        out[1] = static_cast<float>(ty[i]);
+        out[2] = static_cast<float>(cos(psi));
+        out[3] = static_cast<float>(sin(psi));
+        out[4] = static_cast<float>(psi);
+        out[5] = static_cast<float>(kappa);
+        out[6] = static_cast<float>(v);
+        out[7] = static_cast<float>(width / 2.0 - a.margin);
+      }
+    } else {
+      float row[12];
+      row[0] = static_cast<float>(ds);
+      row[1] = static_cast<float>(-(kappa * kappa) * ds);
+      row[2] = static_cast<float>(-kappa / vds);
+      row[3] = static_cast<float>(-1.0 / (v * v * ds + 1e-12));
+      row[4] = static_cast<float>(1.0 / vds);
+      row[5] = static_cast<float>(v);
+      row[6] = static_cast<float>(kappa);
+      row[7] = static_cast<float>(-width / 2.0 + a.margin);
+      row[8] = static_cast<float>(width / 2.0 - a.margin);
+      row[9] = 0.0f;
+      row[10] = 0.0f;
+      row[11] = 0.0f;
+      if (rows.coef != nullptr) {
+#pragma unroll
+        for (int e = 0; e < 12; ++e) rows.coef[i * 12 + e] = row[e];
+      }
+      if (writer) {
+        float* out = a.coef + static_cast<size_t>(i) * 12;
+#pragma unroll
+        for (int e = 0; e < 12; ++e) out[e] = row[e];
+      }
+    }
+    const double uv = fmin(fmax(v, a.u_lo0), a.u_hi0);
+    const double uk = fmin(fmax(kappa, a.u_lo1), a.u_hi1);
+    const float cv = (h.centre_is_reference != 0) ? static_cast<float>(uv) : centre_in_v[q];
+    const float ck = (h.centre_is_reference != 0) ? static_cast<float>(uk) : centre_in_k[q];
+    if (rows.u_ref != nullptr) {
+      rows.u_ref[2 * i] = static_cast<float>(uv);
+      rows.u_ref[2 * i + 1] = static_cast<float>(uk);
+    }
+    if (rows.centre != nullptr) {
+      rows.centre[2 * i] = cv;
+      rows.centre[2 * i + 1] = ck;
+    }
+    if (writer) {
+      a.u_ref[2 * i] = static_cast<float>(uv);
+      a.u_ref[2 * i + 1] = static_cast<float>(uk);
+      a.centre[2 * i] = cv;
+      a.centre[2 * i + 1] = ck;
+    }
+  }
+  ACMPC_PSTAMP(6);
+  if (writer)
+    for (int e = lane; e < 7 * n; e += 64) a.table_out[e] = table[e];
+  ACMPC_PSTAMP(7);
+}
+
+}
+}
```

Result: slower. 15.43 billion candidate-trajectories/s (-4.6%).
